# krlong014/PySolvers

Measured on AMD Instinct MI355X. Metric: CG iterations/sec + SpMV GB/s vs HBM roofline, 5-pt Laplacian N=10M, higher is better.
Workload: dtype f64

## Files before the change

include/psk_lab.h:

```cpp
#ifndef PSK_LAB_H
#define PSK_LAB_H

#include "psk.h"

#ifdef __cplusplus
extern "C" {
#endif

int psk_lab_occupy_begin(int32_t wgs, int32_t lds_bytes, double seconds);
int psk_lab_occupy_end(int32_t *timed_out);
int psk_lab_dispatch_probe(int32_t nwg, int32_t lds_bytes, double usec, int64_t *rec_out);
int psk_lab_occupy_xcc(int32_t *counts);
int psk_lab_trisolve_workers(const psk_prec *M, int32_t which, int32_t *enrolled, int32_t *grid);
int psk_lab_trisolve_plan(int64_t n, const int32_t *rowptr, const int32_t *colidx, const double *vals, int32_t upper,
                          int32_t unit, const int32_t *nat, int32_t num_cus, int64_t syncfree_waves, int32_t *schedule,
                          double *est, int64_t *info);
int psk_lab_amg_gs_pair(psk_prec *M, int32_t set, int32_t *levels_on, int32_t *levels_eligible);
int psk_lab_spmv_rotate(const psk_csr *A, const double *const *xs, double *const *ys, int32_t nbuf, int32_t reps,
                        int32_t dot, double *avg_ms);
int psk_lab_spmv_after_write(const psk_csr *A, double *x, double *y, const double *src, double *scratch,
                             int32_t target, int32_t reps, int32_t dot, double *avg_ms);
int psk_lab_cheby_ab(const psk_prec *M, const double *v, int32_t reps, double *fused_ms, double *pieces_ms);
#ifdef __cplusplus
}
#endif

#endif
```

pysolvers_amd/_native.py:

```python
import atexit
import ctypes
import os
import sys

import numpy as np

_HERE = os.path.dirname(os.path.abspath(__file__))
LIB_PATH = os.environ.get("PSK_LIBRARY", os.path.join(_HERE, "_lib", "libpsk.so"))

PSK_OK = 0
PSK_ERR_ARG, PSK_ERR_HIP, PSK_ERR_RCCL, PSK_ERR_ALLOC, PSK_ERR_UNSUPPORTED = -1, -2, -3, -4, -5
ABI_VERSION = 4
PSK_CONVERGED, PSK_MAXITER, PSK_BREAKDOWN, PSK_TRUE_RESID_FAIL = 0, 1, 2, 3
PSK_EXIT_NONE, PSK_EXIT_TOLERANCE, PSK_EXIT_ARNOLDI_BREAKDOWN, PSK_EXIT_MAXITER, PSK_EXIT_DOT_BREAKDOWN = 0, 1, 2, 3, 4
PSK_HOST, PSK_DEVICE = 0, 1
PSK_VCYCLE_X0_GIVEN = 1
PSK_PREC_IDENTITY, PSK_PREC_JACOBI, PSK_PREC_ILU, PSK_PREC_AMG, PSK_PREC_DENSE, PSK_PREC_CHEBYSHEV = 0, 1, 2, 3, 4, 5
PSK_LAYOUT_CSR, PSK_LAYOUT_SLICED, PSK_LAYOUT_SLICED_WIDE, PSK_LAYOUT_SLICED_DICT, PSK_LAYOUT_DIAG = 0, 1, 2, 3, 4
PSK_UNIQUE_ID_BYTES = 128

STATUS_NAMES = {PSK_CONVERGED: "converged", PSK_MAXITER: "maxiter", PSK_BREAKDOWN: "breakdown",
                PSK_TRUE_RESID_FAIL: "true residual above tolerance"}


class PskCtl(ctypes.Structure):
    _fields_ = [("maxiter", ctypes.c_int64), ("tau", ctypes.c_double),
                ("fail_on_maxiter", ctypes.c_int32), ("restart", ctypes.c_int32),
                ("check_every", ctypes.c_int32), ("time_kernels", ctypes.c_int32), ("norm_b", ctypes.c_double)]


class PskResult(ctypes.Structure):
    _fields_ = [("status", ctypes.c_int32), ("success", ctypes.c_int32), ("iters", ctypes.c_int64),
                ("resid", ctypes.c_double), ("resid_recursive", ctypes.c_double),
                ("norm_b", ctypes.c_double), ("loop_ms", ctypes.c_double), ("spmv_ms", ctypes.c_double),
                ("spmv_launches", ctypes.c_int64), ("hist_len", ctypes.c_int64), ("msg", ctypes.c_char * 256),
                ("exit", ctypes.c_int32), ("reserved", ctypes.c_int32),
                ("gather_ms", ctypes.c_double), ("halo_ms", ctypes.c_double), ("comm_samples", ctypes.c_int64)]


P = ctypes.c_void_p
I32, I64, F64 = ctypes.c_int32, ctypes.c_int64, ctypes.c_double
PP = ctypes.POINTER(ctypes.c_void_p)
SIGNATURES = {
    "psk_abi_version": (ctypes.c_int, []),
    "psk_last_error": (ctypes.c_char_p, []),
    "psk_device_count": (ctypes.c_int, [ctypes.POINTER(I32)]),
    "psk_set_device": (ctypes.c_int, [I32]),
    "psk_synchronize": (ctypes.c_int, []),
    "psk_shutdown": (ctypes.c_int, []),
    "psk_shutdown_ex": (ctypes.c_int, [ctypes.c_int32]),
    "psk_dmalloc": (ctypes.c_int, [I64, PP]),
    "psk_dfree": (ctypes.c_int, [P]),
    "psk_h2d": (ctypes.c_int, [P, P, I64]),
    "psk_d2h": (ctypes.c_int, [P, P, I64]),
    "psk_dmemset0": (ctypes.c_int, [P, I64]),
    "psk_csr_create": (ctypes.c_int, [I64, I64, P, P, P, I32, PP]),
    "psk_csr_create_fd2d": (ctypes.c_int, [F64, F64, I64, PP]),
    "psk_csr_create_rect": (ctypes.c_int, [I64, I64, I64, P, P, P, I32, PP]),
    "psk_csr_info": (ctypes.c_int, [P, ctypes.POINTER(I64), ctypes.POINTER(I64)]),
    "psk_csr_layout": (ctypes.c_int, [P, I32, ctypes.POINTER(I32)] + [ctypes.POINTER(I64)] * 3),
    "psk_csr_download": (ctypes.c_int, [P, P, P, P]),
    "psk_csr_destroy": (ctypes.c_int, [P]),
    "psk_spmv": (ctypes.c_int, [P, P, P, I32]),
    "psk_spmv_timed": (ctypes.c_int, [P, P, P, I32, ctypes.POINTER(F64)]),
    "psk_dot": (ctypes.c_int, [I64, P, P, I32, ctypes.POINTER(F64)]),
    "psk_nrm2": (ctypes.c_int, [I64, P, I32, ctypes.POINTER(F64)]),
    "psk_axpy": (ctypes.c_int, [I64, F64, P, P, I32]),
    "psk_prec_create": (ctypes.c_int, [P, I32, PP]),
    "psk_prec_apply": (ctypes.c_int, [P, I64, P, P, I32]),
    "psk_prec_jacobi_uniform": (ctypes.c_int, [P, ctypes.POINTER(I32), ctypes.POINTER(ctypes.c_double)]),
    "psk_prec_create_ilu": (ctypes.c_int, [I64, P, P, P, P, P, P, P, P, PP]),
    "psk_prec_destroy": (ctypes.c_int, [P]),
    "psk_prec_create_trisolve": (ctypes.c_int, [I64, P, P, P, I32, P, P, P, I32, P, P, PP]),
    "psk_prec_create_amg": (ctypes.c_int, [I32, PP, PP, PP, PP, P, I32, I32, I32, F64, PP]),
    "psk_prec_create_dense_inverse": (ctypes.c_int, [P, I32, PP]),
    "psk_prec_create_chebyshev": (ctypes.c_int, [P, I32, F64, F64, PP]),
    "psk_prec_chebyshev_info": (ctypes.c_int, [P, ctypes.POINTER(I32), ctypes.POINTER(F64), ctypes.POINTER(F64), P]),
    "psk_prec_trisolve_schedule": (ctypes.c_int, [P, I32, I32, ctypes.POINTER(I32), ctypes.POINTER(I64),
                                                   ctypes.POINTER(I32), ctypes.POINTER(F64), ctypes.POINTER(F64)]),
    "psk_prec_trisolve_grid_info": (ctypes.c_int, [P, I32, ctypes.POINTER(I64)]),
    "psk_trisolve_grid_plan": (ctypes.c_int, [I64, P, P, P, I32, ctypes.POINTER(I64)]),
    "psk_prec_info": (ctypes.c_int, [P, ctypes.POINTER(I32)] + [ctypes.POINTER(I64)] * 5),
    "psk_mm_info": (ctypes.c_int, [ctypes.c_char_p] + [ctypes.POINTER(I64)] * 3),
    "psk_mm_read": (ctypes.c_int, [ctypes.c_char_p, P, P, P, ctypes.POINTER(I64)]),
    "psk_csr_create_mm": (ctypes.c_int, [ctypes.c_char_p, PP]),
    "psk_sa_aggregate": (ctypes.c_int, [I64, P, P, P, F64, P, ctypes.POINTER(I64), P]),
    "psk_pcg": (ctypes.c_int, [P, P, P, P, ctypes.POINTER(PskCtl), ctypes.POINTER(PskResult), P, I32]),
    "psk_gmres": (ctypes.c_int, [P, P, P, P, ctypes.POINTER(PskCtl), ctypes.POINTER(PskResult), P, I32]),
    "psk_vcycle": (ctypes.c_int, [P, P, P, ctypes.POINTER(PskCtl), ctypes.POINTER(PskResult), P, I32, I32]),
    "psk_comm_unique_id": (ctypes.c_int, [P]),
    "psk_comm_init": (ctypes.c_int, [I32, I32, P, PP]),
    "psk_comm_destroy": (ctypes.c_int, [P]),
    "psk_comm_init_dry": (ctypes.c_int, [I32, I32, PP]),
    "psk_comm_init_host": (ctypes.c_int, [I32, I32, ctypes.c_char_p, PP]),
    "psk_comm_mailbox": (ctypes.c_int, [P, ctypes.c_char_p]),
    "psk_comm_mailbox_check": (ctypes.c_int, [P, I32]),
    "psk_csr_create_fd2d_dist": (ctypes.c_int, [F64, F64, I64, P, PP, ctypes.POINTER(I64),
                                                ctypes.POINTER(I64)]),
    "psk_csr_create_dist": (ctypes.c_int, [I64, P, P, P, P, P, PP]),
    "psk_csr_halo_cols": (ctypes.c_int, [P, P, ctypes.POINTER(I64)]),
    "psk_csr_halo_peers": (ctypes.c_int, [P, P, P, P, P, ctypes.POINTER(I32)]),
    "psk_csr_halo_pack": (ctypes.c_int, [P, P, P]),
    "psk_fd2d_dist_plan": (ctypes.c_int, [I64, I32, I32] + [ctypes.POINTER(I64)] * 5),
}


LAB_PATH = os.path.join(os.path.dirname(LIB_PATH), "libpsk_lab.so")
LAB_SIGNATURES = {
    "psk_lab_occupy_begin": (ctypes.c_int, [I32, I32, F64]),
    "psk_lab_occupy_end": (ctypes.c_int, [ctypes.POINTER(I32)]),
    "psk_lab_occupy_xcc": (ctypes.c_int, [ctypes.POINTER(I32)]),
    "psk_lab_dispatch_probe": (ctypes.c_int, [I32, I32, F64, P]),
    "psk_lab_trisolve_workers": (ctypes.c_int, [P, I32, ctypes.POINTER(I32), ctypes.POINTER(I32)]),
    "psk_lab_trisolve_plan": (ctypes.c_int, [I64, P, P, P, I32, I32, P, I32, I64, ctypes.POINTER(I32),
                                             ctypes.POINTER(F64), ctypes.POINTER(I64)]),
    "psk_lab_amg_gs_pair": (ctypes.c_int, [P, I32, ctypes.POINTER(I32), ctypes.POINTER(I32)]),
    "psk_lab_spmv_rotate": (ctypes.c_int, [P, ctypes.POINTER(P), ctypes.POINTER(P), I32, I32, I32, ctypes.POINTER(F64)]),
    "psk_lab_cheby_ab": (ctypes.c_int, [P, P, I32, ctypes.POINTER(F64), ctypes.POINTER(F64)]),
    "psk_lab_spmv_after_write": (ctypes.c_int, [P, P, P, P, P, I32, I32, I32, ctypes.POINTER(F64)]),
}
_lab = None


def load_lab():
    global _lab
    if _lab is None:
        if not os.path.exists(LAB_PATH):
            raise ImportError("libpsk_lab.so not found at %s (make -C pysolvers_amd/csrc)" % LAB_PATH)
        lab = ctypes.CDLL(LAB_PATH)
        for name, (res, args) in LAB_SIGNATURES.items():
            fn = getattr(lab, name)
            fn.restype = res
            fn.argtypes = args
        _lab = lab
    return _lab


def prec_info(h):
    k = I32()
    v = [I64() for _ in range(5)]
    check(lib.psk_prec_info(h, ctypes.byref(k), *[ctypes.byref(x) for x in v]), "psk_prec_info")
    return dict(kind=k.value, n=v[0].value, nnz_l=v[1].value, nnz_u=v[2].value, levels_l=v[3].value,
                levels_u=v[4].value)


def handle_array(hs):
    arr = (ctypes.c_void_p * max(len(hs), 1))()
    for i, h in enumerate(hs):
        arr[i] = h.value if isinstance(h, ctypes.c_void_p) else h
    return ctypes.cast(arr, PP), arr


def fd2d_dist_plan(m, nranks, rank):
    v = [I64() for _ in range(5)]
    check(lib.psk_fd2d_dist_plan(m, nranks, rank, *[ctypes.byref(x) for x in v]), "psk_fd2d_dist_plan")
    return tuple(x.value for x in v)


class PskError(RuntimeError):

    def __init__(self, code, where, text):
        super().__init__("%s failed (%d): %s" % (where, code, text))
        self.code = code


def _pin_runtime():
    import importlib.util
    if os.environ.get("PSK_NO_TORCH") == "1":
        return
    if importlib.util.find_spec("torch") is not None:
        import torch


def _load():
    if not os.path.exists(LIB_PATH):
        raise ImportError("libpsk.so not found at %s — build it with `python -c 'import __graft_entry__ as "
                          "g; g.build()'` (make -C pysolvers_amd/csrc)" % LIB_PATH)
    _pin_runtime()
    lib = ctypes.CDLL(LIB_PATH, mode=ctypes.RTLD_GLOBAL)
    for name, (res, args) in SIGNATURES.items():
        fn = getattr(lib, name)
        fn.restype = res
        fn.argtypes = args
    if lib.psk_abi_version() != ABI_VERSION:
        raise ImportError("libpsk ABI version mismatch (library %d, bindings %d)" % (lib.psk_abi_version(), ABI_VERSION))
    return lib


PSK_SHUTDOWN_RESET_DEVICE = 1
lib = _load()
shut_down = False


def _shutdown():
    global shut_down
    if not shut_down:
        shut_down = True
        reset = os.environ.get("PSK_SHUTDOWN_RESET") == "1"
        lib.psk_shutdown_ex(PSK_SHUTDOWN_RESET_DEVICE if reset else 0)


atexit.register(_shutdown)


def check(rc, where):
    if rc != PSK_OK:
        raise PskError(rc, where, lib.psk_last_error().decode(errors="replace"))


def ptr(a):
    if a is None:
        return None
    if isinstance(a, int):
        return ctypes.c_void_p(a)
    if isinstance(a, np.ndarray):
        return a.ctypes.data_as(ctypes.c_void_p)
    if hasattr(a, "data_ptr"):
        return ctypes.c_void_p(a.data_ptr())
    raise TypeError("cannot take the address of %r" % type(a))


def device_count():
    n = I32(0)
    check(lib.psk_device_count(ctypes.byref(n)), "psk_device_count")
    return n.value
```

pysolvers_amd/csrc/lab.hip:

```cpp
#include "trisolve.hpp"
#include "../../include/psk_lab.h"

#include <chrono>
#include <string>

namespace psk {

__global__ __launch_bounds__(1024) void occupy_kernel(uint32_t *flag, int64_t *started, uint64_t ticks,
                                                      int32_t *timed_out) {
    extern __shared__ unsigned char occ_lds[];
    if (threadIdx.x == 0) {
        occ_lds[0] = 1;
        __hip_atomic_fetch_add(started, (int64_t)1, __ATOMIC_RELAXED, __HIP_MEMORY_SCOPE_SYSTEM);
        const uint32_t xcc = __builtin_amdgcn_s_getreg((3 << 11) | 20) & 7u;
        __hip_atomic_fetch_add(reinterpret_cast<uint32_t *>(timed_out) + 32 + xcc, 1u, __ATOMIC_RELAXED,
                               __HIP_MEMORY_SCOPE_AGENT);
    }
    const uint64_t t0 = __builtin_amdgcn_s_memrealtime();
    while (__hip_atomic_load(flag, __ATOMIC_RELAXED, __HIP_MEMORY_SCOPE_AGENT) == 0) {
        if (__builtin_amdgcn_s_memrealtime() - t0 > ticks) {
            if (threadIdx.x == 0) atomicOr(timed_out, 1);
            break;
        }
        __builtin_amdgcn_s_sleep(8);
    }
}
__global__ void occupy_release_kernel(uint32_t *flag) {
    __hip_atomic_store(flag, 1u, __ATOMIC_RELAXED, __HIP_MEMORY_SCOPE_AGENT);
}

namespace {
struct Occupier {
    hipStream_t s = nullptr;
    uint32_t *dw = nullptr;
    int64_t *started = nullptr;
    bool active = false;
};
Occupier g_occ;
}

}

extern "C" int psk_lab_occupy_begin(int32_t wgs, int32_t lds_bytes, double seconds) {
    using namespace psk;
    Context *c;
    PSK_TRY(ctx(&c));
    if (g_occ.active) return fail(PSK_ERR_ARG, "psk_lab_occupy_begin: already active");
    if (wgs < 1 || lds_bytes < 16 || lds_bytes > 160 * 1024 || seconds <= 0)
        return fail(PSK_ERR_ARG, "psk_lab_occupy_begin: bad arguments");
    if (!g_occ.s) {
        PSK_HIP(hipStreamCreateWithFlags(&g_occ.s, hipStreamNonBlocking));
        PSK_HIP(hipMalloc(&g_occ.dw, 128 * sizeof(uint32_t)));
        PSK_HIP(hipHostMalloc(&g_occ.started, 64, hipHostMallocCoherent));
    }
    PSK_HIP(hipMemsetAsync(g_occ.dw, 0, 128 * sizeof(uint32_t), g_occ.s));
    PSK_HIP(hipStreamSynchronize(g_occ.s));
    *reinterpret_cast<volatile int64_t *>(g_occ.started) = 0;
    const uint64_t ticks = (uint64_t)(seconds * 1e8);
    hipLaunchKernelGGL(occupy_kernel, dim3((unsigned)wgs), dim3(1024), (size_t)lds_bytes, g_occ.s, g_occ.dw,
                       g_occ.started, ticks, reinterpret_cast<int32_t *>(g_occ.dw + 64));
    PSK_HIP(hipGetLastError());
    g_occ.active = true;
    const auto t0 = std::chrono::steady_clock::now();
    while (*reinterpret_cast<volatile int64_t *>(g_occ.started) < wgs &&
           std::chrono::steady_clock::now() - t0 < std::chrono::seconds(5)) {
    }
    const int64_t got = *reinterpret_cast<volatile int64_t *>(g_occ.started);
    return got >= wgs ? PSK_OK : fail(PSK_ERR_HIP, "psk_lab_occupy_begin: only " + std::to_string(got) + " of " +
                                                       std::to_string(wgs) + " occupiers started");
}

extern "C" int psk_lab_occupy_end(int32_t *timed_out) {
    using namespace psk;
    Context *c;
    PSK_TRY(ctx(&c));
    if (!g_occ.active) return fail(PSK_ERR_ARG, "psk_lab_occupy_end: not active");
    hipLaunchKernelGGL(occupy_release_kernel, dim3(1), dim3(1), 0, c->stream, g_occ.dw);
    PSK_HIP(hipGetLastError());
    PSK_HIP(hipStreamSynchronize(g_occ.s));
    int32_t h = 0;
    PSK_HIP(hipMemcpy(&h, g_occ.dw + 64, sizeof(int32_t), hipMemcpyDeviceToHost));
    g_occ.active = false;
    if (timed_out) *timed_out = h;
    return PSK_OK;
}

__global__ void dispatch_probe_kernel(uint64_t ticks, int64_t *rec) {
    extern __shared__ unsigned char dp_lds[];
    if (threadIdx.x == 0) {
        dp_lds[0] = 1;
        const uint64_t t0 = __builtin_amdgcn_s_memrealtime();
        uint64_t t = t0;
        while (t - t0 < ticks) {
            __builtin_amdgcn_s_sleep(4);
            t = __builtin_amdgcn_s_memrealtime();
        }
        rec[3 * blockIdx.x + 0] = (int64_t)t0;
        rec[3 * blockIdx.x + 1] = (int64_t)t;
        rec[3 * blockIdx.x + 2] = (int64_t)(__builtin_amdgcn_s_getreg((3 << 11) | 20) & 7u);
    }
}

extern "C" int psk_lab_dispatch_probe(int32_t nwg, int32_t lds_bytes, double usec, int64_t *rec_out) {
    using namespace psk;
    if (nwg < 1 || lds_bytes < 16 || lds_bytes > 160 * 1024 || usec < 0 || !rec_out)
        return fail(PSK_ERR_ARG, "psk_lab_dispatch_probe: bad arguments");
    Context *c;
    PSK_TRY(ctx(&c));
    int64_t *rec = nullptr;
    PSK_HIP(hipMalloc(&rec, (size_t)nwg * 3 * sizeof(int64_t)));
    hipLaunchKernelGGL(dispatch_probe_kernel, dim3((unsigned)nwg), dim3(128), (size_t)lds_bytes, c->stream,
                       (uint64_t)(usec * 100.0), rec);
    hipError_t e = hipGetLastError();
    if (e == hipSuccess) e = hipMemcpyAsync(rec_out, rec, (size_t)nwg * 3 * sizeof(int64_t), hipMemcpyDeviceToHost, c->stream);
    if (e == hipSuccess) e = hipStreamSynchronize(c->stream);
    (void)hipFree(rec);
    return e == hipSuccess ? PSK_OK : fail(PSK_ERR_HIP, hipGetErrorString(e));
}

extern "C" int psk_lab_occupy_xcc(int32_t *counts) {
    using namespace psk;
    if (!counts || !g_occ.dw) return fail(PSK_ERR_ARG, "psk_lab_occupy_xcc: no occupiers yet");
    PSK_HIP(hipMemcpy(counts, g_occ.dw + 96, 8 * sizeof(int32_t), hipMemcpyDeviceToHost));
    return PSK_OK;
}

extern "C" int psk_lab_trisolve_workers(const psk_prec *M, int32_t which, int32_t *enrolled, int32_t *grid) {
    using namespace psk;
    if (!M || M->kind != PSK_PREC_ILU) return fail(PSK_ERR_ARG, "psk_lab_trisolve_workers: not a triangular-solve chain");
    const TriFactor &T = which == 0 ? M->lo : M->up;
    if (!T.present || !T.sched) return fail(PSK_ERR_ARG, "psk_lab_trisolve_workers: factor absent");
    Context *c;
    PSK_TRY(ctx(&c));
    uint32_t v = 0;
    PSK_HIP(hipStreamSynchronize(c->stream));
    PSK_HIP(hipMemcpy(&v, T.sched + kSchedLast, sizeof(uint32_t), hipMemcpyDeviceToHost));
    if (enrolled) *enrolled = (int32_t)v;
    if (grid) *grid = syncfree_grid(c);
    return PSK_OK;
}

extern "C" int psk_lab_trisolve_plan(int64_t n, const int32_t *rowptr, const int32_t *colidx, const double *vals,
                                     int32_t upper, int32_t unit, const int32_t *nat, int32_t num_cus,
                                     int64_t syncfree_waves, int32_t *schedule, double *est, int64_t *info) {
    using namespace psk;
    if (n < 0 || !rowptr || (rowptr[n] > 0 && (!colidx || !vals)) || num_cus < 1 || syncfree_waves < 1 || !schedule || !est || !info)
        return fail(PSK_ERR_ARG, "psk_lab_trisolve_plan: bad arguments");
    FactorPlan P;
    PSK_TRY(plan_factor(n, rowptr, colidx, vals, upper != 0, unit != 0,
                        nat ? std::vector<int32_t>(nat, nat + n) : std::vector<int32_t>(), num_cus, syncfree_waves, P));
    const TriFactor &T = P.T;
    *schedule = T.schedule;
    for (int i = 0; i < 6; ++i) est[i] = T.est_us[i];
    const int64_t v[8] = {T.levels, T.band.K, T.band.nblocks, T.band.ring_words, T.band.narrow ? 1 : 0,
                          T.grid.K, T.grid.dict_n, T.lv.steps};
    for (int i = 0; i < 8; ++i) info[i] = v[i];
    return PSK_OK;
}

extern "C" int psk_lab_cheby_ab(const psk_prec *M, const double *v, int32_t reps, double *fused_ms, double *pieces_ms) {
    return psk::cheby_ab(M, v, reps, fused_ms, pieces_ms);
}

extern "C" int psk_lab_amg_gs_pair(psk_prec *M, int32_t set, int32_t *levels_on, int32_t *levels_eligible) {
    using namespace psk;
    if (set < -1 || set > 1) return fail(PSK_ERR_ARG, "psk_lab_amg_gs_pair: set must be -1, 0 or 1");
    Context *c;
    PSK_TRY(ctx(&c));
    PSK_HIP(hipStreamSynchronize(c->stream));
    int on = 0, el = 0;
    PSK_TRY(amg_gs_pair(M, set, &on, &el));
    if (levels_on) *levels_on = on;
    if (levels_eligible) *levels_eligible = el;
    return PSK_OK;
}

__global__ __launch_bounds__(256) void lab_copy_kernel(int64_t n, const double *__restrict__ src, double *__restrict__ dst) {
    const int64_t i = ((int64_t)blockIdx.x * 256 + threadIdx.x) * 2;
    if (i + 1 < n) {
        const double2 v = *reinterpret_cast<const double2 *>(src + i);
        *reinterpret_cast<double2 *>(dst + i) = v;
    } else if (i < n) {
        dst[i] = src[i];
    }
}

extern "C" int psk_lab_spmv_rotate(const psk_csr *A, const double *const *xs, double *const *ys, int32_t nbuf,
                                   int32_t reps, int32_t dot, double *avg_ms) {
    using namespace psk;
    if (!A || !xs || !ys || nbuf < 1 || reps < 1 || !avg_ms) return fail(PSK_ERR_ARG, "psk_lab_spmv_rotate: bad arguments");
    if (A->comm) return fail(PSK_ERR_UNSUPPORTED, "psk_lab_spmv_rotate: sharded matrix");
    for (int32_t i = 0; i < nbuf; ++i)
        if (!xs[i] || !ys[i]) return fail(PSK_ERR_ARG, "psk_lab_spmv_rotate: NULL buffer");
    Context *c;
    PSK_TRY(ctx(&c));
    hipEvent_t e0, e1;
    PSK_HIP(hipEventCreateWithFlags(&e0, hipEventDisableSystemFence));
    PSK_HIP(hipEventCreateWithFlags(&e1, hipEventDisableSystemFence));
    const int mode = dot ? kSpmvDot : kSpmvPlain;
    DevBuf part;
    int rc = part.ensure(64);
    double *pp = dot ? part.as<double>() : nullptr;
    for (int32_t i = 0; i < nbuf && rc == PSK_OK; ++i)
        rc = launch_spmv(A, mode, xs[i], ys[i], nullptr, nullptr, pp, nullptr, c->stream);
    if (rc == PSK_OK && hipEventRecord(e0, c->stream) != hipSuccess) rc = fail(PSK_ERR_HIP, "event record");
    for (int32_t r = 0; r < reps && rc == PSK_OK; ++r)
        rc = launch_spmv(A, mode, xs[r % nbuf], ys[r % nbuf], nullptr, nullptr, pp, nullptr, c->stream);
    if (rc == PSK_OK && hipEventRecord(e1, c->stream) != hipSuccess) rc = fail(PSK_ERR_HIP, "event record");
    float ms = 0.f;
    if (rc == PSK_OK && hipEventSynchronize(e1) != hipSuccess) rc = fail(PSK_ERR_HIP, "event sync");
    if (rc == PSK_OK && hipEventElapsedTime(&ms, e0, e1) != hipSuccess) rc = fail(PSK_ERR_HIP, "event time");
    (void)hipStreamSynchronize(c->stream);
    (void)hipEventDestroy(e0);
    (void)hipEventDestroy(e1);
    part.release();
    if (rc == PSK_OK) *avg_ms = (double)ms / reps;
    return rc;
}

extern "C" int psk_lab_spmv_after_write(const psk_csr *A, double *x, double *y, const double *src, double *scratch,
                                        int32_t target, int32_t reps, int32_t dot, double *avg_ms) {
    using namespace psk;
    if (!A || !x || !y || !src || !scratch || reps < 1 || reps > 256 || !avg_ms)
        return fail(PSK_ERR_ARG, "psk_lab_spmv_after_write: bad arguments");
    if (A->comm || A->ncols != A->n) return fail(PSK_ERR_UNSUPPORTED, "psk_lab_spmv_after_write: square unsharded only");
    Context *c;
    PSK_TRY(ctx(&c));
    std::vector<hipEvent_t> ea((size_t)reps), eb((size_t)reps);
    for (int32_t r = 0; r < reps; ++r) {
        PSK_HIP(hipEventCreateWithFlags(&ea[(size_t)r], hipEventDisableSystemFence));
        PSK_HIP(hipEventCreateWithFlags(&eb[(size_t)r], hipEventDisableSystemFence));
    }
    const int mode = dot ? kSpmvDot : kSpmvPlain;
    DevBuf part;
    int rc = part.ensure(64);
    double *pp = dot ? part.as<double>() : nullptr;
    const int64_t n = A->n;
    const unsigned g = (unsigned)((n + 511) / 512);
    double *dst = target == 1 ? x : scratch;
    rc = launch_spmv(A, mode, x, y, nullptr, nullptr, pp, nullptr, c->stream);
    for (int32_t r = 0; r < reps && rc == PSK_OK; ++r) {
        if (target > 0) {
            hipLaunchKernelGGL(lab_copy_kernel, dim3(g), dim3(256), 0, c->stream, n, src, dst);
            if (hipGetLastError() != hipSuccess) rc = fail(PSK_ERR_HIP, "lab copy");
        }
        if (rc == PSK_OK)
            rc = launch_spmv(A, mode, x, y, nullptr, nullptr, pp, nullptr, c->stream, ea[(size_t)r], eb[(size_t)r]);
    }
    double tot = 0.0;
    if (rc == PSK_OK && hipStreamSynchronize(c->stream) != hipSuccess) rc = fail(PSK_ERR_HIP, "sync");
    for (int32_t r = 0; r < reps && rc == PSK_OK; ++r) {
        float ms = 0.f;
        if (hipEventElapsedTime(&ms, ea[(size_t)r], eb[(size_t)r]) != hipSuccess) rc = fail(PSK_ERR_HIP, "event time");
        tot += ms;
    }
    (void)hipStreamSynchronize(c->stream);
    for (int32_t r = 0; r < reps; ++r) {
        (void)hipEventDestroy(ea[(size_t)r]);
        (void)hipEventDestroy(eb[(size_t)r]);
    }
    part.release();
    if (rc == PSK_OK) *avg_ms = tot / reps;
    return rc;
}
```

pysolvers_amd/csrc/pcg.hip:

```cpp
#include "psk_internal.hpp"
#include "pcg_state.hpp"

#include <cstdlib>

#include <climits>
#include <cmath>
#include <cstdio>


namespace psk {

template <int JAC, bool FUSED>
__global__ __launch_bounds__(kBlock) void pcg_init_kernel(int64_t n, const double *__restrict__ b,
                                                          const double *__restrict__ dinv, double ds,
                                                          double *__restrict__ p, GridSum gs, PcgInitFin fin,
                                                          int64_t ntiles) {
    constexpr int TPW = 2;
    const int tid = threadIdx.x;
    int64_t tl[TPW];
    bool tv[TPW];
    double acc[TPW][2];
    uint32_t ticket[TPW];
#pragma unroll
    for (int q = 0; q < TPW; ++q) {
        const int64_t t = (int64_t)blockIdx.x * TPW + q;
        tv[q] = t < ntiles;
        tl[q] = tv[q] ? t : ntiles - 1;
        const int64_t row = tl[q] * kBlock + tid;
        const bool has = tv[q] && row < n;
        const double bi = has ? __builtin_nontemporal_load(b + row) : 0.0;
        const double d = JAC == 1 ? (has ? dinv[row] : 0.0) : ds;
        const double u = JAC ? d * bi : bi;
        if (has) p[row] = u;
        acc[q][0] = has ? bi * bi : 0.0;
        acc[q][1] = has ? u * bi : 0.0;
    }
    __shared__ GridSumTile<2> gsl[TPW];
#pragma unroll
    for (int q = 0; q < TPW; ++q) {
        ticket[q] = 0;
        if (tv[q] && gs.grp_log2 >= 0 && tid == 0)
            ticket[q] = gridsum_draw(gridsum_counter(gs, gridsum_group_of(tl[q], gs.grp_log2)));
    }
    if (tid < TPW) gsl[tid].cnt = 0;
    if (tid == 0 && blockIdx.x == 0 && (gs.nt + TPW - 1) / TPW != gridDim.x) atomicOr(gs.err, 2);
    __syncthreads();
    if (FUSED)
        gridsum_tiles_publish<TPW, 2>(gs, gsl, acc, ticket, tl, tv, fin);
    else
        gridsum_tiles_publish<TPW, 2>(gs, gsl, acc, ticket, tl, tv);
}

__global__ void pcg_init_finish_kernel(const double *g, int P, double tau, PcgState *st, double *udr,
                                       int64_t *hdone, int64_t hgen) {
    if (threadIdx.x == 0) pcg_init_state(rank_sum(g, P, 2, 0), rank_sum(g, P, 2, 1), tau, st, udr, hdone, hgen, 0);
}

template <int JAC, bool FIRST>
__global__ __launch_bounds__(kBlock) void pcg_update_kernel(
    int64_t n, double *__restrict__ r, const double *__restrict__ b, const double *__restrict__ Ap,
    const double *__restrict__ dinv, double ds, const double *__restrict__ pap, int nparts, GridSum gs, PcgState *st,
    const double *__restrict__ udr, int64_t k, TileMap tm) {
    const double udk = udr[k];
    const int32_t dn = st->done;
    const double pap0 = pap[0];
    __asm__ volatile("" ::"s"(dn), "s"(pap0), "s"(udk));
    if (dn) return;
    double pTAp = pap0;
    for (int q = 1; q < nparts; ++q) pTAp += pap[q];
    __shared__ double sh[2 * kWaves];
    if (pTAp == 0.0) {
        if (blockIdx.x == 0 && threadIdx.x == 0) {
            st->brk_kind = 2;
            st->iters = k;
            set_done(st, 2, k + 2);
        }
        return;
    }
    const double alpha = udk / pTAp;
    if (blockIdx.x == 0 && threadIdx.x == 0) st->live = k;
    const int64_t tile = tile_of_block(tm);
    const int64_t i = tile * kVecTile + 2 * threadIdx.x;
    const bool pair = i + 1 < n;
    uint32_t ticket = 0;
    double rr = 0.0, ur = 0.0;
    if (pair) {
        const dv2 ro = FIRST ? ld2nt(b + i) : ld2(r + i), a = ld2nt(Ap + i);
        dv2 d{ds, ds};
        if (JAC == 1) d = ld2(dinv + i);
        ticket = gridsum_ticket(gs, tile);
        dv2 rn;
        rn.x = ro.x - alpha * a.x;
        rn.y = ro.y - alpha * a.y;
        double u0 = rn.x, u1 = rn.y;
        if (JAC) {
            u0 = d.x * rn.x;
            u1 = d.y * rn.y;
        }
        st2(r + i, rn);
        rr = fma(rn.x, rn.x, rr);
        rr = fma(rn.y, rn.y, rr);
        ur = fma(u0, rn.x, ur);
        ur = fma(u1, rn.y, ur);
    } else if (i < n) {
        ticket = gridsum_ticket(gs, tile);
        const double rn = (FIRST ? b[i] : r[i]) - alpha * Ap[i];
        const double u0 = JAC == 2 ? ds * rn : JAC ? dinv[i] * rn : rn;
        r[i] = rn;
        rr = rn * rn;
        ur = u0 * rn;
    }
    block_sum2(rr, ur, sh);
    const double v[2] = {rr, ur};
    if (threadIdx.x >= 64) return;
    const bool lane0 = threadIdx.x == 0;
    if (gs.grp_log2 < 0) {
        if (lane0) {
            gridsum_put(gs.gslots + tile * 2, v[0]);
            gridsum_put(gs.gslots + tile * 2 + 1, v[1]);
        }
        gridsum_final_wave<2>(gs);
        return;
    }
    if (lane0) {
        gridsum_put(gs.slots + gridsum_slot(gs, tile) * 2, v[0]);
        gridsum_put(gs.slots + gridsum_slot(gs, tile) * 2 + 1, v[1]);
    }
    const uint32_t tk = __builtin_amdgcn_readfirstlane(ticket);
    const int64_t g = gridsum_group_of(tile, gs.grp_log2);
    int64_t base;
    const int64_t cnt = gridsum_members(gs, g, base);
    if (tk != (uint32_t)(cnt - 1)) return;
    double gr[2];
    gridsum_take<2, 64>(gs.slots, g << gs.grp_log2, cnt, gs.err, nullptr, gr);
    if (lane0) {
        gridsum_reset(gridsum_counter(gs, g));
        gridsum_put(gs.gslots + g * 2, gr[0]);
        gridsum_put(gs.gslots + g * 2 + 1, gr[1]);
    }
    gridsum_final_wave<2>(gs);
}

template <int JAC>
__global__ __launch_bounds__(kBlock) void pcg_direction_kernel(
    int64_t n, double *__restrict__ x, const double *__restrict__ r, PRing pr, const double *__restrict__ dinv,
    double ds, const double *__restrict__ pap, const double *__restrict__ rrur, int nparts, PcgState *st,
    double *__restrict__ udr, double *__restrict__ hist, double *__restrict__ alphas, int64_t k, int64_t maxiter,
    int fail_on_maxiter, int64_t tile_base, TileMap tm) {
    const double udk = udr[k];
    const int64_t live = st->live;
    const double tauNB = st->tauNormB, pap0 = pap[0], rr0 = rrur[0], ur0 = rrur[1];
    __asm__ volatile("" ::"s"(live), "s"(pap0), "s"(rr0), "s"(ur0), "s"(udk), "s"(tauNB));
    if (live != k) return;
    double pTAp = pap0, rr = rr0, ur = ur0;
    for (int q = 1; q < nparts; ++q) {
        pTAp += pap[q];
        rr += rrur[2 * q];
        ur += rrur[2 * q + 1];
    }
    const int64_t tile = tile_base + tile_of_block(tm);
    const double *pcur = pr.b[k % kPcgDefer];
    double *pnext = pr.b[(k + 1) % kPcgDefer];
    const int q = pcg_pending(k);
    double alpha, beta;
    if (!pcg_direction_scalars(n, x, pcur, pTAp, rr, ur, udk, tauNB, st, udr, hist, k, maxiter, fail_on_maxiter,
                               alpha, beta, tile, &pr, alphas))
        return;
    const bool flush = q == kPcgDefer - 1 || k == maxiter - 1;
    const bool x0 = k < kPcgDefer;
    if (tile == 0 && threadIdx.x == 0) {
        alphas[k] = alpha;
        if (flush) st->x_written = 1;
    }
    const int64_t i = tile * kVecTile + 2 * threadIdx.x;
    if (i + 1 < n) {
        const dv2 ro = ld2nt(r + i), po = ld2(pcur + i);
        dv2 d{ds, ds};
        if (JAC == 1) d = ld2nt(dinv + i);
        double u0 = ro.x, u1 = ro.y;
        if (JAC) {
            u0 = d.x * ro.x;
            u1 = d.y * ro.y;
        }
        if (flush) {
            dv2 xo{0.0, 0.0};
            if (!x0) xo = ld2nt(x + i);
            dv2 pp[kPcgDefer > 1 ? kPcgDefer - 1 : 1];
#pragma unroll
            for (int t = 1; t < kPcgDefer; ++t)
                if (t <= q) pp[t - 1] = ld2nt(pr.b[(k - t) % kPcgDefer] + i);
#pragma unroll
            for (int t = kPcgDefer - 1; t >= 1; --t)
                if (t <= q) {
                    const double a = alphas[k - t];
                    xo.x = xo.x + a * pp[t - 1].x;
                    xo.y = xo.y + a * pp[t - 1].y;
                }
            dv2 xn;
            xn.x = xo.x + alpha * po.x;
            xn.y = xo.y + alpha * po.y;
            st2nt(x + i, xn);
        }
        dv2 pn;
        pn.x = u0 + beta * po.x;
        pn.y = u1 + beta * po.y;
        st2(pnext + i, pn);
    } else if (i < n) {
        const double u0 = JAC == 2 ? ds * r[i] : JAC ? dinv[i] * r[i] : r[i];
        const double pi = pcur[i];
        if (flush) x[i] = pcg_catch_up(x0 ? 0.0 : x[i], &pr, q, k, alphas, i) + alpha * pi;
        pnext[i] = u0 + beta * pi;
    }
}

__global__ void pcg_flush_kernel(int64_t n, double *__restrict__ x, PRing pr, const double *__restrict__ alphas,
                                 int64_t k) {
    const int64_t i = (int64_t)blockIdx.x * kBlock + threadIdx.x;
    if (i < n) x[i] = pcg_catch_up(k < kPcgDefer ? 0.0 : x[i], &pr, pcg_pending(k), k, alphas, i);
}

constexpr int kPcgStateWords = (int)(sizeof(PcgState) / 8);
constexpr int kPcgFinishWord = 8;
static_assert(sizeof(PcgState) % 8 == 0 && kPcgFinishWord + kPcgStateWords + 1 <= 64, "SolveKit::hmap words");
__global__ __launch_bounds__(kBlock) void pcg_finish_kernel(const PcgState *st, const uint32_t *cnt, const int32_t *err,
                                                            int64_t *hw) {
    constexpr int kPer = (kGridSumMaxGroups + kBlock) / kBlock;
    uint32_t v[kPer];
#pragma unroll
    for (int i = 0; i < kPer; ++i) {
        const int g = (int)threadIdx.x + i * kBlock;
        v[i] = cnt[(int64_t)(g < kGridSumMaxGroups ? g : kGridSumMaxGroups) * kGridSumCntStride];
    }
    uint32_t any = 0;
#pragma unroll
    for (int i = 0; i < kPer; ++i) any |= v[i];
    const bool bad = __syncthreads_or(any != 0);
    if (threadIdx.x < kPcgStateWords)
        __hip_atomic_store(hw + threadIdx.x, reinterpret_cast<const int64_t *>(st)[threadIdx.x], __ATOMIC_RELAXED,
                           __HIP_MEMORY_SCOPE_SYSTEM);
    if (threadIdx.x == 0)
        __hip_atomic_store(hw + kPcgStateWords, (int64_t)(*err | (bad ? 4 : 0)), __ATOMIC_RELAXED,
                           __HIP_MEMORY_SCOPE_SYSTEM);
}

__global__ __launch_bounds__(kBlock) void pcg_gen_init_kernel(int64_t n, const double *__restrict__ b,
                                                              double *__restrict__ x, double *__restrict__ r) {
    const int64_t i = (int64_t)blockIdx.x * kBlock + threadIdx.x;
    if (i < n) {
        r[i] = b[i];
        x[i] = 0.0;
    }
}

__global__ __launch_bounds__(kBlock) void pcg_gen_init2_kernel(int64_t n, const double *__restrict__ r,
                                                               const double *__restrict__ u, double *__restrict__ p,
                                                               GridSum gs, PcgInitFin fin) {
    __shared__ double sh[kWaves];
    const int64_t i = (int64_t)blockIdx.x * kVecTile + 2 * threadIdx.x;
    const uint32_t ticket = gridsum_ticket(gs);
    double bb = 0.0, ur = 0.0;
    for (int64_t j = i; j < i + 2 && j < n; ++j) {
        const double rj = r[j], uj = u[j];
        p[j] = uj;
        bb = fma(rj, rj, bb);
        ur = fma(uj, rj, ur);
    }
    const double v[2] = {block_sum(bb, sh), block_sum(ur, sh)};
    gridsum_publish<2>(gs, v, sh, ticket, fin);
}

__global__ __launch_bounds__(kBlock) void pcg_dot_kernel(int64_t n, const double *__restrict__ a,
                                                         const double *__restrict__ c, GridSum gs,
                                                         const PcgState *st) {
    if (st->done) return;
    __shared__ double sh[kWaves];
    const int64_t i = (int64_t)blockIdx.x * kVecTile + threadIdx.x;
    const uint32_t ticket = gridsum_ticket(gs);
    double acc = 0.0;
    if (i < n) acc = a[i] * c[i];
    if (i + kBlock < n) acc = fma(a[i + kBlock], c[i + kBlock], acc);
    const double v = block_sum(acc, sh);
    gridsum_publish<1>(gs, &v, sh, ticket);
}

__global__ __launch_bounds__(kBlock) void pcg_gen_direction_kernel(
    int64_t n, double *__restrict__ x, const double *__restrict__ u, double *__restrict__ p,
    const double *__restrict__ pap, const double *__restrict__ rrur, const double *__restrict__ ur_gen, PcgState *st,
    double *__restrict__ udr, double *__restrict__ hist, int64_t k, int64_t maxiter, int fail_on_maxiter) {
    if (st->live != k) return;
    double alpha, beta;
    if (!pcg_direction_scalars(n, x, p, *pap, rrur[0], *ur_gen, udr[k], st->tauNormB, st, udr, hist, k, maxiter,
                               fail_on_maxiter, alpha, beta, blockIdx.x))
        return;
    const int64_t i = (int64_t)blockIdx.x * kVecTile + 2 * threadIdx.x;
    for (int64_t j = i; j < i + 2 && j < n; ++j) {
        const double pj = p[j];
        x[j] = x[j] + alpha * pj;
        p[j] = u[j] + beta * pj;
    }
}


static inline size_t align_up(size_t v, size_t a) { return (v + a - 1) / a * a; }

struct PcgWork {
    double *x, *r, *p, *Ap, *u, *part1, *part2, *part3, *udr, *hist;
    PRing pr;
    double *alphas;
    double *pinit;
    double *part1g, *part2g, *initg;
    PcgState *st;
};

static int pcg_workspace(psk_csr *A, int64_t maxiter, bool gen, bool own_x, int P, PcgWork &w) {
    const size_t vec = align_up((size_t)A->n * 8, 256), vecc = align_up((size_t)A->ncols * 8, 256);
    const size_t nx = own_x ? 1 : 0;
    const size_t big = (2 + nx + (gen ? 1 : 0)) * vec + (gen ? 1 : kPcgDefer) * vecc;
    PSK_TRY(A->ws.ensure(big > 0 ? big : 256));
    char *b = A->ws.as<char>();
    w.r = reinterpret_cast<double *>(b);
    w.Ap = reinterpret_cast<double *>(b + vec);
    w.x = own_x ? reinterpret_cast<double *>(b + 2 * vec) : nullptr;
    char *pb = b + (2 + nx) * vec;
    w.p = reinterpret_cast<double *>(pb);
    w.u = gen ? reinterpret_cast<double *>(pb + vecc) : nullptr;
    for (int t = 0; t < kPcgDefer; ++t)
        w.pr.b[t] = gen ? (t == 0 ? w.p : nullptr) : reinterpret_cast<double *>(pb + t * vecc);
    const size_t small = align_up(sizeof(PcgState), 256) + 2 * align_up(kMaxGrid * 8, 256) +
                         align_up(2 * kMaxGrid * 8, 256) + align_up((size_t)(maxiter + 2) * 8, 256) +
                         align_up((size_t)(maxiter + 1) * 8, 256) + align_up((size_t)(maxiter + 1) * 8, 256) + 256;
    const size_t gath = P > 1 ? align_up((size_t)P * 8, 256) + 2 * align_up((size_t)P * 16, 256) : 0;
    PSK_TRY(A->ws_small.ensure(small + gath));
    char *s = A->ws_small.as<char>();
    w.st = reinterpret_cast<PcgState *>(s);
    s += align_up(sizeof(PcgState), 256);
    w.part1 = reinterpret_cast<double *>(s);
    s += align_up(kMaxGrid * 8, 256);
    w.part3 = reinterpret_cast<double *>(s);
    s += align_up(kMaxGrid * 8, 256);
    w.part2 = reinterpret_cast<double *>(s);
    s += align_up(2 * kMaxGrid * 8, 256);
    w.udr = reinterpret_cast<double *>(s);
    s += align_up((size_t)(maxiter + 2) * 8, 256);
    w.hist = reinterpret_cast<double *>(s);
    s += align_up((size_t)(maxiter + 1) * 8, 256);
    w.alphas = reinterpret_cast<double *>(s);
    s += align_up((size_t)(maxiter + 1) * 8, 256);
    w.pinit = reinterpret_cast<double *>(s);
    s += 256;
    if (P > 1) {
        w.part1g = reinterpret_cast<double *>(s);
        s += align_up((size_t)P * 8, 256);
        w.part2g = reinterpret_cast<double *>(s);
        s += align_up((size_t)P * 16, 256);
        w.initg = reinterpret_cast<double *>(s);
    } else {
        w.part1g = w.part1;
        w.part2g = w.part2;
        w.initg = w.pinit;
    }
    return PSK_OK;
}

static void set_msg(psk_result *res, const char *m) {
    std::snprintf(res->msg, sizeof(res->msg), "%s", m);
}

}

using namespace psk;

extern "C" int psk_pcg(const psk_csr *Ac, const psk_prec *M, const double *b, double *xout,
                       const psk_ctl *ctl, psk_result *res, double *hist, int32_t loc) {
    if (!Ac || !b || !xout || !ctl || !res) return fail(PSK_ERR_ARG, "psk_pcg: NULL argument");
    if (ctl->maxiter < 0) return fail(PSK_ERR_ARG, "psk_pcg: maxiter < 0");
    if (M && M->n != Ac->n) return fail(PSK_ERR_ARG, "psk_pcg: preconditioner size mismatch");
    if (!Ac->comm && Ac->ncols != Ac->n) return fail(PSK_ERR_ARG, "psk_pcg: matrix must be square");
    psk_csr *A = const_cast<psk_csr *>(Ac);
    Context *c;
    PSK_TRY(ctx(&c));
    std::lock_guard<std::mutex> solve_lock(c->solve_mu);
    hipStream_t s = c->stream;
    std::memset(res, 0, sizeof(*res));
    const int64_t n = A->n, maxiter = ctl->maxiter;
    const bool gen = prec_is_general(M);
    if (gen && A->comm) return fail(PSK_ERR_UNSUPPORTED, "psk_pcg: ILU preconditioning of a sharded matrix");
    const bool sharded = A->comm != nullptr;
    const int P = sharded ? A->comm->nranks : 1;
    const bool dev_io = loc == PSK_DEVICE;
    PcgWork w;
    PSK_TRY(pcg_workspace(A, maxiter, gen, !dev_io, P, w));
    if (dev_io) w.x = xout;
    SolveKit *kit;
    PSK_TRY(solve_kit(c, ctl->time_kernels > 0, &kit));
    const double *dinv = (M && M->kind == PSK_PREC_JACOBI) ? M->dinv : nullptr;
    const int jac = !dinv ? 0 : M->dinv_uniform ? 2 : 1;
    const double ds = jac == 2 ? M->dinv_value : 0.0;
    const int64_t nv = n > 0 ? (n + kVecTile - 1) / kVecTile : 1;
    if (nv > INT32_MAX) return fail(PSK_ERR_UNSUPPORTED, "psk_pcg: vector too long for a one-shot grid");
    const bool init_diag = !gen && !sharded && (jac == 0 || jac == 2) && pcg_init_diag_eligible(A);
    const int64_t nsl = n > 0 ? (n + kBlock - 1) / kBlock : 1;
    GridSum gs0, gs2, gs3;
    if (!init_diag) PSK_TRY(gridsum_prepare(c, gen ? nv : nsl, 2, w.pinit, &gs0));
    PSK_TRY(gridsum_prepare(c, nv, 2, w.part2, &gs2));
    PSK_TRY(gridsum_prepare(c, nv, 1, w.part3, &gs3));
    volatile int64_t *hdone = kit->hmap;
    const int64_t hgen = (int64_t)(++kit->solve_gen & 0x7FFFFF) << kStampGenShift;
    *hdone = 0;
    const PcgInitFin fin{ctl->tau, w.st, w.udr, const_cast<int64_t *>(hdone), hgen, gen ? 1 : 0, 0};
    const double *bd = b;
    if (!dev_io) {
        PSK_TRY(to_device_vec(b, loc, n, gen ? w.Ap : w.r, s));
        bd = gen ? w.Ap : w.r;
    }
    psk_comm *mbc = sharded && A->comm->mb ? A->comm : nullptr;
    uint64_t seq0 = 0;
    if (mbc) seq0 = mbox_next(mbc, &gs0);
    PSK_HIP(hipEventRecord(kit->ev0, s));
    const dim3 gk((unsigned)nv);
    if (gen) {
        const unsigned nb = (unsigned)((n + kBlock - 1) / kBlock);
        if (n > 0) hipLaunchKernelGGL(pcg_gen_init_kernel, dim3(nb), dim3(kBlock), 0, s, n, bd, w.x, w.r);
        PSK_TRY(prec_apply_dev(M, n, w.r, w.u, s));
        hipLaunchKernelGGL(pcg_gen_init2_kernel, gk, dim3(kBlock), 0, s, n, w.r, w.u, w.p, gs0, fin);
    } else if (init_diag) {
        PcgInitFin fin3 = fin;
        fin3.off = 1;
        PSK_TRY(launch_pcg_init_diag(A, bd, jac == 2 ? ds : 1.0, w.p, w.Ap, w.part1, fin3, s));
    } else {
        const dim3 gi((unsigned)((nsl + 1) / 2));
#define PSK_PCG_INIT(J, F) \
        hipLaunchKernelGGL((pcg_init_kernel<J, F>), gi, dim3(kBlock), 0, s, n, bd, dinv, ds, w.p, gs0, fin, nsl)
        if (jac == 2) { if (sharded) PSK_PCG_INIT(2, false); else PSK_PCG_INIT(2, true); }
        else if (jac == 1) { if (sharded) PSK_PCG_INIT(1, false); else PSK_PCG_INIT(1, true); }
        else { if (sharded) PSK_PCG_INIT(0, false); else PSK_PCG_INIT(0, true); }
#undef PSK_PCG_INIT
    }
    PSK_HIP(hipGetLastError());
    if (sharded) {
        if (mbc) PSK_TRY(mbox_gather(mbc, seq0, 2, w.initg, nullptr, s));
        else PSK_TRY(allgather(A, w.pinit, w.initg, 2, s));
        hipLaunchKernelGGL(pcg_init_finish_kernel, dim3(1), dim3(64), 0, s, w.initg, P, ctl->tau, w.st, w.udr,
                           const_cast<int64_t *>(hdone), hgen);
        PSK_HIP(hipGetLastError());
    }

    const int L = 2, NS = kPollSlots;
    static_assert(kPollSlots >= L + 2, "poll slots");
    int C = ctl->check_every > 0 ? ctl->check_every : (n >= (1 << 20) ? 2 : 16);
    hipEvent_t *fev = kit->fev;
    const int TP = kTimedSlots;
    hipEvent_t *ta = kit->ta, *tb = kit->tb;
    int64_t tk[kTimedSlots];
    bool tgat[kTimedSlots], thalo[kTimedSlots];
    for (int i = 0; i < TP; ++i) {
        tk[i] = -1;
        tgat[i] = thalo[i] = false;
    }
    std::vector<float> spmv_ms;
    if (ctl->time_kernels) spmv_ms.assign((size_t)maxiter, -1.0f);
    double gat_sum = 0.0, halo_sum = 0.0;
    int64_t gat_n = 0, halo_n = 0;
    auto harvest = [&](int slot) -> int {
        if (tk[slot] < 0) return PSK_OK;
        float ms = 0.f;
        PSK_HIP(hipEventSynchronize(tb[slot]));
        PSK_HIP(hipEventElapsedTime(&ms, ta[slot], tb[slot]));
        spmv_ms[(size_t)tk[slot]] = ms;
        tk[slot] = -1;
        if (tgat[slot]) {
            PSK_HIP(hipEventSynchronize(kit->gb[slot]));
            PSK_HIP(hipEventElapsedTime(&ms, kit->ga[slot], kit->gb[slot]));
            gat_sum += ms;
            ++gat_n;
            tgat[slot] = false;
        }
        if (thalo[slot]) {
            PSK_HIP(hipEventSynchronize(kit->hb[slot]));
            PSK_HIP(hipEventElapsedTime(&ms, kit->ha[slot], kit->hb[slot]));
            halo_sum += ms;
            ++halo_n;
            thalo[slot] = false;
        }
        return PSK_OK;
    };

    int64_t ov_lo = 0, ov_hi = nv;
    static const bool overlap_on = [] {
        const char *e = std::getenv("PSK_HALO_OVERLAP");
        return !(e && std::atoi(e) == 0);
    }();
    const bool overlap = overlap_on && sharded && !gen && halo_split(A, kVecTile, nv, ov_lo, ov_hi);
    hipStream_t cs = nullptr;
    hipEvent_t ev_k3a = kit->ev_a, ev_halo = kit->ev_b;
    bool halo_pending = false;
    if (overlap) PSK_TRY(comm_stream(c, &cs));

    int64_t launched = 0;
    int rc = PSK_OK;
    for (int64_t k = 0; k < maxiter && rc == PSK_OK; ++k) {
        if (k > 0 && k % C == 0) {
            const int64_t chunk = k / C;
            const int slot = (int)((chunk - 1) % NS);
            if (hipEventRecord(fev[slot], s) != hipSuccess) rc = fail(PSK_ERR_HIP, "event");
            if (rc == PSK_OK && chunk - 1 - L >= 0) {
                const int os = (int)((chunk - 1 - L) % NS);
                if (hipEventSynchronize(fev[os]) != hipSuccess) rc = fail(PSK_ERR_HIP, "event sync");
                else {
                    const int64_t hv = *hdone;
                    if ((hv & ~kStampMask) == hgen && (hv & kStampMask) != 0 &&
                        (hv & kStampMask) <= (chunk - L) * (int64_t)C + 1)
                        break;
                }
            }
            if (rc != PSK_OK) break;
        }
        double *pk = gen ? w.p : w.pr.b[k % kPcgDefer];
        double *pn = gen ? w.p : w.pr.b[(k + 1) % kPcgDefer];
        const bool timed = ctl->time_kernels > 0 && k % ctl->time_kernels == 0 && !(init_diag && k == 0);
        int slot = (int)((k / (ctl->time_kernels > 0 ? ctl->time_kernels : 1)) % TP);
        if (timed) {
            if ((rc = harvest(slot)) != PSK_OK) break;
            tk[slot] = k;
        }
        if (halo_pending) {
            if (hipStreamWaitEvent(s, ev_halo, 0) != hipSuccess) { rc = fail(PSK_ERR_HIP, "halo wait"); break; }
            halo_pending = false;
        } else if (A->comm) {
            const bool th = timed && !A->comm->dry && !A->peers.empty();
            if (th && hipEventRecord(kit->ha[slot], s) != hipSuccess) { rc = fail(PSK_ERR_HIP, "event"); break; }
            if ((rc = halo_exchange(A, pk, s)) != PSK_OK) break;
            if (th) {
                if (hipEventRecord(kit->hb[slot], s) != hipSuccess) { rc = fail(PSK_ERR_HIP, "event"); break; }
                thalo[slot] = true;
            }
        }
        uint64_t seq1 = 0;
        if (!(init_diag && k == 0) &&
            (rc = launch_spmv(A, kSpmvDot, pk, w.Ap, nullptr, nullptr, w.part1, &w.st->done, s, timed ? ta[slot] : nullptr,
                              timed ? tb[slot] : nullptr, 0, mbc ? &seq1 : nullptr)) != PSK_OK)
            break;
        const TileMap tm2 = tile_map_for(nv, false);
        if (sharded) {
            hipEvent_t g0 = timed ? kit->ga[slot] : nullptr, g1 = timed ? kit->gb[slot] : nullptr;
            if (mbc) {
                rc = mbox_gather(mbc, seq1, 1, w.part1g, &w.st->done, s, g0, g1);
            } else {
                if (g0 && hipEventRecord(g0, s) != hipSuccess) rc = fail(PSK_ERR_HIP, "event");
                if (rc == PSK_OK) rc = allgather(A, w.part1, w.part1g, 1, s);
                if (rc == PSK_OK && g1 && hipEventRecord(g1, s) != hipSuccess) rc = fail(PSK_ERR_HIP, "event");
            }
            if (rc != PSK_OK) break;
            if (timed) tgat[slot] = true;
        }
        GridSum gs2k = gs2;
        const uint64_t seq2 = mbc ? mbox_next(mbc, &gs2k) : 0;
        const bool first = k == 0 && !gen && dev_io;
        const double *pap_k = w.part1g;
#define PSK_PCG_K2(J, F)                                                                                       \
        hipLaunchKernelGGL((pcg_update_kernel<J, F>), gk, dim3(kBlock), 0, s, n, w.r, bd, w.Ap, dinv, ds, pap_k,     \
                           P, gs2k, w.st, w.udr, k, tm2)
        if (jac == 2) { if (first) PSK_PCG_K2(2, true); else PSK_PCG_K2(2, false); }
        else if (jac == 1) { if (first) PSK_PCG_K2(1, true); else PSK_PCG_K2(1, false); }
        else { if (first) PSK_PCG_K2(0, true); else PSK_PCG_K2(0, false); }
#undef PSK_PCG_K2
        if (sharded && (rc = mbc ? mbox_gather(mbc, seq2, 2, w.part2g, &w.st->done, s)
                                 : allgather(A, w.part2, w.part2g, 2, s)) != PSK_OK)
            break;
        if (gen) {
            if ((rc = prec_apply_dev(M, n, w.r, w.u, s)) != PSK_OK) break;
            hipLaunchKernelGGL(pcg_dot_kernel, gk, dim3(kBlock), 0, s, n, w.u, w.r, gs3, w.st);
            hipLaunchKernelGGL(pcg_gen_direction_kernel, gk, dim3(kBlock), 0, s, n, w.x, w.u, w.p, w.part1, w.part2,
                               w.part3, w.st, w.udr, w.hist, k, maxiter, ctl->fail_on_maxiter);
        } else {
            auto k3 = [&](int64_t t0, int64_t t1) {
                if (t1 <= t0) return;
                const dim3 g3((unsigned)(t1 - t0));
                const TileMap tm3 = tile_map_for(t1 - t0, false);
                if (jac == 2)
                    hipLaunchKernelGGL(pcg_direction_kernel<2>, g3, dim3(kBlock), 0, s, n, w.x, w.r, w.pr, dinv, ds,
                                       w.part1g, w.part2g, P, w.st, w.udr, w.hist, w.alphas, k, maxiter,
                                       ctl->fail_on_maxiter, t0, tm3);
                else if (jac == 1)
                    hipLaunchKernelGGL(pcg_direction_kernel<1>, g3, dim3(kBlock), 0, s, n, w.x, w.r, w.pr, dinv, ds,
                                       w.part1g, w.part2g, P, w.st, w.udr, w.hist, w.alphas, k, maxiter,
                                       ctl->fail_on_maxiter, t0, tm3);
                else
                    hipLaunchKernelGGL(pcg_direction_kernel<0>, g3, dim3(kBlock), 0, s, n, w.x, w.r, w.pr, dinv, ds,
                                       w.part1g, w.part2g, P, w.st, w.udr, w.hist, w.alphas, k, maxiter,
                                       ctl->fail_on_maxiter, t0, tm3);
            };
            if (overlap && k + 1 < maxiter) {
                k3(0, ov_lo);
                k3(ov_hi, nv);
                if ((rc = halo_exchange_async(A, pn, s, cs, ev_k3a, ev_halo, timed ? kit->ha[slot] : nullptr,
                                              timed ? kit->hb[slot] : nullptr)) != PSK_OK)
                    break;
                if (timed) thalo[slot] = true;
                k3(ov_lo, ov_hi);
                halo_pending = true;
            } else {
                k3(0, nv);
            }
        }
        if (hipGetLastError() != hipSuccess) { rc = fail(PSK_ERR_HIP, "pcg launch"); break; }
        launched = k + 1;
    }
    if (halo_pending && hipStreamWaitEvent(s, ev_halo, 0) != hipSuccess && rc == PSK_OK) rc = fail(PSK_ERR_HIP, "halo wait");
    if (rc == PSK_OK && hipEventRecord(kit->ev1, s) != hipSuccess) rc = fail(PSK_ERR_HIP, "event");
    int64_t *hw = kit->hmap + kPcgFinishWord;
    if (rc == PSK_OK) {
        hipLaunchKernelGGL(pcg_finish_kernel, dim3(1), dim3(kBlock), 0, s, w.st, c->gs_cnt, c->gs_err, hw);
        if (hipGetLastError() != hipSuccess) rc = fail(PSK_ERR_HIP, "pcg finish");
    }
    if (rc == PSK_OK && hipStreamSynchronize(s) != hipSuccess) rc = fail(PSK_ERR_HIP, "pcg sync");
    PcgState hs;
    std::memcpy(&hs, hw, sizeof(PcgState));
    if (rc == PSK_OK) rc = gridsum_check_result(c, (int32_t)hw[kPcgStateWords]);
    if (rc == PSK_OK && gen) rc = prec_check_error(M, s);
    if (rc == PSK_OK && ctl->time_kernels)
        for (int i = 0; i < TP && rc == PSK_OK; ++i) rc = harvest(i);
    if (rc == PSK_OK) {
        float ms = 0.f;
        (void)hipEventElapsedTime(&ms, kit->ev0, kit->ev1);
        res->loop_ms = ms;
        res->norm_b = hs.normB;
        int64_t nk = 0, nhist = 0;
        if (hs.done == 1) {
            res->status = PSK_CONVERGED;
            res->success = 1;
            res->iters = hs.iters;
            res->resid = hs.resid;
            res->exit = hs.normB == 0.0 ? PSK_EXIT_NONE
                        : hs.resid <= hs.tauNormB ? PSK_EXIT_TOLERANCE : PSK_EXIT_MAXITER;
            nk = nhist = hs.normB == 0.0 ? 0 : hs.iters;
        } else if (hs.done == 2) {
            res->status = PSK_BREAKDOWN;
            res->exit = PSK_EXIT_DOT_BREAKDOWN;
            res->success = 0;
            res->iters = hs.iters;
            res->resid = NAN;
            set_msg(res, hs.brk_kind == 1 ? "breakdown dot(u,r)==0" : "breakdown dot(p, Ap)==0");
            nk = hs.brk_kind == 1 ? 0 : hs.iters + 1;
            nhist = hs.brk_kind == 1 ? 0 : hs.iters;
        } else {
            res->status = PSK_MAXITER;
            res->exit = PSK_EXIT_MAXITER;
            res->success = 0;
            res->iters = maxiter > 0 ? maxiter - 1 : 0;
            set_msg(res, "failure to converge");
            nk = nhist = launched;
        }
        const int64_t nh = nhist < maxiter ? nhist : maxiter;
        if (hist && nh > 0 && hipMemcpy(hist, w.hist, (size_t)nh * 8, hipMemcpyDeviceToHost) != hipSuccess)
            rc = fail(PSK_ERR_HIP, "hist copy");
        if (rc == PSK_OK) {
            res->hist_len = nh;
            res->resid_recursive = nh > 0 ? hs.last_hist : hs.normB;
            if (res->status == PSK_MAXITER) res->resid = maxiter > 0 ? res->resid_recursive : hs.normB;
            bool x_written = hs.x_written != 0;
            bool more = !dev_io;
            if (!gen && hs.done == 2 && hs.brk_kind != 1 && pcg_pending(hs.iters) > 0 && n > 0) {
                hipLaunchKernelGGL(pcg_flush_kernel, dim3((unsigned)((n + kBlock - 1) / kBlock)), dim3(kBlock), 0, s, n,
                                   w.x, w.pr, w.alphas, (int64_t)hs.iters);
                if (hipGetLastError() != hipSuccess) rc = fail(PSK_ERR_HIP, "pcg flush");
                x_written = true;
                more = true;
            }
            if (rc == PSK_OK && !x_written && n > 0) {
                if (hipMemsetAsync(w.x, 0, (size_t)n * 8, s) != hipSuccess) rc = fail(PSK_ERR_HIP, "x zero");
                more = true;
            }
            if (rc == PSK_OK && !dev_io) rc = from_device_vec(w.x, loc, n, xout, s);
            if (rc == PSK_OK && more && hipStreamSynchronize(s) != hipSuccess) rc = fail(PSK_ERR_HIP, "x copy");
        }
        if (ctl->time_kernels) {
            double tot = 0.0;
            const int64_t cnt = nk < (int64_t)spmv_ms.size() ? nk : (int64_t)spmv_ms.size();
            int64_t nt = 0;
            for (int64_t i = 0; i < cnt; i += ctl->time_kernels)
                if (spmv_ms[(size_t)i] >= 0.0f) {
                    tot += spmv_ms[(size_t)i];
                    ++nt;
                }
            res->spmv_launches = nt;
            res->spmv_ms = nt > 0 ? tot / (double)nt : 0.0;
            res->gather_ms = gat_n > 0 ? gat_sum / (double)gat_n : 0.0;
            res->halo_ms = halo_n > 0 ? halo_sum / (double)halo_n : 0.0;
            res->comm_samples = gat_n;
        }
    }
    if (rc != PSK_OK) (void)hipStreamSynchronize(s);
    return rc;
}
```

pysolvers_amd/csrc/pcg_state.hpp:

```cpp
#pragma once
#include "psk_internal.hpp"

namespace psk {

struct PcgState {
    int32_t done;
    int32_t brk_kind;
    int64_t iters;
    double resid;
    double normB;
    double tauNormB;
    int64_t live;
    int64_t *hdone;
    int64_t hgen;
    double last_hist;
    int32_t x_written;
    int32_t pad;
};

constexpr int kStampGenShift = 40;
constexpr int64_t kStampMask = ((int64_t)1 << kStampGenShift) - 1;
__device__ __forceinline__ void set_done(PcgState *st, int32_t v, int64_t stamp) {
    st->done = v;
    if (st->hdone) {
        __hip_atomic_store(st->hdone, st->hgen | stamp, __ATOMIC_RELAXED, __HIP_MEMORY_SCOPE_SYSTEM);
        __threadfence_system();
    }
}

__device__ __forceinline__ void pcg_init_state(double bb, double ur, double tau, PcgState *st, double *udr,
                                               int64_t *hdone, int64_t hgen, int32_t x_written) {
    const double normB = sqrt(bb);
    st->normB = normB;
    st->tauNormB = tau * normB;
    st->iters = 0;
    st->resid = 0.0;
    st->brk_kind = 0;
    st->live = -1;
    st->hdone = hdone;
    st->hgen = hgen;
    st->last_hist = normB;
    st->x_written = x_written;
    udr[0] = ur;
    if (normB == 0.0) {
        st->iters = 1;
        set_done(st, 1, 1);
    } else if (ur == 0.0) {
        st->brk_kind = 1;
        st->iters = 0;
        set_done(st, 2, 1);
    } else {
        st->done = 0;
    }
}

struct PcgInitFin {
    double tau;
    PcgState *st;
    double *udr;
    int64_t *hdone;
    int64_t hgen;
    int32_t x_written;
    int32_t off;
    __device__ void operator()(const double *r) const {
        pcg_init_state(r[off], r[off + 1], tau, st, udr, hdone, hgen, x_written);
    }
};

#ifndef PSK_PCG_DEFER
#define PSK_PCG_DEFER 8
#endif
constexpr int kPcgDefer = PSK_PCG_DEFER;
static_assert(kPcgDefer >= 1 && kPcgDefer <= 8, "kPcgDefer");
struct PRing {
    double *b[kPcgDefer];
};
__host__ __device__ inline int pcg_pending(int64_t k) { return (int)(k % kPcgDefer); }

__device__ __forceinline__ double pcg_catch_up(double xj, const PRing *pr, int q, int64_t k,
                                               const double *__restrict__ alphas, int64_t j) {
    for (int t = q; t >= 1; --t) xj = xj + alphas[k - t] * pr->b[(k - t) % kPcgDefer][j];
    return xj;
}

__device__ inline bool pcg_direction_scalars(int64_t n, double *__restrict__ x, const double *__restrict__ p,
                                             double pTAp, double rr, double ur, double udk, double tauNB,
                                             PcgState *st, double *__restrict__ udr, double *__restrict__ hist, int64_t k,
                                             int64_t maxiter, int fail_on_maxiter, double &alpha, double &beta,
                                             int64_t tile, const PRing *pr = nullptr,
                                             const double *__restrict__ alphas = nullptr) {
    alpha = udk / pTAp;
    const double normR = sqrt(rr);
    if (tile == 0 && threadIdx.x == 0) {
        hist[k] = normR;
        st->last_hist = normR;
    }
    if (normR <= tauNB || (!fail_on_maxiter && k == maxiter - 1)) {
        const int64_t i = tile * kVecTile + 2 * threadIdx.x;
        const bool x0 = pr && k < kPcgDefer;
        for (int64_t j = i; j < i + 2 && j < n; ++j) {
            double xj = x0 ? 0.0 : x[j];
            if (pr) xj = pcg_catch_up(xj, pr, pcg_pending(k), k, alphas, j);
            x[j] = xj + alpha * p[j];
        }
        if (tile == 0 && threadIdx.x == 0) {
            st->iters = k + 1;
            st->resid = normR;
            st->x_written = 1;
            set_done(st, 1, k + 2);
        }
        return false;
    }
    beta = ur / udk;
    if (tile == 0 && threadIdx.x == 0) udr[k + 1] = ur;
    return true;
}

bool pcg_init_diag_eligible(const psk_csr *A);
int launch_pcg_init_diag(const psk_csr *A, const double *b, double xs, double *p, double *Ap, double *out3,
                         const PcgInitFin &fin, hipStream_t s);

}
```

pysolvers_amd/csrc/psk_internal.hpp:

```cpp
#pragma once

#include <hip/hip_runtime.h>
#include <rccl/rccl.h>

#include <cstdint>
#include <cstring>
#include <mutex>
#include <string>
#include <vector>

#include "../../include/psk.h"

namespace psk {

constexpr int kBlock = 256;
constexpr int kWaves = kBlock / 64;
constexpr int kChunk = 1280;
constexpr int kMaxGrid = 2048;
constexpr int kVecTile = 2 * kBlock;
constexpr int64_t kMaxNnz = (int64_t)INT32_MAX - kChunk - kBlock;

void set_error(int code, const std::string &msg);
int fail(int code, const std::string &msg);
const char *hip_err_str(hipError_t e);
// ... 356 lines not shown
    const int64_t t = gs.nt - sb * S;
    return t >= S ? ((int64_t)1 << gl) : (t - l + kGridSumL - 1) >> kGridSumLLog;
}

__device__ __forceinline__ void gridsum_put(uint64_t *sl, double v) {
    __hip_atomic_store(sl, (uint64_t)__double_as_longlong(v), __ATOMIC_RELAXED, __HIP_MEMORY_SCOPE_AGENT);
}
__device__ __forceinline__ uint32_t gridsum_draw(uint32_t *c) {
    return __hip_atomic_fetch_add(c, 1u, __ATOMIC_RELAXED, __HIP_MEMORY_SCOPE_AGENT);
}
__device__ __forceinline__ void gridsum_reset(uint32_t *c) {
    __hip_atomic_store(c, 0u, __ATOMIC_RELAXED, __HIP_MEMORY_SCOPE_AGENT);
}
__device__ __forceinline__ uint32_t *gridsum_counter(const GridSum &gs, int64_t g) {
    return gs.cnt + g * kGridSumCntStride;
}
__device__ __forceinline__ uint64_t gridsum_wait(const uint64_t *sl, int32_t *err) {
    uint64_t bits = __hip_atomic_load(sl, __ATOMIC_RELAXED, __HIP_MEMORY_SCOPE_AGENT);
    if (bits != kGridSumSentinel) return bits;
    const uint64_t t0 = __builtin_amdgcn_s_memrealtime();
    while ((bits = __hip_atomic_load(sl, __ATOMIC_RELAXED, __HIP_MEMORY_SCOPE_AGENT)) == kGridSumSentinel) {
        if (__builtin_amdgcn_s_memrealtime() - t0 > kGridSumWaitTicks) {
            atomicOr(err, 1);
            return 0x7FF8000000000000ull;
        }
        __builtin_amdgcn_s_sleep(1);
    }
    return bits;
}

template <int W, int NT>
__device__ __forceinline__ void gridsum_take(uint64_t *src, int64_t start, int64_t cnt, int32_t *err, double *sh,
                                             double *res) {
    constexpr int B = NT == 64 ? 8 : 4;
    const uint32_t lane = NT == 64 ? (threadIdx.x & 63) : threadIdx.x;
    const uint32_t n = (uint32_t)cnt;
    uint64_t *p = src + start * W;
#pragma unroll
    for (int c = 0; c < W; ++c) {
        double a = 0.0;
        bool ok = true;
        for (uint32_t m0 = lane; m0 < n; m0 += NT * B) {
            uint64_t v[B];
#pragma unroll
            for (int i = 0; i < B; ++i) {
                const uint32_t m = __builtin_elementwise_min(m0 + (uint32_t)(i * NT), n - 1);
                v[i] = __hip_atomic_load(p + (m * W + c), __ATOMIC_RELAXED, __HIP_MEMORY_SCOPE_AGENT);
            }
#pragma unroll
            for (int i = 0; i < B; ++i) {
                const uint64_t x = m0 + (uint32_t)(i * NT) < n ? v[i] : 0x8000000000000000ull;
                ok = ok && x != kGridSumSentinel;
                a += __longlong_as_double((long long)x);
            }
        }
        if (!ok) {
            a = 0.0;
            for (uint32_t m = lane; m < n; m += NT)
                a += __longlong_as_double((long long)gridsum_wait(p + (m * W + c), err));
        }
        for (uint32_t m = lane; m < n; m += NT)
            p[m * W + c] = kGridSumSentinel;
        res[c] = NT == 64 ? wave_total(a) : block_sum(a, sh);
    }
}

__device__ __forceinline__ int64_t gridsum_slot(const GridSum &gs, int64_t t) {
    const int32_t gl = gs.grp_log2;
    const int64_t g = gridsum_group_of(t, gl), j = (t & ((kGridSumL << gl) - 1)) >> kGridSumLLog;
    return (g << gl) + j;
}

__device__ __forceinline__ uint32_t gridsum_ticket(const GridSum &gs, int64_t tile) {
    uint32_t t = 0;
    if (threadIdx.x == 0 && gridDim.x != gs.nt) atomicOr(gs.err, 2);
    if (gs.grp_log2 >= 0 && threadIdx.x == 0) t = gridsum_draw(gridsum_counter(gs, gridsum_group_of(tile, gs.grp_log2)));
    return t;
}
__device__ __forceinline__ uint32_t gridsum_ticket(const GridSum &gs) { return gridsum_ticket(gs, blockIdx.x); }

struct GridSumNoFin {
    __device__ void operator()(const double *) const {}
};

template <int W, class F = GridSumNoFin>
__device__ __forceinline__ void gridsum_final(const GridSum &gs, double *sh, const F &fin = F()) {
    __shared__ uint32_t tk;
    if (threadIdx.x == 0) tk = gridsum_draw(gridsum_counter(gs, kGridSumMaxGroups));
    __syncthreads();
    const bool last = tk == (uint32_t)(gs.ngroups - 1);
    __syncthreads();
    if (!last) return;
    double r[W];
    gridsum_take<W, kBlock>(gs.gslots, 0, gs.ngroups, gs.err, sh, r);
    if (threadIdx.x == 0) {
        gridsum_reset(gridsum_counter(gs, kGridSumMaxGroups));
#pragma unroll
        for (int c = 0; c < W; ++c) gs.out[c] = r[c];
        gridsum_mail<W>(gs, r);
        fin(r);
    }
}

template <int W, class F = GridSumNoFin>
__device__ __forceinline__ void gridsum_publish_tile(const GridSum &gs, const double *v, double *sh, uint32_t ticket,
                                                     int64_t b, const F &fin = F()) {
    if (gs.grp_log2 < 0) {
        if (threadIdx.x == 0)
#pragma unroll
            for (int c = 0; c < W; ++c) gridsum_put(gs.gslots + b * W + c, v[c]);
        gridsum_final<W>(gs, sh, fin);
        return;
    }
    __shared__ uint32_t tk;
    if (threadIdx.x == 0) {
#pragma unroll
        for (int c = 0; c < W; ++c) gridsum_put(gs.slots + gridsum_slot(gs, b) * W + c, v[c]);
        tk = ticket;
    }
    __syncthreads();
    const int64_t g = gridsum_group_of(b, gs.grp_log2);
    int64_t base;
    const int64_t cnt = gridsum_members(gs, g, base);
    const bool last = tk == (uint32_t)(cnt - 1);
    __syncthreads();
    if (!last) return;
    double r[W];
    gridsum_take<W, kBlock>(gs.slots, g << gs.grp_log2, cnt, gs.err, sh, r);
    if (threadIdx.x == 0) {
        gridsum_reset(gridsum_counter(gs, g));
#pragma unroll
        for (int c = 0; c < W; ++c) gridsum_put(gs.gslots + g * W + c, r[c]);
    }
    gridsum_final<W>(gs, sh, fin);
}
template <int W, class F = GridSumNoFin>
__device__ __forceinline__ void gridsum_publish(const GridSum &gs, const double *v, double *sh, uint32_t ticket,
                                                const F &fin = F()) {
    gridsum_publish_tile<W>(gs, v, sh, ticket, blockIdx.x, fin);
}

template <int W>
struct GridSumTile {
    uint32_t cnt;
    uint32_t ticket;
    double part[kWaves * W];
};
template <int W>
__device__ __forceinline__ uint32_t gridsum_tile_begin(const GridSum &gs, GridSumTile<W> &L, int64_t tile) {
    if (threadIdx.x == 0) {
        L.cnt = 0;
        if (gridDim.x != gs.nt) atomicOr(gs.err, 2);
    }
    __syncthreads();
    uint32_t t = 0;
    if (gs.grp_log2 >= 0 && threadIdx.x == 0) t = gridsum_draw(gridsum_counter(gs, gridsum_group_of(tile, gs.grp_log2)));
    return t;
}

template <int W, class F = GridSumNoFin>
__device__ __forceinline__ void gridsum_final_wave(const GridSum &gs, const F &fin = F()) {
    const bool lane0 = (threadIdx.x & 63) == 0;
    uint32_t f = 0;
    if (lane0) f = gridsum_draw(gridsum_counter(gs, kGridSumMaxGroups));
    f = __builtin_amdgcn_readfirstlane(f);
    if (f != (uint32_t)(gs.ngroups - 1)) return;
    double r[W];
    gridsum_take<W, 64>(gs.gslots, 0, gs.ngroups, gs.err, nullptr, r);
    if (lane0) {
        gridsum_reset(gridsum_counter(gs, kGridSumMaxGroups));
#pragma unroll
        for (int c = 0; c < W; ++c) gs.out[c] = r[c];
        gridsum_mail<W>(gs, r);
        fin(r);
    }
}

template <int W>
__device__ __forceinline__ void gridsum_tile_publish(const GridSum &gs, GridSumTile<W> &L, const double *v,
                                                     uint32_t ticket, int64_t tile) {
    const bool lane0 = (threadIdx.x & 63) == 0;
    const int wave = __builtin_amdgcn_readfirstlane(threadIdx.x >> 6);
    uint32_t old = 0;
    if (lane0) {
#pragma unroll
        for (int c = 0; c < W; ++c) L.part[wave * W + c] = v[c];
        if (threadIdx.x == 0) L.ticket = ticket;
        __builtin_amdgcn_fence(__ATOMIC_RELEASE, "workgroup", "local");
        old = atomicAdd(&L.cnt, 1u);
    }
    if (__builtin_amdgcn_readfirstlane(old) != kWaves - 1) return;
    __builtin_amdgcn_fence(__ATOMIC_ACQUIRE, "workgroup", "local");
    double s[W];
#pragma unroll
    for (int c = 0; c < W; ++c) {
        s[c] = L.part[c];
#pragma unroll
        for (int w = 1; w < kWaves; ++w) s[c] += L.part[w * W + c];
    }
    const uint32_t tk = L.ticket;
    if (gs.grp_log2 < 0) {
        if (lane0)
#pragma unroll
            for (int c = 0; c < W; ++c) gridsum_put(gs.gslots + tile * W + c, s[c]);
        gridsum_final_wave<W>(gs);
        return;
    }
    if (lane0)
#pragma unroll
        for (int c = 0; c < W; ++c) gridsum_put(gs.slots + gridsum_slot(gs, tile) * W + c, s[c]);
    const int64_t g = gridsum_group_of(tile, gs.grp_log2);
    int64_t base;
    const int64_t cnt = gridsum_members(gs, g, base);
    if (tk != (uint32_t)(cnt - 1)) return;
    double r[W];
    gridsum_take<W, 64>(gs.slots, g << gs.grp_log2, cnt, gs.err, nullptr, r);
    if (lane0) {
        gridsum_reset(gridsum_counter(gs, g));
#pragma unroll
        for (int c = 0; c < W; ++c) gridsum_put(gs.gslots + g * W + c, r[c]);
    }
    gridsum_final_wave<W>(gs);
}

template <int TPW, int W, class F = GridSumNoFin>
__device__ __forceinline__ void gridsum_tiles_publish(const GridSum &gs, GridSumTile<W> *L, const double (*acc)[W],
                                                      const uint32_t *ticket, const int64_t *tl, const bool *tv,
                                                      const F &fin = F()) {
    const bool lane0 = (threadIdx.x & 63) == 0;
    const int wave = __builtin_amdgcn_readfirstlane(threadIdx.x >> 6);
    bool mine[TPW];
    uint32_t tk[TPW];
#pragma unroll
    for (int q = 0; q < TPW; ++q) {
        mine[q] = false;
        tk[q] = 0;
        if (!tv[q]) continue;
        double ws[W];
#pragma unroll
        for (int c = 0; c < W; ++c) ws[c] = wave_total(acc[q][c]);
        uint32_t old = 0;
        if (lane0) {
#pragma unroll
            for (int c = 0; c < W; ++c) L[q].part[wave * W + c] = ws[c];
            if (threadIdx.x == 0) L[q].ticket = ticket[q];
            __builtin_amdgcn_fence(__ATOMIC_RELEASE, "workgroup", "local");
            old = atomicAdd(&L[q].cnt, 1u);
        }
        if (__builtin_amdgcn_readfirstlane(old) != kWaves - 1) continue;
        __builtin_amdgcn_fence(__ATOMIC_ACQUIRE, "workgroup", "local");
        double sum[W];
#pragma unroll
        for (int c = 0; c < W; ++c) {
            sum[c] = L[q].part[c];
#pragma unroll
            for (int w = 1; w < kWaves; ++w) sum[c] += L[q].part[w * W + c];
        }
        tk[q] = L[q].ticket;
        if (lane0)
#pragma unroll
            for (int c = 0; c < W; ++c)
                gridsum_put(gs.grp_log2 < 0 ? gs.gslots + tl[q] * W + c : gs.slots + gridsum_slot(gs, tl[q]) * W + c, sum[c]);
        mine[q] = true;
    }
#pragma unroll
    for (int q = 0; q < TPW; ++q) {
        if (!mine[q]) continue;
        if (gs.grp_log2 < 0) {
            gridsum_final_wave<W>(gs, fin);
            continue;
        }
        const int64_t g = gridsum_group_of(tl[q], gs.grp_log2);
        int64_t base;
        const int64_t cnt = gridsum_members(gs, g, base);
        if (tk[q] != (uint32_t)(cnt - 1)) continue;
        double r[W];
        gridsum_take<W, 64>(gs.slots, g << gs.grp_log2, cnt, gs.err, nullptr, r);
        if (lane0) {
            gridsum_reset(gridsum_counter(gs, g));
#pragma unroll
            for (int c = 0; c < W; ++c) gridsum_put(gs.gslots + g * W + c, r[c]);
        }
        gridsum_final_wave<W>(gs, fin);
    }
}

int gridsum_prepare(Context *c, int64_t nt, int W, double *out, GridSum *gs);
int gridsum_check(Context *c);
int gridsum_check_enqueue(Context *c, int32_t *host_word);
int gridsum_check_result(Context *c, int32_t host_word);

struct TileMap {
    int64_t a;
    int32_t r;
    int32_t rev;
    int64_t c;
};
inline TileMap tile_map_for(int64_t ntiles, bool banded, bool rev = false) {
    return banded && ntiles >= 64 ? TileMap{ntiles >> 3, (int32_t)(ntiles & 7), rev ? 1 : 0, 0} : TileMap{0, 0, 0, 0};
}
inline TileMap tile_map_chunked(int64_t ntiles, int64_t c) {
    return c > 0 && ntiles >= 8 * c ? TileMap{0, 0, 0, c} : TileMap{0, 0, 0, 0};
}
__device__ __forceinline__ int64_t tile_of_block(TileMap tm) {
    const int64_t b = blockIdx.x;
    if (tm.c > 0) {
        const int64_t k = b & 7, j = b >> 3;
        const int64_t t = ((j / tm.c) * 8 + k) * tm.c + j % tm.c;
        const int64_t full = (int64_t)(gridDim.x / (8 * tm.c)) * 8 * tm.c;
        return b < full ? t : b;
    }
    if (tm.a == 0) return b;
    const int64_t k = b & 7, j = b >> 3;
    const int64_t start = k * tm.a + (k < tm.r ? k : tm.r);
    return tm.rev ? start + (tm.a + (k < tm.r ? 1 : 0)) - 1 - j : start + j;
}

typedef double dv2 __attribute__((ext_vector_type(2)));
__device__ __forceinline__ dv2 ld2(const double *p) { return *reinterpret_cast<const dv2 *>(p); }
__device__ __forceinline__ dv2 ld2nt(const double *p) {
    return __builtin_nontemporal_load(reinterpret_cast<const dv2 *>(p));
}
__device__ __forceinline__ void st2(double *p, dv2 v) { *reinterpret_cast<dv2 *>(p) = v; }
__device__ __forceinline__ void st2nt(double *p, dv2 v) { __builtin_nontemporal_store(v, reinterpret_cast<dv2 *>(p)); }

__device__ __forceinline__ void block_range(int64_t ntiles, int64_t &t0, int64_t &t1) {
    const int64_t g = gridDim.x, b = blockIdx.x;
    t0 = ntiles * b / g;
    t1 = ntiles * (b + 1) / g;
}

inline int grid_for_rows(const Context *c, int64_t rows, int per_tile) {
    int64_t tiles = (rows + per_tile - 1) / per_tile;
    if (tiles < 1) tiles = 1;
    return (int)(tiles < c->grid_cap ? tiles : c->grid_cap);
}

int to_device_vec(const double *src, int32_t loc, int64_t n, double *dst, hipStream_t s);
int from_device_vec(const double *src, int32_t loc, int64_t n, double *dst, hipStream_t s);
int halo_exchange(psk_csr *A, double *x_local, hipStream_t s);
int halo_exchange_async(psk_csr *A, double *x, hipStream_t s, hipStream_t cs, hipEvent_t ev_a, hipEvent_t ev_b,
                        hipEvent_t t0 = nullptr, hipEvent_t t1 = nullptr);
bool halo_split(const psk_csr *A, int64_t tile, int64_t nv, int64_t &lo, int64_t &hi);
int allgather(psk_csr *A, const double *send, double *recv, int64_t count, hipStream_t s);
uint64_t mbox_next(psk_comm *c, GridSum *gs);
int mbox_gather(psk_comm *c, uint64_t seq, int W, double *recv, const int32_t *done, hipStream_t s,
                hipEvent_t ev0 = nullptr, hipEvent_t ev1 = nullptr);

enum SpmvMode : int {
    kSpmvPlain = 0,
    kSpmvDot = 1,
    kSpmvJacobiDot = 2,
    kSpmvPlainDot = 3,
    kSpmvResid = 4,
    kSpmvAdd = 5,
};
int fd2d_fill(psk_csr *A, int64_t m, double a, double b, int64_t row_begin, int64_t row_end,
              int64_t halo_lo_start, hipStream_t s);
int prec_apply_dev(const psk_prec *M, int64_t n, const double *v, double *out, hipStream_t s);
int ilu_apply(const psk_prec *M, const double *v, double *out, hipStream_t s);
int ilu_apply_add(const psk_prec *M, const double *v, double *x, hipStream_t s);
int amg_gs_pair(psk_prec *M, int set, int *on, int *eligible);
int ilu_check_error(const psk_prec *M, hipStream_t s);
int amg_apply(const psk_prec *M, const double *v, double *out, hipStream_t s);
void amg_free(AmgHierarchy *h);
struct AmgLoop {
    psk_csr *A;
    double *x, *r, *normb2, *sum;
    DevBuf *work;
};
int amg_loop_view(const psk_prec *M, AmgLoop *out);
int amg_loop_start(const psk_prec *M, const Context *c, const double *v, hipStream_t s);
int amg_cycle(const psk_prec *M, const Context *c, const double *v, hipStream_t s);
int amg_residual(const psk_prec *M, const double *v, hipStream_t s);
int dense_apply(const psk_prec *M, const double *v, double *out, hipStream_t s);
int dense_check_error(const psk_prec *M, hipStream_t s);
void dense_free(DenseInverse *d);
int cheby_apply(const psk_prec *M, const double *v, double *out, hipStream_t s);
void cheby_free(Chebyshev *ch);
int cheby_ab(const psk_prec *M, const double *v, int reps, double *fused_ms, double *pieces_ms);
inline bool prec_is_general(const psk_prec *M) {
    return M && (M->kind == PSK_PREC_ILU || M->kind == PSK_PREC_AMG || M->kind == PSK_PREC_DENSE ||
                 M->kind == PSK_PREC_CHEBYSHEV);
}
int prec_check_error(const psk_prec *M, hipStream_t s);
int tile_rows_for(int64_t n, int64_t nnz);
int csr_choose_layout(psk_csr *A, hipStream_t s);
void sliced_free(psk_csr *A);
int launch_spmv(const psk_csr *A, int mode, const double *x, double *y, const double *aux_d,
                const double *aux_q, double *partial, const int32_t *done_flag, hipStream_t s,
                hipEvent_t ev0 = nullptr, hipEvent_t ev1 = nullptr, int rev = 0, uint64_t *mail_seq = nullptr);

}
```

pysolvers_amd/csrc/spmv.hip:

```cpp
#include "psk_internal.hpp"
#include "pcg_state.hpp"

#include <hip/hip_ext.h>

#include <algorithm>
#include <atomic>
#include <climits>
#include <cstdlib>
#include <cmath>

namespace psk {

__device__ __forceinline__ int32_t ld_stream(const int32_t *p) { return __builtin_nontemporal_load(p); }
__device__ __forceinline__ double ld_stream(const double *p) { return __builtin_nontemporal_load(p); }

template <int MODE>
__device__ __forceinline__ bool spmv_publishes(const GridSum &gs) {
    return MODE != kSpmvPlain && MODE != kSpmvAdd && (MODE != kSpmvResid || gs.out != nullptr);
}
template <int MODE>
__device__ __forceinline__ uint32_t spmv_begin(const GridSum &gs, GridSumTile<1> &L, int64_t t) {
    return spmv_publishes<MODE>(gs) ? gridsum_tile_begin<1>(gs, L, t) : 0u;
}
__device__ __forceinline__ void spmv_publish(const GridSum &gs, GridSumTile<1> &L, double acc, uint32_t ticket,
// ... 355 lines not shown
        const int32_t *pword = spcol + tl[q] * (int64_t)((NP + NI) * kSlice) + tid;
#pragma unroll
        for (int p = 0; p < NP; ++p) cw[q][p] = (uint32_t)ld_stream(pword + p * kSlice);
        if (DK > 0) {
#pragma unroll
            for (int i = 0; i < NI; ++i) iw[q][i] = (uint32_t)ld_stream(pword + (NP + i) * kSlice);
            if (CMP) iw[q][0] = 0;
        } else {
            const double *v0 = sval + tl[q] * (int64_t)(UW * kSlice);
#pragma unroll
            for (int p = 0; p < UW / 2; ++p) {
                const dv2 v2 = __builtin_nontemporal_load(reinterpret_cast<const dv2 *>(v0 + 2 * p * kSlice) + tid);
                vv[q][2 * p] = v2.x;
                vv[q][2 * p + 1] = v2.y;
            }
            if (UW & 1) vv[q][UW - 1] = ld_stream(v0 + (UW - 1) * kSlice + tid);
        }
    }
    double eq[TPW];
#pragma unroll
    for (int q = 0; q < TPW; ++q) {
        const int64_t row = tl[q] * kSlice + tid;
        eq[q] = 0.0;
        if (MODE == kSpmvResid || MODE == kSpmvAdd || MODE == kSpmvJacobiDot || MODE == kSpmvPlainDot)
            eq[q] = aux_q[row < n ? row : 0];
    }
    const DictRegs dv = load_dict<DK>(sdict);
    if (dn != 0) {
#pragma unroll
        for (int q = 0; q < TPW; ++q) {
#pragma unroll
            for (int p = 0; p < NP; ++p) __asm__ volatile("" ::"v"(cw[q][p]));
            if (DK > 0) {
#pragma unroll
                for (int i = 0; i < NI; ++i) __asm__ volatile("" ::"v"(iw[q][i]));
            } else {
#pragma unroll
                for (int j = 0; j < UW; ++j) __asm__ volatile("" ::"v"(vv[q][j]));
            }
        }
        return;
    }
    constexpr bool PUB = MODE != kSpmvPlain && MODE != kSpmvAdd;
    __shared__ GridSumTile<1> gsl[TPW];
    uint32_t ticket[TPW];
    const bool pub = PUB && spmv_publishes<MODE>(gs);
    if (pub) {
        if (tid < TPW) gsl[tid].cnt = 0;
        if (tid == 0 && blockIdx.x == 0 && (gs.nt + TPW - 1) / TPW != gridDim.x) atomicOr(gs.err, 2);
        __syncthreads();
#pragma unroll
        for (int q = 0; q < TPW; ++q) {
            ticket[q] = 0;
            if (tv[q] && gs.grp_log2 >= 0 && tid == 0)
                ticket[q] = gridsum_draw(gridsum_counter(gs, gridsum_group_of(tl[q], gs.grp_log2)));
        }
    }
    int32_t cc[TPW][UW];
    double xv[TPW][UW], acc[TPW], yv[TPW];
#pragma unroll
    for (int q = 0; q < TPW; ++q) {
        const int32_t row32 = (int32_t)(tl[q] * kSlice + tid);
#pragma unroll
        for (int j = 0; j < UW; ++j) {
            cc[q][j] = unpack_delta(row32, (int16_t)((j & 1) ? (cw[q][j >> 1] >> 16) : (cw[q][j >> 1] & 0xffff)));
            const int32_t cl = cc[q][j] >= 0 ? cc[q][j] : 0;
            xv[q][j] = x[cl];
            if (MODE == kSpmvJacobiDot) xv[q][j] = aux_d[cl] * xv[q][j];
        }
    }
#pragma unroll
    for (int q = 0; q < TPW; ++q) {
        const int64_t row = tl[q] * kSlice + tid;
        const bool has = tv[q] && row < n;
        if (DK > 0) {
#pragma unroll
            for (int j = 0; j < UW; ++j)
                vv[q][j] = dict_pick<DK>(dv, CMP ? (cw[q][NP - 1] >> (16 + j)) & 1u : (iw[q][j >> 2] >> (8 * (j & 3))) & 0xff);
        }
        double sum = 0.0;
#pragma unroll
        for (int j = 0; j < UW; ++j)
            if (cc[q][j] >= 0) sum = sum + vv[q][j] * xv[q][j];
        if (MODE == kSpmvDot) eq[q] = diag_x<UW>(cc[q], xv[q], (int32_t)row, x, has);
        yv[q] = spmv_row_value<MODE>(has, sum, eq[q], acc[q]);
    }
    if (pub) spmv_publish_multi<TPW>(gs, gsl, acc, ticket, tl, tv);
#pragma unroll
    for (int q = 0; q < TPW; ++q) {
        const int64_t row = tl[q] * kSlice + tid;
        spmv_store_row<MODE>(tv[q] && row < n, row, yv[q], y);
    }
}

constexpr int kDiagMax = 8;
#ifndef PSK_DIAG_TPW
#define PSK_DIAG_TPW 2
#endif
constexpr int kDiagTpw = PSK_DIAG_TPW;
#ifndef PSK_DIAG_DPP
#define PSK_DIAG_DPP 1
#endif
constexpr bool kDiagDpp = PSK_DIAG_DPP != 0;
struct DiagDesc {
    int32_t d[kDiagMax];
    double v[kDiagMax];
    int64_t lo, hi;
    int64_t ncols;
    int32_t K, jd;
};

__device__ __forceinline__ int64_t diag_col(const DiagDesc &dd, int64_t n, int64_t row, int j) {
    int64_t c = row + dd.d[j];
    c += c < 0 ? dd.lo : (c >= n ? dd.hi : 0);
    return c < 0 ? 0 : (c >= dd.ncols ? dd.ncols - 1 : c);
}

__device__ __forceinline__ int32_t spmv_vzero() {
    int32_t z;
    __asm__ volatile("v_mov_b32 %0, 0" : "=v"(z));
    return z;
}

template <bool SHR>
__device__ __forceinline__ double wave_shift1(double v, double edge) {
    constexpr int ctrl = SHR ? 0x138 : 0x130;
    const int lo = __builtin_amdgcn_update_dpp(__double2loint(edge), __double2loint(v), ctrl, 0xF, 0xF, false);
    const int hi = __builtin_amdgcn_update_dpp(__double2hiint(edge), __double2hiint(v), ctrl, 0xF, 0xF, false);
    return __hiloint2double(hi, lo);
}

__device__ __forceinline__ int64_t diag_col_off(const DiagDesc &dd, int64_t n, int64_t row, int64_t off) {
    int64_t c = row + off;
    c += c < 0 ? dd.lo : (c >= n ? dd.hi : 0);
    return c < 0 ? 0 : (c >= dd.ncols ? dd.ncols - 1 : c);
}

template <int MODE, int KM, int TPW, int NB = 0>
__global__ __launch_bounds__(kBlock) void spmv_diag_kernel(
    int64_t n, const uint8_t *__restrict__ mask, DiagDesc dd, const double *__restrict__ x, double *__restrict__ y,
    const double *__restrict__ aux_d, const double *__restrict__ aux_q, GridSum gs, const int32_t *__restrict__ done,
    TileMap tm, int64_t ntiles) {
    constexpr int JD = NB == 1 ? 0 : NB == 2 ? 2 : -1, JM1 = NB == 1 ? 3 : NB == 2 ? 1 : -1,
                  JP1 = NB == 1 ? 4 : NB == 2 ? 3 : -1;
    static_assert(NB == 0 || KM == 5, "NB: the 5-diagonal patterns only");
    PSK_SPMV_PROF_AT(0);
    const int32_t dnv = (done ? done : &g_spmv_never_done)[spmv_vzero()];
    const int tid = threadIdx.x;
    const int64_t grp = tile_of_block(tm);
    int64_t tl[TPW];
    bool tv[TPW];
    uint32_t mk[TPW];
    double xv[TPW][KM], eq[TPW], xe[TPW];
#pragma unroll
    for (int q = 0; q < TPW; ++q) {
        const int64_t t = grp * TPW + q;
        tv[q] = t < ntiles;
        tl[q] = tv[q] ? t : ntiles - 1;
        mk[q] = __builtin_nontemporal_load(mask + tl[q] * kSlice + tid);
    }
#pragma unroll
    for (int q = 0; q < TPW; ++q) {
        const int64_t row = tl[q] * kSlice + tid;
#pragma unroll
        for (int j = 0; j < KM; ++j) {
            if (NB && (j == JM1 || j == JP1)) continue;
            const int64_t c = diag_col(dd, n, row, j);
            xv[q][j] = x[c];
            if (MODE == kSpmvJacobiDot) xv[q][j] = aux_d[c] * xv[q][j];
        }
        if (NB) {
            const int lane = tid & 63;
            const int64_t c = diag_col_off(dd, n, row, lane == 0 ? -1 : (lane == 63 ? 1 : 0));
            xe[q] = x[c];
            if (MODE == kSpmvJacobiDot) xe[q] = aux_d[c] * xe[q];
        }
        eq[q] = 0.0;
        if (MODE == kSpmvResid || MODE == kSpmvAdd || MODE == kSpmvJacobiDot || MODE == kSpmvPlainDot)
            eq[q] = aux_q[row < n ? row : 0];
    }
    constexpr bool PUB = MODE != kSpmvPlain && MODE != kSpmvAdd;
    const bool pub = PUB && spmv_publishes<MODE>(gs);
    uint32_t ticket[TPW];
#pragma unroll
    for (int q = 0; q < TPW; ++q) {
        ticket[q] = 0;
        if (pub && tv[q] && gs.grp_log2 >= 0 && tid == 0)
            ticket[q] = gridsum_draw(gridsum_counter(gs, gridsum_group_of(tl[q], gs.grp_log2)));
    }
    if (__builtin_amdgcn_readfirstlane(dnv) != 0) {
#pragma unroll
        for (int q = 0; q < TPW; ++q) {
            __asm__ volatile("" ::"v"(mk[q]));
            if (NB) __asm__ volatile("" ::"v"(xe[q]));
#pragma unroll
            for (int j = 0; j < KM; ++j)
                if (!(NB && (j == JM1 || j == JP1))) __asm__ volatile("" ::"v"(xv[q][j]));
            if (pub && tv[q] && gs.grp_log2 >= 0 && tid == 0)
                __hip_atomic_fetch_sub(gridsum_counter(gs, gridsum_group_of(tl[q], gs.grp_log2)), 1u, __ATOMIC_RELAXED,
                                       __HIP_MEMORY_SCOPE_AGENT);
        }
        return;
    }
    __shared__ GridSumTile<1> gsl[TPW];
    if (pub) {
        if (tid < TPW) gsl[tid].cnt = 0;
        if (tid == 0 && blockIdx.x == 0 && (gs.nt + TPW - 1) / TPW != gridDim.x) atomicOr(gs.err, 2);
        __syncthreads();
    }
    double acc[TPW], yv[TPW];
    if (NB) {
#pragma unroll
        for (int q = 0; q < TPW; ++q) {
            xv[q][JM1] = wave_shift1<true>(xv[q][JD], xe[q]);
            xv[q][JP1] = wave_shift1<false>(xv[q][JD], xe[q]);
        }
    }
#pragma unroll
    for (int q = 0; q < TPW; ++q) {
        const int64_t row = tl[q] * kSlice + tid;
        const bool has = tv[q] && row < n;
        double sum = 0.0;
#pragma unroll
        for (int j = 0; j < KM; ++j) {
            const double t = sum + dd.v[j] * xv[q][j];
            sum = ((mk[q] >> j) & 1u) ? t : sum;
        }
        if (MODE == kSpmvDot) {
            double d = 0.0;
            bool found = false;
#pragma unroll
            for (int j = 0; j < KM; ++j) {
                const bool here = j == dd.jd && ((mk[q] >> j) & 1u);
                d = here ? xv[q][j] : d;
                found = found || here;
            }
            if (!found && has) d = x[row];
            eq[q] = d;
        }
        yv[q] = spmv_row_value<MODE>(has, sum, eq[q], acc[q]);
    }
#ifdef PSK_SPMV_PROF
    if (threadIdx.x == 0) __asm__ volatile("" ::"v"(acc[0]));
#endif
    PSK_SPMV_PROF_AT(1);
    if (pub) spmv_publish_multi<TPW>(gs, gsl, acc, ticket, tl, tv);
#pragma unroll
    for (int q = 0; q < TPW; ++q) {
        const int64_t row = tl[q] * kSlice + tid;
        spmv_store_row<MODE>(tv[q] && row < n, row, yv[q], y);
    }
    PSK_SPMV_PROF_AT(2);
}


typedef double dv2u __attribute__((ext_vector_type(2), aligned(8)));
__device__ __forceinline__ dv2 ldu2(const double *p) {
    const dv2u v = *reinterpret_cast<const dv2u *>(p);
    return dv2{v.x, v.y};
}
__device__ __forceinline__ dv2 ldu2nt(const double *p) {
    const dv2u v = __builtin_nontemporal_load(reinterpret_cast<const dv2u *>(p));
    return dv2{v.x, v.y};
}
__device__ __forceinline__ void stu2(double *p, dv2 v) { *reinterpret_cast<dv2u *>(p) = dv2u{v.x, v.y}; }
__device__ __forceinline__ void stu2nt(double *p, dv2 v) {
    __builtin_nontemporal_store(dv2u{v.x, v.y}, reinterpret_cast<dv2u *>(p));
}

__device__ __forceinline__ double lane_f64(double x, int l) {
    return __hiloint2double(__builtin_amdgcn_readlane(__double2hiint(x), l),
                            __builtin_amdgcn_readlane(__double2loint(x), l));
}
__device__ __forceinline__ void diag_pair_totals(double v, double &t0, double &t1) {
    v += dpp_f64<0xB1>(v);
    v += dpp_f64<0x141>(v);
    v += dpp_f64<0x104>(v);
    t0 = ((lane_f64(v, 0) + lane_f64(v, 8)) + lane_f64(v, 16)) + lane_f64(v, 24);
    t1 = ((lane_f64(v, 32) + lane_f64(v, 40)) + lane_f64(v, 48)) + lane_f64(v, 56);
}

struct PairFix {
    int64_t c0, c1;
    bool bad;
};
__device__ __forceinline__ dv2 diag_pair_x(const DiagDesc &dd, int64_t n, int64_t r, int64_t d,
                                           const double *__restrict__ x, PairFix &f) {
    int64_t c0 = r + d, c1 = c0 + 1;
    c0 += c0 < 0 ? dd.lo : (c0 >= n ? dd.hi : 0);
    c1 += c1 < 0 ? dd.lo : (c1 >= n ? dd.hi : 0);
    f.bad = !(c1 == c0 + 1 && c0 >= 0 && c1 < dd.ncols);
    f.c0 = c0 < 0 ? 0 : (c0 >= dd.ncols ? dd.ncols - 1 : c0);
    f.c1 = c1 < 0 ? 0 : (c1 >= dd.ncols ? dd.ncols - 1 : c1);
    const int64_t a = c0 < 0 ? 0 : (c0 > dd.ncols - 2 ? dd.ncols - 2 : c0);
    return ldu2(x + a);
}
__device__ __forceinline__ void diag_pair_fix(dv2 &v, const PairFix &f, const double *__restrict__ x) {
    if (f.bad) {
        v.x = x[f.c0];
        v.y = x[f.c1];
    }
}

template <int MODE, int NB, int H>
__global__ __launch_bounds__(kBlock, (H == 2 && MODE != kSpmvPlain && MODE != kSpmvDot) ? 4 : 8) void spmv_diagp_kernel(
    int64_t n, const uint8_t *__restrict__ mask, DiagDesc dd, const double *__restrict__ x, double *__restrict__ y,
    const double *__restrict__ aux_d, const double *__restrict__ aux_q, GridSum gs, const int32_t *__restrict__ done,
    TileMap tm, int64_t ntiles) {
    constexpr int KM = 5;
    static_assert(NB == 1 || NB == 2, "the 5-diagonal DPP orders");
    static_assert(H == 1 || H == 2, "half-slices per wave");
    constexpr int JD = NB == 1 ? 0 : 2, JM1 = NB == 1 ? 3 : 1, JP1 = NB == 1 ? 4 : 3;
    constexpr int GD = NB == 1 ? 0 : 1;
    constexpr int TPB = H == 2 ? kWaves : kWaves / 2;
    constexpr bool JX = MODE == kSpmvJacobiDot;
    constexpr bool EQ = MODE == kSpmvResid || MODE == kSpmvAdd || MODE == kSpmvJacobiDot || MODE == kSpmvPlainDot;
    const int32_t dnv = (done ? done : &g_spmv_never_done)[spmv_vzero()];
    const int lane = threadIdx.x & 63;
    const int wave = __builtin_amdgcn_readfirstlane(threadIdx.x >> 6);
    const int64_t grp = tile_of_block(tm);
    const int64_t t = grp * TPB + (H == 2 ? wave : wave >> 1);
    const bool tv = t < ntiles;
    const int64_t tl = tv ? t : ntiles - 1;
    const int64_t r0 = tl * kSlice + (H == 2 ? 0 : 128 * (wave & 1));
    uint32_t mk[H];
    dv2 xv[H][3], dg[H][3], eq[H];
    PairFix fx[H][3];
    double xe, de = 1.0;
#pragma unroll
    for (int h = 0; h < H; ++h) {
        const int64_t row = r0 + 128 * h + 2 * lane;
        mk[h] = __builtin_nontemporal_load(reinterpret_cast<const uint16_t *>(mask + row));
    }
#pragma unroll
    for (int h = 0; h < H; ++h) {
        const int64_t row = r0 + 128 * h + 2 * lane;
        int g = 0;
#pragma unroll
        for (int j = 0; j < KM; ++j) {
            if (j == JM1 || j == JP1) continue;
            xv[h][g] = diag_pair_x(dd, n, row, dd.d[j], x, fx[h][g]);
            if (JX) dg[h][g] = diag_pair_x(dd, n, row, dd.d[j], aux_d, fx[h][g]);
            ++g;
        }
        eq[h] = dv2{0.0, 0.0};
        if (EQ) eq[h] = ldu2(aux_q + (row + 1 < n ? row : (n >= 2 ? n - 2 : 0)));
    }
    {
        const int64_t er = lane == 0 ? r0 - 1 : (lane == 63 ? r0 + 128 * H : r0 + 2 * lane);
        const int64_t c = diag_col_off(dd, n, er, 0);
        xe = x[c];
        if (JX) de = aux_d[c];
    }
    constexpr bool PUB = MODE != kSpmvPlain && MODE != kSpmvAdd;
    const bool pub = PUB && spmv_publishes<MODE>(gs);
    const bool drawer = H == 2 || (wave & 1) == 0;
    uint32_t ticket = 0;
    if (pub && tv && drawer && gs.grp_log2 >= 0 && lane == 0)
        ticket = gridsum_draw(gridsum_counter(gs, gridsum_group_of(tl, gs.grp_log2)));
    if (__builtin_amdgcn_readfirstlane(dnv) != 0) {
#pragma unroll
        for (int h = 0; h < H; ++h) {
            __asm__ volatile("" ::"v"(mk[h]));
#pragma unroll
            for (int g = 0; g < 3; ++g) {
                __asm__ volatile("" ::"v"(xv[h][g].x), "v"(xv[h][g].y));
                if (JX) __asm__ volatile("" ::"v"(dg[h][g].x), "v"(dg[h][g].y));
            }
            if (EQ) __asm__ volatile("" ::"v"(eq[h].x), "v"(eq[h].y));
        }
        __asm__ volatile("" ::"v"(xe), "v"(de));
        if (pub && tv && drawer && gs.grp_log2 >= 0 && lane == 0)
            __hip_atomic_fetch_sub(gridsum_counter(gs, gridsum_group_of(tl, gs.grp_log2)), 1u, __ATOMIC_RELAXED,
                                   __HIP_MEMORY_SCOPE_AGENT);
        return;
    }
    __shared__ GridSumTile<1> gsl[H == 1 ? TPB : 1];
    if (H == 1 && pub) {
        if (threadIdx.x < TPB) gsl[threadIdx.x].cnt = 0;
        __syncthreads();
    }
    if (pub && threadIdx.x == 0 && blockIdx.x == 0 && (gs.nt + TPB - 1) / TPB != gridDim.x) atomicOr(gs.err, 2);
#pragma unroll
    for (int h = 0; h < H; ++h)
#pragma unroll
        for (int g = 0; g < 3; ++g) {
            diag_pair_fix(xv[h][g], fx[h][g], x);
            if (JX) {
                diag_pair_fix(dg[h][g], fx[h][g], aux_d);
                xv[h][g].x = dg[h][g].x * xv[h][g].x;
                xv[h][g].y = dg[h][g].y * xv[h][g].y;
            }
        }
    if (JX) xe = de * xe;
    double xl[H], xr[H];
    if constexpr (H == 2) {
        const double a63 = lane_f64(xv[0][GD].y, 63), b0 = lane_f64(xv[1][GD].x, 0);
        xl[0] = wave_shift1<true>(xv[0][GD].y, xe);
        xr[0] = wave_shift1<false>(xv[0][GD].x, b0);
        xl[1] = wave_shift1<true>(xv[1][GD].y, a63);
        xr[1] = wave_shift1<false>(xv[1][GD].x, xe);
    } else {
        xl[0] = wave_shift1<true>(xv[0][GD].y, xe);
        xr[0] = wave_shift1<false>(xv[0][GD].x, xe);
    }
    double acc[H];
    dv2 yv[H];
#pragma unroll
    for (int h = 0; h < H; ++h) {
        const int64_t row = r0 + 128 * h + 2 * lane;
        double c0[KM], c1[KM];
        int g = 0;
#pragma unroll
        for (int j = 0; j < KM; ++j) {
            if (j == JM1) {
                c0[j] = xl[h];
                c1[j] = xv[h][GD].x;
            } else if (j == JP1) {
                c0[j] = xv[h][GD].y;
                c1[j] = xr[h];
            } else {
                c0[j] = xv[h][g].x;
                c1[j] = xv[h][g].y;
                ++g;
            }
        }
        const uint32_t m0 = mk[h] & 0xffu, m1 = mk[h] >> 8;
        double s0 = 0.0, s1 = 0.0;
#pragma unroll
        for (int j = 0; j < KM; ++j) {
            const double u0 = s0 + dd.v[j] * c0[j], u1 = s1 + dd.v[j] * c1[j];
            s0 = ((m0 >> j) & 1u) ? u0 : s0;
            s1 = ((m1 >> j) & 1u) ? u1 : s1;
        }
        const bool has0 = tv && row < n, has1 = tv && row + 1 < n;
        double e0 = eq[h].x, e1 = eq[h].y;
        if (EQ && row + 1 >= n) {
            e0 = eq[h].y;
            e1 = 0.0;
        }
        if (MODE == kSpmvDot) {
            const bool f0 = (m0 >> JD) & 1u, f1 = (m1 >> JD) & 1u;
            e0 = f0 ? c0[JD] : 0.0;
            e1 = f1 ? c1[JD] : 0.0;
            if (!f0 && has0) e0 = x[row];
            if (!f1 && has1) e1 = x[row + 1];
        }
        double a0, a1;
        yv[h].x = spmv_row_value<MODE>(has0, s0, e0, a0);
        yv[h].y = spmv_row_value<MODE>(has1, s1, e1, a1);
        acc[h] = a0 + a1;
    }
    if (pub && tv) {
        double w[2 * H];
#pragma unroll
        for (int h = 0; h < H; ++h) diag_pair_totals(acc[h], w[2 * h], w[2 * h + 1]);
        bool reduce = false;
        uint32_t tk = 0;
        double s = 0.0;
        if (H == 2) {
            s = ((w[0] + w[1]) + w[2]) + w[3];
            tk = __builtin_amdgcn_readfirstlane(ticket);
            reduce = true;
        } else {
            GridSumTile<1> &L = gsl[wave >> 1];
            const int hb = wave & 1;
            uint32_t old = 0;
            if (lane == 0) {
                L.part[2 * hb] = w[0];
                L.part[2 * hb + 1] = w[1];
                if (hb == 0) L.ticket = ticket;
                __builtin_amdgcn_fence(__ATOMIC_RELEASE, "workgroup", "local");
                old = atomicAdd(&L.cnt, 1u);
            }
            if (__builtin_amdgcn_readfirstlane(old) == 1) {
                __builtin_amdgcn_fence(__ATOMIC_ACQUIRE, "workgroup", "local");
                s = ((L.part[0] + L.part[1]) + L.part[2]) + L.part[3];
                tk = L.ticket;
                reduce = true;
            }
        }
        if (reduce) {
            if (gs.grp_log2 < 0) {
                if (lane == 0) gridsum_put(gs.gslots + tl, s);
                gridsum_final_wave<1>(gs);
            } else {
                if (lane == 0) gridsum_put(gs.slots + gridsum_slot(gs, tl), s);
                const int64_t g = gridsum_group_of(tl, gs.grp_log2);
                int64_t base;
                const int64_t cnt = gridsum_members(gs, g, base);
                if (tk == (uint32_t)(cnt - 1)) {
                    double r[1];
                    gridsum_take<1, 64>(gs.slots, g << gs.grp_log2, cnt, gs.err, nullptr, r);
                    if (lane == 0) {
                        gridsum_reset(gridsum_counter(gs, g));
                        gridsum_put(gs.gslots + g, r[0]);
                    }
                    gridsum_final_wave<1>(gs);
                }
            }
        }
    }
#pragma unroll
    for (int h = 0; h < H; ++h) {
        const int64_t row = r0 + 128 * h + 2 * lane;
        if (!tv || row >= n) continue;
        if (row + 1 < n) {
            if (MODE == kSpmvResid || MODE == kSpmvAdd) stu2(y + row, yv[h]);
            else stu2nt(y + row, yv[h]);
        } else {
            spmv_store_row<MODE>(true, row, yv[h].x, y);
        }
    }
}

template <int NB>
__global__ __launch_bounds__(kBlock) void pcg_init_diag_kernel(int64_t n, const uint8_t *__restrict__ mask, DiagDesc dd,
                                                               const double *__restrict__ b, double xs,
                                                               double *__restrict__ p, double *__restrict__ y,
                                                               GridSum gs, PcgInitFin fin, TileMap tm, int64_t ntiles) {
    constexpr int TPW = kDiagTpw, KM = 5;
    static_assert(NB == 1 || NB == 2, "the DPP orders of spmv_diag_kernel");
    constexpr int JD = NB == 1 ? 0 : 2, JM1 = NB == 1 ? 3 : 1, JP1 = NB == 1 ? 4 : 3;
    const int tid = threadIdx.x, lane = tid & 63;
    const int64_t grp = tile_of_block(tm);
    int64_t tl[TPW];
    bool tv[TPW];
    uint32_t mk[TPW];
    double xv[TPW][KM], xe[TPW];
#pragma unroll
    for (int q = 0; q < TPW; ++q) {
        const int64_t t = grp * TPW + q;
        tv[q] = t < ntiles;
        tl[q] = tv[q] ? t : ntiles - 1;
        mk[q] = __builtin_nontemporal_load(mask + tl[q] * kSlice + tid);
    }
#pragma unroll
    for (int q = 0; q < TPW; ++q) {
        const int64_t row = tl[q] * kSlice + tid;
#pragma unroll
        for (int j = 0; j < KM; ++j) {
            if (j == JM1 || j == JP1) continue;
            xv[q][j] = b[diag_col(dd, n, row, j)];
        }
        xe[q] = b[diag_col_off(dd, n, row, lane == 0 ? -1 : (lane == 63 ? 1 : 0))];
    }
    uint32_t ticket[TPW];
#pragma unroll
    for (int q = 0; q < TPW; ++q) {
        ticket[q] = 0;
        if (tv[q] && gs.grp_log2 >= 0 && tid == 0)
            ticket[q] = gridsum_draw(gridsum_counter(gs, gridsum_group_of(tl[q], gs.grp_log2)));
    }
    __shared__ GridSumTile<3> gsl[TPW];
    if (tid < TPW) gsl[tid].cnt = 0;
    if (tid == 0 && blockIdx.x == 0 && (gs.nt + TPW - 1) / TPW != gridDim.x) atomicOr(gs.err, 2);
    __syncthreads();
    double acc[TPW][3], yv[TPW], pv[TPW];
#pragma unroll
    for (int q = 0; q < TPW; ++q) {
        const int64_t row = tl[q] * kSlice + tid;
        const bool has = tv[q] && row < n;
        const double braw = xv[q][JD];
#pragma unroll
        for (int j = 0; j < KM; ++j)
            if (j != JM1 && j != JP1) xv[q][j] = xs * xv[q][j];
        xe[q] = xs * xe[q];
        xv[q][JM1] = wave_shift1<true>(xv[q][JD], xe[q]);
        xv[q][JP1] = wave_shift1<false>(xv[q][JD], xe[q]);
        double sum = 0.0;
#pragma unroll
        for (int j = 0; j < KM; ++j) {
            const double t = sum + dd.v[j] * xv[q][j];
            sum = ((mk[q] >> j) & 1u) ? t : sum;
        }
        pv[q] = xv[q][JD];
        yv[q] = sum;
        acc[q][0] = has ? pv[q] * sum : 0.0;
        acc[q][1] = has ? braw * braw : 0.0;
        acc[q][2] = has ? pv[q] * braw : 0.0;
    }
    gridsum_tiles_publish<TPW, 3>(gs, gsl, acc, ticket, tl, tv, fin);
#pragma unroll
    for (int q = 0; q < TPW; ++q) {
        const int64_t row = tl[q] * kSlice + tid;
        if (tv[q] && row < n) {
            __builtin_nontemporal_store(yv[q], y + row);
            p[row] = pv[q];
        }
    }
}



__global__ __launch_bounds__(kBlock) void diag_detect_kernel(int64_t n, const int32_t *__restrict__ rowptr,
                                                             const int32_t *__restrict__ colidx,
                                                             const double *__restrict__ vals, DiagDesc dd,
                                                             uint8_t *__restrict__ mask, int64_t npad,
                                                             int32_t *__restrict__ bad) {
    const int64_t row = (int64_t)blockIdx.x * kBlock + threadIdx.x;
    if (row >= npad) return;
    uint32_t mk = 0;
    if (row < n) {
        int j = 0;
        bool ok = true;
        for (int32_t e = rowptr[row]; e < rowptr[row + 1] && ok; ++e) {
            const int64_t c = colidx[e];
            const double v = vals[e];
            while (j < dd.K) {
                int64_t cj = row + dd.d[j];
                cj += cj < 0 ? dd.lo : (cj >= n ? dd.hi : 0);
                if (cj == c && same_bits(v, dd.v[j])) break;
                ++j;
            }
            if (j == dd.K) ok = false;
            else mk |= 1u << j++;
        }
        if (!ok) atomicOr(bad, 1);
    }
    mask[row] = (uint8_t)mk;
}

template <int MODE, int DK>
__global__ __launch_bounds__(kBlock) void spmv_sliced_kernel(
    int64_t n, const int64_t *__restrict__ soff, const int64_t *__restrict__ swoff, const int8_t *__restrict__ sfmt,
    const int32_t *__restrict__ scol, const int32_t *__restrict__ spcol, const double *__restrict__ sval,
    const double *__restrict__ sdict,
    const double *__restrict__ x, double *__restrict__ y, const double *__restrict__ aux_d,
    const double *__restrict__ aux_q, GridSum gs, const int32_t *__restrict__ done, TileMap tm) {
    if (done != nullptr && *done != 0) return;
    const int tid = threadIdx.x;
    const int64_t t = tile_of_block(tm), row = t * kSlice + tid;
    const bool has = row < n;
    const int64_t o = soff[t];
    const int w = (int)((soff[t + 1] - o) / kSlice);
    const bool packed = sfmt[t] != 0;
    const int64_t wo = swoff[t];
    const int32_t *pword = spcol + wo;
    const int32_t *vword = pword + (packed ? (int64_t)((w + 1) / 2) * kSlice : 0);
    const DictRegs dv = load_dict<DK>(sdict);
    __shared__ GridSumTile<1> gsl;
    const uint32_t ticket = spmv_begin<MODE>(gs, gsl, t);
    const int32_t row32 = (int32_t)row;
    double eq = 0.0;
    if (has) {
        if (MODE == kSpmvDot && w > kSliceRegs) eq = x[row];
        if (MODE == kSpmvResid || MODE == kSpmvAdd || MODE == kSpmvJacobiDot || MODE == kSpmvPlainDot)
            eq = aux_q[row];
    }
    double sum = 0.0;
    if (w <= kSliceRegs) {
        int32_t cc[kSliceRegs];
        double vv[kSliceRegs], xv[kSliceRegs];
#pragma unroll
        for (int j = 0; j < kSliceRegs; ++j) {
            cc[j] = -1;
            vv[j] = 0.0;
        }
        int32_t vw[kSliceRegs / 4];
        if (DK > 0) {
#pragma unroll
            for (int q = 0; q < kSliceRegs / 4; ++q) vw[q] = 4 * q < w ? ld_stream(vword + q * kSlice + tid) : 0;
        } else {
#pragma unroll
            for (int p = 0; p < kSliceRegs / 2; ++p) {
                if (2 * p + 1 < w) {
                    const dv2 v2 =
                        __builtin_nontemporal_load(reinterpret_cast<const dv2 *>(sval + o + 2 * p * kSlice) + tid);
                    vv[2 * p] = v2.x;
                    vv[2 * p + 1] = v2.y;
                } else if (2 * p < w) {
                    vv[2 * p] = ld_stream(sval + o + 2 * p * kSlice + tid);
                }
            }
        }
        if (packed) {
#pragma unroll
            for (int p = 0; p < kSliceRegs / 2; ++p)
                if (2 * p < w) {
                    const int32_t word = ld_stream(pword + p * kSlice + tid);
                    cc[2 * p] = unpack_delta(row32, (int16_t)(word & 0xffff));
                    cc[2 * p + 1] = unpack_delta(row32, (int16_t)(word >> 16));
                }
        } else {
#pragma unroll
// ... 157 lines not shown
void sliced_free(psk_csr *A) {
    void *ptrs[] = {A->sl_off, A->sl_woff, A->sl_fmt, A->sl_col, A->sl_pcol, A->sl_val, A->sl_dict};
    for (void *p : ptrs)
        if (p) (void)hipFree(p);
    A->sl_off = nullptr;
    A->sl_woff = nullptr;
    A->sl_fmt = nullptr;
    A->sl_col = nullptr;
    A->sl_pcol = nullptr;
    A->sl_val = nullptr;
    A->sl_dict = nullptr;
    A->sl_dict_n = 0;
    A->sl_uniform_w = 0;
    A->sl_compact = 0;
    A->sl_slots = 0;
    A->sl_packed_slots = 0;
    A->sl_stream_bytes = 0;
}

void diag_free(psk_csr *A) {
    if (A->dg_mask) (void)hipFree(A->dg_mask);
    A->dg_mask = nullptr;
    A->dg_K = 0;
    A->dg_jd = -1;
}

static DiagDesc diag_desc(const psk_csr *A) {
    DiagDesc dd{};
    for (int j = 0; j < kDiagMax; ++j) {
        dd.d[j] = A->dg_d[j];
        dd.v[j] = A->dg_v[j];
    }
    dd.lo = A->dg_lo;
    dd.hi = A->dg_hi;
    dd.ncols = A->ncols;
    dd.K = A->dg_K;
    dd.jd = A->dg_jd;
    return dd;
}

static int diag_build(psk_csr *A, hipStream_t s, bool force) {
    auto no = [&](const char *why) { return force ? fail(PSK_ERR_UNSUPPORTED, std::string("diagonal layout: ") + why) : PSK_OK; };
    const int64_t n = A->n, nt = (n + kSlice - 1) / kSlice;
    if (n == 0 || A->nnz == 0) return no("empty matrix");
    if (nt > INT32_MAX) return no("too many slices");
    DevBuf tmp;
    struct Release {
        DevBuf &b;
        ~Release() { b.release(); }
    } rel{tmp};
    PSK_TRY(tmp.ensure((size_t)nt * 2 * sizeof(int32_t) + 64));
    int32_t *dw = tmp.as<int32_t>(), *dspan = dw + nt;
    int32_t *dbad = dw + 2 * nt;
    hipLaunchKernelGGL(sliced_shape_kernel, dim3((unsigned)nt), dim3(kBlock), 0, s, n, A->rowptr, A->colidx, dw, dspan);
    PSK_HIP(hipGetLastError());
    std::vector<int32_t> wd((size_t)nt);
    PSK_HIP(hipMemcpyAsync(wd.data(), dw, (size_t)nt * sizeof(int32_t), hipMemcpyDeviceToHost, s));
    PSK_HIP(hipStreamSynchronize(s));
    const int32_t K = *std::max_element(wd.begin(), wd.end());
    if (K < 1 || K > kDiagMax) return no("rows wider than 8 entries");
    std::vector<int32_t> rp(kSlice + 1), cols(K);
    std::vector<double> vals(K);
    int64_t trow = -1;
    for (int64_t tries = 0, i = 0; i < nt && tries < 64 && trow < 0; ++i) {
        const int64_t t = (nt / 2 + i) % nt;
        if (wd[(size_t)t] != K) continue;
        ++tries;
        const int64_t r0 = t * kSlice, nr = std::min<int64_t>(kSlice, n - r0);
        PSK_HIP(hipMemcpy(rp.data(), A->rowptr + r0, (size_t)(nr + 1) * sizeof(int32_t), hipMemcpyDeviceToHost));
        for (int64_t r = 0; r < nr && trow < 0; ++r) {
            if (rp[(size_t)r + 1] - rp[(size_t)r] != K) continue;
            PSK_HIP(hipMemcpy(cols.data(), A->colidx + rp[(size_t)r], (size_t)K * 4, hipMemcpyDeviceToHost));
            bool owned = true;
            for (int j = 0; j < K; ++j) owned = owned && cols[(size_t)j] >= 0 && cols[(size_t)j] < n;
            if (!owned) continue;
            PSK_HIP(hipMemcpy(vals.data(), A->vals + rp[(size_t)r], (size_t)K * 8, hipMemcpyDeviceToHost));
            trow = r0 + r;
        }
    }
    if (trow < 0) return no("no full-width row of owned columns");
    DiagDesc dd{};
    dd.K = K;
    dd.jd = -1;
    int64_t dmin = 0;
    for (int j = 0; j < K; ++j) {
        const int64_t d = (int64_t)cols[(size_t)j] - trow;
        for (int i = 0; i < j; ++i)
            if (dd.d[i] == d) return no("repeated column in a row");
        dd.d[j] = (int32_t)d;
        dd.v[j] = vals[(size_t)j];
        if (d == 0) dd.jd = j;
        dmin = std::min(dmin, d);
    }
    const int64_t halo = A->ncols - n;
    dd.lo = halo > 0 ? n - dmin : 0;
    dd.hi = halo > 0 && halo == -2 * dmin ? -dmin : 0;
    dd.ncols = A->ncols;
    uint8_t *mask = nullptr;
    if (hipMalloc(&mask, (size_t)nt * kSlice) != hipSuccess) {
        (void)hipGetLastError();
        return force ? fail(PSK_ERR_ALLOC, "diagonal layout: hipMalloc") : PSK_OK;
    }
    PSK_HIP(hipMemsetAsync(dbad, 0, sizeof(int32_t), s));
    hipLaunchKernelGGL(diag_detect_kernel, dim3((unsigned)nt), dim3(kBlock), 0, s, n, A->rowptr, A->colidx, A->vals, dd,
                       mask, nt * kSlice, dbad);
    int32_t bad = 0;
    hipError_t e = hipGetLastError();
    if (e == hipSuccess) e = hipMemcpyAsync(&bad, dbad, sizeof(int32_t), hipMemcpyDeviceToHost, s);
    if (e == hipSuccess) e = hipStreamSynchronize(s);
    if (e != hipSuccess || bad) {
        (void)hipFree(mask);
        if (e != hipSuccess) return fail(PSK_ERR_HIP, std::string("diagonal layout: ") + hipGetErrorString(e));
        return no("an entry off the diagonals or with another value");
    }
    sliced_free(A);
    diag_free(A);
    A->dg_mask = mask;
    A->dg_K = K;
    A->dg_jd = dd.jd;
    for (int j = 0; j < kDiagMax; ++j) {
        A->dg_d[j] = j < K ? dd.d[j] : 0;
        A->dg_v[j] = j < K ? dd.v[j] : 0.0;
    }
    A->dg_lo = dd.lo;
    A->dg_hi = dd.hi;
    return PSK_OK;
}

static int find_value_dict(const psk_csr *A, hipStream_t s, std::vector<double> &dict) {
    dict.clear();
    if (A->nnz == 0) return PSK_OK;
    DevBuf tmp;
    struct Release {
        DevBuf &b;
        ~Release() { b.release(); }
    } rel{tmp};
    PSK_TRY(tmp.ensure((size_t)(kDictMax + kDictCand + 1) * sizeof(double)));
    double *ddict = tmp.as<double>(), *dcand = ddict + kDictMax;
    int32_t *dn = reinterpret_cast<int32_t *>(dcand + kDictCand);
    const int64_t blocks = std::min<int64_t>((A->nnz + kBlock - 1) / kBlock, 2048);
    std::vector<double> cand(kDictCand);
    for (int pass = 0; pass <= kDictMax; ++pass) {
        if (!dict.empty())
            PSK_HIP(hipMemcpyAsync(ddict, dict.data(), dict.size() * sizeof(double), hipMemcpyHostToDevice, s));
        PSK_HIP(hipMemsetAsync(dn, 0, sizeof(int32_t), s));
        hipLaunchKernelGGL(dict_scan_kernel, dim3((unsigned)blocks), dim3(kBlock), 0, s, A->nnz, A->vals, ddict,
                           (int)dict.size(), dn, dcand);
        PSK_HIP(hipGetLastError());
        int32_t nc = 0;
        PSK_HIP(hipMemcpyAsync(&nc, dn, sizeof(int32_t), hipMemcpyDeviceToHost, s));
        PSK_HIP(hipMemcpyAsync(cand.data(), dcand, kDictCand * sizeof(double), hipMemcpyDeviceToHost, s));
        PSK_HIP(hipStreamSynchronize(s));
        if (nc == 0) return PSK_OK;
        for (int i = 0; i < std::min(nc, kDictCand); ++i) {
            bool seen = false;
            for (double d : dict) seen = seen || std::memcmp(&d, &cand[(size_t)i], sizeof(double)) == 0;
            if (!seen) dict.push_back(cand[(size_t)i]);
            if ((int)dict.size() > kDictMax) {
                dict.clear();
                return PSK_OK;
            }
        }
    }
    dict.clear();
    return PSK_OK;
}

static int sliced_build(psk_csr *A, hipStream_t s, bool force, bool pack, bool use_dict, bool force_dict) {
    sliced_free(A);
    diag_free(A);
    std::vector<double> dict;
    if (use_dict) PSK_TRY(find_value_dict(A, s, dict));
    if (force_dict && dict.empty())
        return fail(PSK_ERR_UNSUPPORTED, "sliced layout: more than 8 distinct values, no value dictionary");
    const int64_t nt = (A->n + kSlice - 1) / kSlice;
    if (nt == 0) return PSK_OK;
    if (nt > INT32_MAX) return force ? fail(PSK_ERR_UNSUPPORTED, "sliced layout: too many slices") : PSK_OK;
    DevBuf tmp;
    struct Release {
        DevBuf &b;
        ~Release() { b.release(); }
    } rel{tmp};
    PSK_TRY(tmp.ensure((size_t)nt * 2 * sizeof(int32_t)));
    int32_t *dw = tmp.as<int32_t>(), *dspan = dw + nt;
    hipLaunchKernelGGL(sliced_shape_kernel, dim3((unsigned)nt), dim3(kBlock), 0, s, A->n, A->rowptr, A->colidx, dw,
                       dspan);
    PSK_HIP(hipGetLastError());
    std::vector<int32_t> wd((size_t)nt * 2);
    PSK_HIP(hipMemcpyAsync(wd.data(), tmp.p, (size_t)nt * 2 * sizeof(int32_t), hipMemcpyDeviceToHost, s));
    PSK_HIP(hipStreamSynchronize(s));
    int64_t wmax = 0, wsum = 0;
    bool all_pack = pack;
    for (int64_t t = 0; t < nt; ++t) {
        wmax = std::max<int64_t>(wmax, wd[(size_t)t]);
        wsum += wd[(size_t)t];
        all_pack = all_pack && wd[(size_t)(nt + t)] <= kMaxDelta16;
    }
    const bool uniform = all_pack && wmax > 0 && wmax <= kSliceRegs && wmax * nt * 100 <= wsum * 101;
    if (uniform)
        for (int64_t t = 0; t < nt; ++t) wd[(size_t)t] = (int32_t)wmax;
    const bool compact = uniform && !dict.empty() && dict.size() <= 2 && (wmax & 1) && wmax <= 15;
    std::vector<int64_t> off((size_t)nt + 1), woff((size_t)nt + 1);
    std::vector<int8_t> fmt((size_t)nt);
    off[0] = 0;
    woff[0] = 0;
    int64_t packed_slots = 0, col_bytes = 0, val_bytes = 0;
    for (int64_t t = 0; t < nt; ++t) {
        const int64_t w = wd[(size_t)t];
        off[(size_t)t + 1] = off[(size_t)t] + w * kSlice;
        fmt[(size_t)t] = (pack && wd[(size_t)(nt + t)] <= kMaxDelta16) ? 1 : 0;
        if (fmt[(size_t)t]) packed_slots += w * kSlice;
        col_bytes += (fmt[(size_t)t] ? 4 * ((w + 1) / 2) : 4 * w) * kSlice;
        val_bytes += (dict.empty() ? 8 * w : compact ? 0 : 4 * ((w + 3) / 4)) * kSlice;
        const int64_t words = (fmt[(size_t)t] ? (w + 1) / 2 : 0) + (dict.empty() || compact ? 0 : (w + 3) / 4);
        woff[(size_t)t + 1] = woff[(size_t)t] + words * kSlice;
    }
    const int64_t slots = off[(size_t)nt], nwords = woff[(size_t)nt];
    const int64_t wide_slots = slots - packed_slots;
    const int64_t stream = val_bytes + 8 * (int64_t)dict.size() + col_bytes + (uniform ? 0 : 17 * nt + 16);
    if (!force && stream > 12 * A->nnz + 4 * (A->n + 1)) return PSK_OK;
    const size_t ms = slots > 0 ? (size_t)slots : 1;
    bool ok = hipMalloc(&A->sl_off, (size_t)(nt + 1) * 8) == hipSuccess &&
              hipMalloc(&A->sl_woff, (size_t)(nt + 1) * 8) == hipSuccess &&
              hipMalloc(&A->sl_fmt, (size_t)nt) == hipSuccess;
    if (ok && dict.empty()) ok = hipMalloc(&A->sl_val, ms * 8) == hipSuccess;
    if (ok && wide_slots > 0) ok = hipMalloc(&A->sl_col, ms * 4) == hipSuccess;
    if (ok && nwords > 0) ok = hipMalloc(&A->sl_pcol, (size_t)nwords * 4) == hipSuccess;
    if (ok && !dict.empty()) ok = hipMalloc(&A->sl_dict, kDictMax * 8) == hipSuccess;
    if (!ok) {
        (void)hipGetLastError();
        sliced_free(A);
        return force ? fail(PSK_ERR_ALLOC, "sliced layout: hipMalloc") : PSK_OK;
    }
    PSK_HIP(hipMemcpyAsync(A->sl_off, off.data(), (size_t)(nt + 1) * 8, hipMemcpyHostToDevice, s));
    PSK_HIP(hipMemcpyAsync(A->sl_woff, woff.data(), (size_t)(nt + 1) * 8, hipMemcpyHostToDevice, s));
    PSK_HIP(hipMemcpyAsync(A->sl_fmt, fmt.data(), (size_t)nt, hipMemcpyHostToDevice, s));
    if (!dict.empty()) {
        std::vector<double> padded(dict);
        padded.resize(kDictMax, 0.0);
        PSK_HIP(hipMemcpyAsync(A->sl_dict, padded.data(), kDictMax * 8, hipMemcpyHostToDevice, s));
    }
    A->sl_dict_n = (int32_t)dict.size();
    A->sl_uniform_w = uniform ? (int32_t)wmax : 0;
    A->sl_compact = compact ? 1 : 0;
    hipLaunchKernelGGL(sliced_fill_kernel, dim3((unsigned)nt), dim3(kBlock), 0, s, A->n, A->rowptr, A->colidx, A->vals,
                       A->sl_off, A->sl_woff, A->sl_fmt, A->sl_col, A->sl_pcol, A->sl_val, A->sl_dict,
                       A->sl_dict_n, compact ? 1 : 0);
    PSK_HIP(hipGetLastError());
    PSK_HIP(hipStreamSynchronize(s));
    A->sl_slots = slots;
    A->sl_packed_slots = packed_slots;
    A->sl_stream_bytes = stream;
    (void)wide_slots;
    return PSK_OK;
}

int csr_choose_layout(psk_csr *A, hipStream_t s) {
    const char *e = std::getenv("PSK_SPMV_LAYOUT");
    if (e && std::strcmp(e, "csr") == 0) return PSK_OK;
    const char *de = std::getenv("PSK_SPMV_DIAG");
    const bool diag_env = e && std::strcmp(e, "diag") == 0;
    if ((!e || diag_env) && !(de && std::atoi(de) == 0)) {
        PSK_TRY(diag_build(A, s, false));
        if (A->dg_mask) return PSK_OK;
    }
    if (diag_env) e = nullptr;
    const bool wide = e && std::strcmp(e, "sliced_wide") == 0;
    const bool plain = e && std::strcmp(e, "sliced") == 0;
    const bool force = e && (plain || wide || std::strcmp(e, "sliced_dict") == 0);
    int rc = sliced_build(A, s, force, !wide, !wide && !plain, false);
    if (rc != PSK_OK) sliced_free(A);
    return rc;
}

int tile_rows_for(int64_t n, int64_t nnz) {
    const double avg = n > 0 ? (double)nnz / (double)n : 1.0;
    int r = kBlock;
    while (r > 32 && avg * r > kChunk) r >>= 1;
    return r;
}

__global__ void spmv_empty_dot_kernel(GridSum gs, const int32_t *done) {
    if (threadIdx.x != 0 || (done && *done)) return;
    const double z[1] = {0.0};
    gs.out[0] = 0.0;
    gridsum_mail<1>(gs, z);
}

static bool spmv_xcd_bands() { return true; }

#ifndef PSK_CSR_CHUNK
#define PSK_CSR_CHUNK 128
#endif
static int64_t spmv_csr_chunk() { return PSK_CSR_CHUNK; }

#ifndef PSK_DIAG_PAIR
#define PSK_DIAG_PAIR 2
#endif
static int diag_pair_h() { return PSK_DIAG_PAIR; }
static int spmv_tpw() { return 2; }

static int64_t spmv_tiles(const psk_csr *A) { return (A->n + A->tile_rows - 1) / A->tile_rows; }

int launch_spmv(const psk_csr *A, int mode, const double *x, double *y, const double *aux_d,
                const double *aux_q, double *partial, const int32_t *done_flag, hipStream_t s, hipEvent_t ev0,
                hipEvent_t ev1, int rev, uint64_t *mail_seq) {
    Context *c;
    PSK_TRY(ctx(&c));
    const bool sliced = A->sl_off != nullptr || A->dg_mask != nullptr;
    const int64_t nwg = sliced ? (A->n + kSlice - 1) / kSlice : spmv_tiles(A);
    GridSum gs{nullptr, nullptr, nullptr, nullptr, 0, 0, -1, nullptr, nullptr, 0, 0};
    if (partial && nwg > 0) PSK_TRY(gridsum_prepare(c, nwg, 1, partial, &gs));
    if (partial && nwg == 0) gs.out = partial;
    if (mail_seq) {
        if (!partial || !A->comm || !A->comm->mb) return fail(PSK_ERR_ARG, "launch_spmv: mailbox without a dot");
        *mail_seq = mbox_next(A->comm, &gs);
    }
    if (A->n == 0) {
        if (partial) {
            hipLaunchKernelGGL(spmv_empty_dot_kernel, dim3(1), dim3(64), 0, s, gs, done_flag);
            PSK_HIP(hipGetLastError());
        }
        return PSK_OK;
    }
    dim3 gd((unsigned)nwg), bd(kBlock);
    TileMap tm = tile_map_for(nwg, sliced && spmv_xcd_bands(), rev != 0);
    if (!sliced && spmv_csr_chunk() > 0) tm = tile_map_chunked(nwg, spmv_csr_chunk());
    const int tpw = spmv_tpw();
    const int64_t nwg2 = (nwg + tpw - 1) / tpw;
    const dim3 gd2((unsigned)(nwg2 > 0 ? nwg2 : 1));
    const TileMap tm2 = tile_map_for(nwg2, sliced && spmv_xcd_bands(), rev != 0);
    if (A->dg_mask) {
        const DiagDesc dd = diag_desc(A);
        const int km = A->dg_K <= 3 ? 3 : A->dg_K <= 5 ? 5 : 8;
        const int64_t nwgd = (nwg + kDiagTpw - 1) / kDiagTpw;
        const dim3 gdd((unsigned)(nwgd > 0 ? nwgd : 1));
        const TileMap tmd = tile_map_for(nwgd, spmv_xcd_bands(), rev != 0);
        const int nbk = !kDiagDpp || A->dg_K != 5 ? 0
                        : (A->dg_d[0] == 0 && A->dg_d[3] == -1 && A->dg_d[4] == 1) ? 1
                        : (A->dg_d[2] == 0 && A->dg_d[1] == -1 && A->dg_d[3] == 1) ? 2 : 0;
        const int pairh = (nbk != 0 && A->n >= 2 && dd.ncols >= 2) ? diag_pair_h() : 0;
        const int64_t nwgp = pairh ? (nwg + (pairh == 2 ? 4 : 2) - 1) / (pairh == 2 ? 4 : 2) : 1;
        const dim3 gdp((unsigned)nwgp);
        const TileMap tmp = tile_map_for(nwgp, spmv_xcd_bands(), rev != 0);
#define PSK_DIAGP(M, NB, H)                                                                                        \
    hipExtLaunchKernelGGL((spmv_diagp_kernel<M, NB, H>), gdp, bd, 0, s, ev0, ev1, 0, A->n, A->dg_mask, dd, x, y, aux_d, \
                          aux_q, gs, done_flag, tmp, nwg)
#define PSK_DIAG_LAUNCH(M, KM)                                                                                     \
    do {                                                                                                           \
        if (KM == 5 && pairh == 2 && nbk == 1) PSK_DIAGP(M, 1, 2);                                                 \
        else if (KM == 5 && pairh == 2 && nbk == 2) PSK_DIAGP(M, 2, 2);                                            \
        else if (KM == 5 && pairh == 1 && nbk == 1) PSK_DIAGP(M, 1, 1);                                            \
        else if (KM == 5 && pairh == 1 && nbk == 2) PSK_DIAGP(M, 2, 1);                                            \
        else if (KM == 5 && nbk == 1)                                                                              \
            hipExtLaunchKernelGGL((spmv_diag_kernel<M, 5, kDiagTpw, 1>), gdd, bd, 0, s, ev0, ev1, 0, A->n, A->dg_mask, \
                                  dd, x, y, aux_d, aux_q, gs, done_flag, tmd, nwg);                                 \
        else if (KM == 5 && nbk == 2)                                                                              \
            hipExtLaunchKernelGGL((spmv_diag_kernel<M, 5, kDiagTpw, 2>), gdd, bd, 0, s, ev0, ev1, 0, A->n, A->dg_mask, \
                                  dd, x, y, aux_d, aux_q, gs, done_flag, tmd, nwg);                                 \
        else                                                                                                       \
            hipExtLaunchKernelGGL((spmv_diag_kernel<M, KM, kDiagTpw>), gdd, bd, 0, s, ev0, ev1, 0, A->n, A->dg_mask, dd, \
                                  x, y, aux_d, aux_q, gs, done_flag, tmd, nwg);                                     \
    } while (0)
#define PSK_DIAG_MODE(M)                                                                                           \
    do {                                                                                                           \
        if (km == 3) PSK_DIAG_LAUNCH(M, 3);                                                                        \
        else if (km == 5) PSK_DIAG_LAUNCH(M, 5);                                                                   \
        else PSK_DIAG_LAUNCH(M, 8);                                                                                \
    } while (0)
        switch (mode) {
        case kSpmvPlain: PSK_DIAG_MODE(kSpmvPlain); break;
        case kSpmvDot: PSK_DIAG_MODE(kSpmvDot); break;
        case kSpmvJacobiDot: PSK_DIAG_MODE(kSpmvJacobiDot); break;
        case kSpmvPlainDot: PSK_DIAG_MODE(kSpmvPlainDot); break;
        case kSpmvResid: PSK_DIAG_MODE(kSpmvResid); break;
        case kSpmvAdd: PSK_DIAG_MODE(kSpmvAdd); break;
        default:
            return fail(PSK_ERR_ARG, "unknown spmv mode");
        }
#undef PSK_DIAG_MODE
#undef PSK_DIAG_LAUNCH
#undef PSK_DIAGP
        PSK_HIP(hipGetLastError());
        return PSK_OK;
    }
    if (sliced) {
        const int dk = !A->sl_dict ? 0 : A->sl_dict_n <= 2 ? 2 : A->sl_dict_n <= 4 ? 4 : 8;
        const int uw = A->sl_uniform_w;
#define PSK_UNI_LAUNCH(M, DK, UW)                                                                              \
    hipExtLaunchKernelGGL((spmv_uniform_kernel<M, DK, UW>), gd, bd, 0, s, ev0, ev1, 0, A->n, A->sl_pcol, A->sl_val, A->sl_dict, \
                       x, y, aux_d, aux_q, gs, done_flag, tm)
#define PSK_SLICED_LAUNCH_DK(M, DK)                                                                            \
    do {                                                                                                       \
        switch (uw) {                                                                                          \
        case 0:                                                                                                \
            hipExtLaunchKernelGGL((spmv_sliced_kernel<M, DK>), gd, bd, 0, s, ev0, ev1, 0, A->n, A->sl_off, A->sl_woff,         \
                               A->sl_fmt, A->sl_col, A->sl_pcol, A->sl_val, A->sl_dict, x, y, aux_d, aux_q, gs, \
                               done_flag, tm);                                                                     \
            break;                                                                                             \
        case 1: PSK_UNI_LAUNCH(M, DK, 1); break;                                                               \
        case 2: PSK_UNI_LAUNCH(M, DK, 2); break;                                                               \
        case 3: PSK_UNI_LAUNCH(M, DK, 3); break;                                                               \
        case 4: PSK_UNI_LAUNCH(M, DK, 4); break;                                                               \
        case 5: PSK_UNI_LAUNCH(M, DK, 5); break;                                                               \
        case 6: PSK_UNI_LAUNCH(M, DK, 6); break;                                                               \
        case 7: PSK_UNI_LAUNCH(M, DK, 7); break;                                                               \
        default: PSK_UNI_LAUNCH(M, DK, 8); break;                                                              \
        }                                                                                                      \
    } while (0)
#define PSK_UNI_LAUNCH_C(M, UW)                                                                                \
    do {                                                                                                       \
        if (tpw == 2)                                                                                          \
            hipExtLaunchKernelGGL((spmv_uniform_multi_kernel<M, 2, UW, true, 2>), gd2, bd, 0, s, ev0, ev1, 0, A->n,   \
                                  A->sl_pcol, A->sl_val, A->sl_dict, x, y, aux_d, aux_q, gs, done_flag, tm2, nwg);  \
        else if (tpw == 3)                                                                                     \
            hipExtLaunchKernelGGL((spmv_uniform_multi_kernel<M, 2, UW, true, 3>), gd2, bd, 0, s, ev0, ev1, 0, A->n,   \
                                  A->sl_pcol, A->sl_val, A->sl_dict, x, y, aux_d, aux_q, gs, done_flag, tm2, nwg);  \
        else if (tpw == 4)                                                                                     \
            hipExtLaunchKernelGGL((spmv_uniform_multi_kernel<M, 2, UW, true, 4>), gd2, bd, 0, s, ev0, ev1, 0, A->n,   \
                                  A->sl_pcol, A->sl_val, A->sl_dict, x, y, aux_d, aux_q, gs, done_flag, tm2, nwg);  \
        else                                                                                                   \
            hipExtLaunchKernelGGL((spmv_uniform_kernel<M, 2, UW, true>), gd, bd, 0, s, ev0, ev1, 0, A->n, A->sl_pcol,  \
                                  A->sl_val, A->sl_dict, x, y, aux_d, aux_q, gs, done_flag, tm);                 \
    } while (0)
#define PSK_SLICED_LAUNCH(M)                                                                                   \
    do {                                                                                                       \
        if (A->sl_compact) {                                       \
            if (uw == 1) PSK_UNI_LAUNCH_C(M, 1);                                                               \
            else if (uw == 3) PSK_UNI_LAUNCH_C(M, 3);                                                          \
            else if (uw == 5) PSK_UNI_LAUNCH_C(M, 5);                                                          \
            else PSK_UNI_LAUNCH_C(M, 7);                                                                       \
        } else if (dk == 0) PSK_SLICED_LAUNCH_DK(M, 0);                                                        \
        else if (dk == 2) PSK_SLICED_LAUNCH_DK(M, 2);                                                          \
        else if (dk == 4) PSK_SLICED_LAUNCH_DK(M, 4);                                                          \
        else PSK_SLICED_LAUNCH_DK(M, 8);                                                                       \
    } while (0)
        switch (mode) {
        case kSpmvPlain: PSK_SLICED_LAUNCH(kSpmvPlain); break;
        case kSpmvDot: PSK_SLICED_LAUNCH(kSpmvDot); break;
        case kSpmvJacobiDot: PSK_SLICED_LAUNCH(kSpmvJacobiDot); break;
        case kSpmvPlainDot: PSK_SLICED_LAUNCH(kSpmvPlainDot); break;
        case kSpmvResid: PSK_SLICED_LAUNCH(kSpmvResid); break;
        case kSpmvAdd: PSK_SLICED_LAUNCH(kSpmvAdd); break;
        default:
            return fail(PSK_ERR_ARG, "unknown spmv mode");
        }
#undef PSK_SLICED_LAUNCH
#undef PSK_SLICED_LAUNCH_DK
#undef PSK_UNI_LAUNCH
#undef PSK_UNI_LAUNCH_C
        PSK_HIP(hipGetLastError());
        return PSK_OK;
    }
    const int tr = A->tile_rows;
    const int32_t nz = (int32_t)A->nnz;
#define PSK_SPMV_LAUNCH(M)                                                                                  \
    hipExtLaunchKernelGGL(spmv_kernel<M>, gd, bd, 0, s, ev0, ev1, 0, A->n, tr, A->rowptr, A->colidx, A->vals, x, y, aux_d, \
                       aux_q, gs, done_flag, nz, tm)
    switch (mode) {
    case kSpmvPlain: PSK_SPMV_LAUNCH(kSpmvPlain); break;
    case kSpmvDot: PSK_SPMV_LAUNCH(kSpmvDot); break;
    case kSpmvJacobiDot: PSK_SPMV_LAUNCH(kSpmvJacobiDot); break;
    case kSpmvPlainDot: PSK_SPMV_LAUNCH(kSpmvPlainDot); break;
    case kSpmvResid: PSK_SPMV_LAUNCH(kSpmvResid); break;
    case kSpmvAdd: PSK_SPMV_LAUNCH(kSpmvAdd); break;
    default:
        return fail(PSK_ERR_ARG, "unknown spmv mode");
    }
#undef PSK_SPMV_LAUNCH
    PSK_HIP(hipGetLastError());
    return PSK_OK;
}

static int diag_nb(const psk_csr *A) {
    if (!kDiagDpp || !A->dg_mask || A->dg_K != 5) return 0;
    if (A->dg_d[0] == 0 && A->dg_d[3] == -1 && A->dg_d[4] == 1) return 1;
    if (A->dg_d[2] == 0 && A->dg_d[1] == -1 && A->dg_d[3] == 1) return 2;
    return 0;
}

bool pcg_init_diag_eligible(const psk_csr *A) { return !A->comm && A->n > 0 && diag_nb(A) != 0; }

int launch_pcg_init_diag(const psk_csr *A, const double *b, double xs, double *p, double *Ap, double *out3,
                         const PcgInitFin &fin, hipStream_t s) {
    if (!pcg_init_diag_eligible(A)) return fail(PSK_ERR_ARG, "launch_pcg_init_diag: not eligible");
    Context *c;
    PSK_TRY(ctx(&c));
    const int64_t nwg = (A->n + kSlice - 1) / kSlice, nwgd = (nwg + kDiagTpw - 1) / kDiagTpw;
    GridSum gs;
    PSK_TRY(gridsum_prepare(c, nwg, 3, out3, &gs));
    const DiagDesc dd = diag_desc(A);
    const TileMap tmd = tile_map_for(nwgd, spmv_xcd_bands());
    if (diag_nb(A) == 1)
        hipLaunchKernelGGL(pcg_init_diag_kernel<1>, dim3((unsigned)nwgd), dim3(kBlock), 0, s, A->n, A->dg_mask, dd, b, xs,
                           p, Ap, gs, fin, tmd, nwg);
    else
        hipLaunchKernelGGL(pcg_init_diag_kernel<2>, dim3((unsigned)nwgd), dim3(kBlock), 0, s, A->n, A->dg_mask, dd, b, xs,
                           p, Ap, gs, fin, tmd, nwg);
    PSK_HIP(hipGetLastError());
    return PSK_OK;
}

__device__ __forceinline__ int64_t fd_rowptr(int64_t m, int64_t k) {
    int64_t mk = k < m ? k : m;
    int64_t top = k - m * (m - 1);
    if (top < 0) top = 0;
    return 5 * k - mk - top - (k + m - 1) / m - k / m;
}

__global__ void fd2d_kernel(int64_t m, int64_t row_begin, int64_t row_end, double dval, double oval,
                            int32_t *rowptr, int32_t *colidx, double *vals, int64_t halo_lo_start,
                            int64_t n_own) {
    const int64_t i = (int64_t)blockIdx.x * blockDim.x + threadIdx.x;
    const int64_t nloc = row_end - row_begin;
    if (i > nloc) return;
    const int64_t k = row_begin + i;
    const int64_t base = fd_rowptr(m, row_begin);
    const int64_t off = fd_rowptr(m, k) - base;
    rowptr[i] = (int32_t)off;
    if (i == nloc) return;
    const int64_t ix = k % m, iy = k / m;
    auto lc = [&](int64_t c) -> int32_t {
        if (c >= row_begin && c < row_end) return (int32_t)(c - row_begin);
        if (c < row_begin) return (int32_t)(n_own + (c - halo_lo_start));
        return (int32_t)(n_own + (row_begin - halo_lo_start) + (c - row_end));
    };
    int64_t p = off;
    colidx[p] = lc(k);
    vals[p++] = dval;
    if (iy > 0) { colidx[p] = lc(k - m); vals[p++] = oval; }
    if (iy < m - 1) { colidx[p] = lc(k + m); vals[p++] = oval; }
    if (ix > 0) { colidx[p] = lc(k - 1); vals[p++] = oval; }
    if (ix < m - 1) { colidx[p] = lc(k + 1); vals[p++] = oval; }
}

int fd2d_fill(psk_csr *A, int64_t m, double a, double b, int64_t row_begin, int64_t row_end,
              int64_t halo_lo_start, hipStream_t s) {
    const double h = std::fabs(b - a) / (double)(m + 1);
    const double dval = -4.0 / h / h;
    const double oval = 1.0 / h / h;
    const int64_t nloc = row_end - row_begin;
    const int64_t threads = nloc + 1;
    const int64_t blocks = (threads + kBlock - 1) / kBlock;
    hipLaunchKernelGGL(fd2d_kernel, dim3((unsigned)blocks), dim3(kBlock), 0, s, m, row_begin, row_end,
                       dval, oval, A->rowptr, A->colidx, A->vals, halo_lo_start, nloc);
    PSK_HIP(hipGetLastError());
    return PSK_OK;
}

__global__ void jacobi_dinv_kernel(int64_t n, const int32_t *rowptr, const int32_t *colidx,
                                   const double *vals, double *dinv) {
    const int64_t i = (int64_t)blockIdx.x * blockDim.x + threadIdx.x;
    if (i >= n) return;
    double d = 0.0;
    for (int32_t jj = rowptr[i]; jj < rowptr[i + 1]; ++jj)
        if (colidx[jj] == (int32_t)i) d = d + vals[jj];
    dinv[i] = 1.0 / d;
}

__global__ __launch_bounds__(kBlock) void dot_partial_kernel(int64_t n, const double *__restrict__ x,
                                                             const double *__restrict__ y,
                                                             double *__restrict__ part) {
    __shared__ double sh[kWaves];
    int64_t t0, t1;
    const int64_t ntiles = (n + kVecTile - 1) / kVecTile;
    block_range(ntiles, t0, t1);
    const int64_t i0 = t0 * kVecTile, i1 = (t1 * kVecTile < n) ? t1 * kVecTile : n;
    double acc = 0.0;
    for (int64_t i = i0 + threadIdx.x; i < i1; i += kBlock) acc = fma(x[i], y[i], acc);
    const double s = block_sum(acc, sh);
    if (threadIdx.x == 0) part[blockIdx.x] = s;
}

__global__ __launch_bounds__(kBlock) void reduce_final_kernel(const double *part, int np, double *out,
                                                              int do_sqrt) {
    __shared__ double sh[kWaves];
    const double s = reduce_partials(part, np, 1, sh);
    if (threadIdx.x == 0) out[0] = do_sqrt ? sqrt(s) : s;
}

__global__ void axpy_kernel(int64_t n, double alpha, const double *__restrict__ x, double *__restrict__ y) {
    const int64_t i = (int64_t)blockIdx.x * blockDim.x + threadIdx.x;
    if (i < n) y[i] = y[i] + alpha * x[i];
}

__global__ void scale_kernel(int64_t n, const double *__restrict__ d, const double *__restrict__ v,
                             double *__restrict__ out) {
    const int64_t i = (int64_t)blockIdx.x * blockDim.x + threadIdx.x;
    if (i < n) out[i] = d[i] * v[i];
}

int prec_apply_dev(const psk_prec *M, int64_t n, const double *v, double *out, hipStream_t s) {
    if (n == 0) return PSK_OK;
    if (!M || M->kind == PSK_PREC_IDENTITY) {
        PSK_HIP(hipMemcpyAsync(out, v, (size_t)n * 8, hipMemcpyDeviceToDevice, s));
        return PSK_OK;
    }
    if (M->kind == PSK_PREC_JACOBI) {
        hipLaunchKernelGGL(scale_kernel, dim3((unsigned)((n + kBlock - 1) / kBlock)), dim3(kBlock), 0, s, n,
                           M->dinv, v, out);
        PSK_HIP(hipGetLastError());
        return PSK_OK;
    }
    if (M->kind == PSK_PREC_ILU) return ilu_apply(M, v, out, s);
    if (M->kind == PSK_PREC_AMG) return amg_apply(M, v, out, s);
    if (M->kind == PSK_PREC_DENSE) return dense_apply(M, v, out, s);
    if (M->kind == PSK_PREC_CHEBYSHEV) return cheby_apply(M, v, out, s);
    return fail(PSK_ERR_UNSUPPORTED, "unknown preconditioner kind");
}

}

using namespace psk;

static int csr_alloc(psk_csr *A, int64_t n, int64_t nnz) {
    hipError_t e;
    e = hipMalloc(&A->rowptr, (size_t)(n + 1) * sizeof(int32_t));
    if (e != hipSuccess) return fail(PSK_ERR_ALLOC, "hipMalloc rowptr");
    {
        const size_t m = nnz > 0 ? (size_t)nnz : 1;
        e = hipMalloc(&A->colidx, m * sizeof(int32_t));
        if (e != hipSuccess) return fail(PSK_ERR_ALLOC, "hipMalloc colidx");
        e = hipMalloc(&A->vals, m * sizeof(double));
        if (e != hipSuccess) return fail(PSK_ERR_ALLOC, "hipMalloc vals");
        if (nnz == 0) {
            e = hipMemset(A->colidx, 0, sizeof(int32_t));
            if (e == hipSuccess) e = hipMemset(A->vals, 0, sizeof(double));
            if (e != hipSuccess) return fail(PSK_ERR_HIP, "hipMemset dummy entry");
        }
    }
    return PSK_OK;
}

static void csr_free(psk_csr *A) {
    if (A->rowptr) (void)hipFree(A->rowptr);
    if (A->colidx) (void)hipFree(A->colidx);
    if (A->vals) (void)hipFree(A->vals);
    A->rowptr = nullptr;
    A->colidx = nullptr;
    A->vals = nullptr;
    sliced_free(A);
    diag_free(A);
    A->ws.release();
    A->ws_small.release();
    A->sendbuf.release();
    if (A->pack_idx) (void)hipFree(A->pack_idx);
    A->pack_idx = nullptr;
    A->pack_count = 0;
    A->peers.clear();
}

extern "C" {

int psk_csr_create(int64_t n, int64_t nnz, const int32_t *rowptr, const int32_t *colidx,
                   const double *vals, int32_t loc, psk_csr **out) {
    return psk_csr_create_rect(n, n, nnz, rowptr, colidx, vals, loc, out);
}

int psk_csr_create_rect(int64_t n, int64_t ncols, int64_t nnz, const int32_t *rowptr, const int32_t *colidx,
                        const double *vals, int32_t loc, psk_csr **out) {
    if (!out || n < 0 || ncols < 0 || nnz < 0 || !rowptr || (nnz > 0 && (!colidx || !vals)))
        return fail(PSK_ERR_ARG, "psk_csr_create: bad arguments");
    if (nnz > kMaxNnz || n >= INT32_MAX || ncols >= INT32_MAX)
        return fail(PSK_ERR_UNSUPPORTED, "psk_csr_create: int32 CSR indices required (nnz < 2^31 - 1536)");
    if (loc == PSK_HOST) {
        if (rowptr[0] != 0 || rowptr[n] != nnz)
            return fail(PSK_ERR_ARG, "psk_csr_create: rowptr[0] must be 0 and rowptr[n] == nnz");
        for (int64_t i = 0; i < n; ++i)
            if (rowptr[i + 1] < rowptr[i]) return fail(PSK_ERR_ARG, "psk_csr_create: rowptr not monotone");
        for (int64_t j = 0; j < nnz; ++j)
            if (colidx[j] < 0 || colidx[j] >= ncols) return fail(PSK_ERR_ARG, "psk_csr_create: column index out of range");
    }
    Context *c;
    PSK_TRY(ctx(&c));
    psk_csr *A = new psk_csr();
    A->n = n;
    A->ncols = ncols;
    A->nnz = nnz;
    A->tile_rows = tile_rows_for(n, nnz);
    A->n_global = n;
    A->row_begin = 0;
    A->row_end = n;
    A->device = c->device;
    int rc = csr_alloc(A, n, nnz);
    if (rc != PSK_OK) {
        csr_free(A);
        delete A;
        return rc;
    }
    const hipMemcpyKind k = loc == PSK_HOST ? hipMemcpyHostToDevice : hipMemcpyDeviceToDevice;
    hipError_t e = hipMemcpyAsync(A->rowptr, rowptr, (size_t)(n + 1) * sizeof(int32_t), k, c->stream);
    if (e == hipSuccess && nnz > 0)
        e = hipMemcpyAsync(A->colidx, colidx, (size_t)nnz * sizeof(int32_t), k, c->stream);
    if (e == hipSuccess && nnz > 0)
        e = hipMemcpyAsync(A->vals, vals, (size_t)nnz * sizeof(double), k, c->stream);
    if (e == hipSuccess) e = hipStreamSynchronize(c->stream);
    if (e != hipSuccess) {
        csr_free(A);
        delete A;
        return fail(PSK_ERR_HIP, std::string("psk_csr_create copy: ") + hipGetErrorString(e));
    }
    rc = csr_choose_layout(A, c->stream);
    if (rc != PSK_OK) {
        csr_free(A);
        delete A;
        return rc;
    }
    *out = A;
    return PSK_OK;
}

int psk_csr_create_fd2d(double a, double b, int64_t m, psk_csr **out) {
    if (!out || m < 1) return fail(PSK_ERR_ARG, "psk_csr_create_fd2d: m must be >= 1");
    const int64_t n = m * m;
    const int64_t nnz = (m == 1) ? 1 : 5 * n - 4 * m;
    if (nnz > kMaxNnz) return fail(PSK_ERR_UNSUPPORTED, "FD2D: nnz exceeds int32 CSR");
    Context *c;
    PSK_TRY(ctx(&c));
    psk_csr *A = new psk_csr();
    A->n = n;
    A->ncols = n;
    A->nnz = nnz;
    A->tile_rows = tile_rows_for(n, nnz);
    A->n_global = n;
    A->row_end = n;
    A->device = c->device;
    int rc = csr_alloc(A, n, nnz);
    if (rc == PSK_OK) rc = fd2d_fill(A, m, a, b, 0, n, 0, c->stream);
    if (rc == PSK_OK) {
        hipError_t e = hipStreamSynchronize(c->stream);
        if (e != hipSuccess) rc = fail(PSK_ERR_HIP, std::string("fd2d: ") + hipGetErrorString(e));
    }
    if (rc == PSK_OK) rc = csr_choose_layout(A, c->stream);
    if (rc != PSK_OK) {
        csr_free(A);
        delete A;
        return rc;
    }
    *out = A;
    return PSK_OK;
}

int psk_csr_info(const psk_csr *A, int64_t *n, int64_t *nnz) {
    if (!A) return fail(PSK_ERR_ARG, "NULL matrix");
    if (n) *n = A->n;
    if (nnz) *nnz = A->nnz;
    return PSK_OK;
}

int psk_csr_layout(psk_csr *A, int32_t set, int32_t *layout, int64_t *slots, int64_t *packed_slots,
                   int64_t *stream_bytes) {
    if (!A) return fail(PSK_ERR_ARG, "psk_csr_layout: NULL matrix");
    if (set != -1 && set != PSK_LAYOUT_CSR && set != PSK_LAYOUT_SLICED && set != PSK_LAYOUT_SLICED_WIDE &&
        set != PSK_LAYOUT_SLICED_DICT && set != PSK_LAYOUT_DIAG)
        return fail(PSK_ERR_ARG, "psk_csr_layout: set must be -1 or a PSK_LAYOUT_* value");
    if (set != -1) {
        Context *c;
        PSK_TRY(ctx(&c));
        PSK_HIP(hipStreamSynchronize(c->stream));
        if (set == PSK_LAYOUT_CSR) {
            sliced_free(A);
            diag_free(A);
        } else if (set == PSK_LAYOUT_DIAG) {
            PSK_TRY(diag_build(A, c->stream, true));
        } else {
            PSK_TRY(sliced_build(A, c->stream, true, set != PSK_LAYOUT_SLICED_WIDE, set == PSK_LAYOUT_SLICED_DICT,
                                 set == PSK_LAYOUT_SLICED_DICT));
        }
    }
    if (layout)
        *layout = A->dg_mask                  ? PSK_LAYOUT_DIAG
                  : !A->sl_off                ? PSK_LAYOUT_CSR
                  : A->sl_dict                ? PSK_LAYOUT_SLICED_DICT
                  : A->sl_packed_slots == 0   ? PSK_LAYOUT_SLICED_WIDE
                                              : PSK_LAYOUT_SLICED;
    if (slots) *slots = A->dg_mask ? A->n * A->dg_K : A->sl_slots;
    if (packed_slots) *packed_slots = A->dg_mask ? 0 : A->sl_packed_slots;
    if (stream_bytes)
        *stream_bytes = A->dg_mask ? A->n : A->sl_off ? A->sl_stream_bytes : 12 * A->nnz + 4 * (A->n + 1);
    return PSK_OK;
}

int psk_csr_download(const psk_csr *A, int32_t *rowptr, int32_t *colidx, double *vals) {
    if (!A) return fail(PSK_ERR_ARG, "NULL matrix");
// ... 251 lines not shown
```

Measured before the change: 7098.

## Stagger deferred x-update flush across vector blocks, fused into SpMV launch

Replaces the periodic whole-vector x catch-up (every kPcgDefer iterations in the direction kernel) with a staggered scheme. The vector is split into S blocks, and each PCG iteration flushes one block's pending x updates. The flush runs as extra workgroups interleaved inside the diagonal-pair SpMV dot launch, so the catch-up traffic is spread evenly and overlaps the SpMV rather than causing a periodic bandwidth spike in the direction kernel. It adds grid-interleaving arithmetic, an extra template instantiation and more complex end-of-solve flush logic, plus lab hooks for testing.

```diff
diff --git a/include/psk_lab.h b/include/psk_lab.h
--- a/include/psk_lab.h
+++ b/include/psk_lab.h
@@ -21,6 +21,11 @@
 int psk_lab_spmv_after_write(const psk_csr *A, double *x, double *y, const double *src, double *scratch,
                              int32_t target, int32_t reps, int32_t dot, double *avg_ms);
 int psk_lab_cheby_ab(const psk_prec *M, const double *v, int32_t reps, double *fused_ms, double *pieces_ms);
+int psk_lab_pcg_stagger(int32_t *blocks, int32_t *ring);
+int psk_lab_pcg_staggers(const psk_csr *A, const psk_prec *M, int32_t *on);
+int psk_lab_pcg_flush_schedule(int32_t S, int64_t nv, int64_t tile, int64_t k, int32_t in_spmv, int32_t *blk,
+                               int64_t *first_last);
+int psk_lab_pcg_flush(int64_t n, int64_t k, int32_t stag, double *x, const double *ring, const double *alphas);
 #ifdef __cplusplus
 }
 #endif
diff --git a/pysolvers_amd/_native.py b/pysolvers_amd/_native.py
--- a/pysolvers_amd/_native.py
+++ b/pysolvers_amd/_native.py
@@ -118,6 +118,10 @@
     "psk_lab_spmv_rotate": (ctypes.c_int, [P, ctypes.POINTER(P), ctypes.POINTER(P), I32, I32, I32, ctypes.POINTER(F64)]),
     "psk_lab_cheby_ab": (ctypes.c_int, [P, P, I32, ctypes.POINTER(F64), ctypes.POINTER(F64)]),
     "psk_lab_spmv_after_write": (ctypes.c_int, [P, P, P, P, P, I32, I32, I32, ctypes.POINTER(F64)]),
+    "psk_lab_pcg_stagger": (ctypes.c_int, [ctypes.POINTER(I32), ctypes.POINTER(I32)]),
+    "psk_lab_pcg_staggers": (ctypes.c_int, [P, P, ctypes.POINTER(I32)]),
+    "psk_lab_pcg_flush_schedule": (ctypes.c_int, [I32, I64, I64, I64, I32, ctypes.POINTER(I32), ctypes.POINTER(I64)]),
+    "psk_lab_pcg_flush": (ctypes.c_int, [I64, I64, I32, P, P, P]),
 }
 _lab = None
 
diff --git a/pysolvers_amd/csrc/lab.hip b/pysolvers_amd/csrc/lab.hip
--- a/pysolvers_amd/csrc/lab.hip
+++ b/pysolvers_amd/csrc/lab.hip
@@ -1,4 +1,5 @@
 #include "trisolve.hpp"
+#include "pcg_state.hpp"
 #include "../../include/psk_lab.h"
 
 #include <chrono>
@@ -263,3 +264,56 @@
     if (rc == PSK_OK) *avg_ms = tot / reps;
     return rc;
 }
+
+extern "C" int psk_lab_pcg_stagger(int32_t *blocks, int32_t *ring) {
+    if (blocks) *blocks = psk::kPcgStagger;
+    if (ring) *ring = psk::kPcgDefer;
+    return PSK_OK;
+}
+
+extern "C" int psk_lab_pcg_staggers(const psk_csr *A, const psk_prec *M, int32_t *on) {
+    if (!A || !on) return psk::fail(PSK_ERR_ARG, "psk_lab_pcg_staggers: NULL argument");
+    *on = psk::pcg_staggers(A, M) ? 1 : 0;
+    return PSK_OK;
+}
+
+extern "C" int psk_lab_pcg_flush_schedule(int32_t S, int64_t nv, int64_t tile, int64_t k, int32_t in_spmv,
+                                          int32_t *blk, int64_t *first_last) {
+    using namespace psk;
+    if (S < 1 || nv < 1 || tile < 0 || tile >= nv || k < 0 || !blk || !first_last)
+        return fail(PSK_ERR_ARG, "psk_lab_pcg_flush_schedule: bad arguments");
+    *blk = pcg_block_of_tile(tile, nv, S);
+    const PcgPend pd = pcg_flush_pending(S, *blk, k, in_spmv != 0);
+    first_last[0] = pd.first;
+    first_last[1] = pd.last;
+    return PSK_OK;
+}
+
+extern "C" int psk_lab_pcg_flush(int64_t n, int64_t k, int32_t stag, double *x, const double *ring,
+                                 const double *alphas) {
+    using namespace psk;
+    if (n < 1 || k < 1 || !x || !ring || !alphas) return fail(PSK_ERR_ARG, "psk_lab_pcg_flush: bad arguments");
+    if (stag && kPcgStagger == 0) return fail(PSK_ERR_UNSUPPORTED, "psk_lab_pcg_flush: built without the staggered flush");
+    Context *c;
+    PSK_TRY(ctx(&c));
+    const size_t vec = ((size_t)n * 8 + 255) / 256 * 256, al = ((size_t)k * 8 + 255) / 256 * 256;
+    DevBuf buf;
+    PSK_TRY(buf.ensure((kPcgDefer + 1) * vec + al));
+    char *d = buf.as<char>();
+    double *dx = reinterpret_cast<double *>(d), *da = reinterpret_cast<double *>(d + (kPcgDefer + 1) * vec);
+    PRing pr;
+    for (int t = 0; t < kPcgDefer; ++t) pr.b[t] = reinterpret_cast<double *>(d + (size_t)(t + 1) * vec);
+    int rc = PSK_OK;
+    if (hipMemcpyAsync(dx, x, (size_t)n * 8, hipMemcpyHostToDevice, c->stream) != hipSuccess ||
+        hipMemcpyAsync(da, alphas, (size_t)k * 8, hipMemcpyHostToDevice, c->stream) != hipSuccess)
+        rc = fail(PSK_ERR_HIP, "psk_lab_pcg_flush: copy");
+    for (int t = 0; t < kPcgDefer && rc == PSK_OK; ++t)
+        if (hipMemcpyAsync(pr.b[t], ring + (size_t)t * (size_t)n, (size_t)n * 8, hipMemcpyHostToDevice, c->stream) != hipSuccess)
+            rc = fail(PSK_ERR_HIP, "psk_lab_pcg_flush: copy");
+    if (rc == PSK_OK) rc = launch_pcg_flush(n, dx, pr, da, k, stag != 0, c->stream);
+    if (rc == PSK_OK && hipMemcpyAsync(x, dx, (size_t)n * 8, hipMemcpyDeviceToHost, c->stream) != hipSuccess)
+        rc = fail(PSK_ERR_HIP, "psk_lab_pcg_flush: copy back");
+    if (hipStreamSynchronize(c->stream) != hipSuccess && rc == PSK_OK) rc = fail(PSK_ERR_HIP, "psk_lab_pcg_flush: sync");
+    buf.release();
+    return rc;
+}
diff --git a/pysolvers_amd/csrc/pcg.hip b/pysolvers_amd/csrc/pcg.hip
--- a/pysolvers_amd/csrc/pcg.hip
+++ b/pysolvers_amd/csrc/pcg.hip
@@ -141,7 +141,7 @@
     gridsum_final_wave<2>(gs);
 }
 
-template <int JAC>
+template <int JAC, bool STAG>
 __global__ __launch_bounds__(kBlock) void pcg_direction_kernel(
     int64_t n, double *__restrict__ x, const double *__restrict__ r, PRing pr, const double *__restrict__ dinv,
     double ds, const double *__restrict__ pap, const double *__restrict__ rrur, int nparts, PcgState *st,
@@ -161,13 +161,16 @@
     const int64_t tile = tile_base + tile_of_block(tm);
     const double *pcur = pr.b[k % kPcgDefer];
     double *pnext = pr.b[(k + 1) % kPcgDefer];
-    const int q = pcg_pending(k);
+    constexpr int S = kPcgStagger > 0 ? kPcgStagger : 1;
+    const PcgPend pd = STAG ? pcg_flush_pending(S, pcg_block_of_tile(tile, (n + kVecTile - 1) / kVecTile, S), k, false)
+                            : pcg_uniform_pending(k);
+    const int q = (int)(k - pd.first);
     double alpha, beta;
     if (!pcg_direction_scalars(n, x, pcur, pTAp, rr, ur, udk, tauNB, st, udr, hist, k, maxiter, fail_on_maxiter,
-                               alpha, beta, tile, &pr, alphas))
+                               alpha, beta, tile, &pr, alphas, pd))
         return;
-    const bool flush = q == kPcgDefer - 1 || k == maxiter - 1;
-    const bool x0 = k < kPcgDefer;
+    const bool flush = (!STAG && q == kPcgDefer - 1) || k == maxiter - 1;
+    const bool x0 = pd.first == 0;
     if (tile == 0 && threadIdx.x == 0) {
         alphas[k] = alpha;
         if (flush) st->x_written = 1;
@@ -208,15 +211,29 @@
     } else if (i < n) {
         const double u0 = JAC == 2 ? ds * r[i] : JAC ? dinv[i] * r[i] : r[i];
         const double pi = pcur[i];
-        if (flush) x[i] = pcg_catch_up(x0 ? 0.0 : x[i], &pr, q, k, alphas, i) + alpha * pi;
+        if (flush) x[i] = pcg_catch_up(x0 ? 0.0 : x[i], &pr, pd.first, k, alphas, i) + alpha * pi;
         pnext[i] = u0 + beta * pi;
     }
 }
 
+template <bool STAG>
 __global__ void pcg_flush_kernel(int64_t n, double *__restrict__ x, PRing pr, const double *__restrict__ alphas,
                                  int64_t k) {
     const int64_t i = (int64_t)blockIdx.x * kBlock + threadIdx.x;
-    if (i < n) x[i] = pcg_catch_up(k < kPcgDefer ? 0.0 : x[i], &pr, pcg_pending(k), k, alphas, i);
+    constexpr int S = kPcgStagger > 0 ? kPcgStagger : 1;
+    const PcgPend pd = STAG ? pcg_flush_pending(S, pcg_block_of_tile(i / kVecTile, (n + kVecTile - 1) / kVecTile, S), k,
+                                                false)
+                            : pcg_uniform_pending(k);
+    if (i < n && pd.first <= pd.last) x[i] = pcg_catch_up(pd.first == 0 ? 0.0 : x[i], &pr, pd.first, k, alphas, i);
+}
+
+int launch_pcg_flush(int64_t n, double *x, const PRing &pr, const double *alphas, int64_t k, bool stag, hipStream_t s) {
+    if (n <= 0) return PSK_OK;
+    const dim3 g((unsigned)((n + kBlock - 1) / kBlock));
+    if (stag && kPcgStagger > 0) hipLaunchKernelGGL(pcg_flush_kernel<true>, g, dim3(kBlock), 0, s, n, x, pr, alphas, k);
+    else hipLaunchKernelGGL(pcg_flush_kernel<false>, g, dim3(kBlock), 0, s, n, x, pr, alphas, k);
+    PSK_HIP(hipGetLastError());
+    return PSK_OK;
 }
 
 constexpr int kPcgStateWords = (int)(sizeof(PcgState) / 8);
@@ -362,6 +379,10 @@
     return PSK_OK;
 }
 
+bool pcg_staggers(const psk_csr *A, const psk_prec *M) {
+    return kPcgStagger > 0 && !prec_is_general(M) && !A->comm && A->n > 0 && spmv_flush_eligible(A);
+}
+
 static void set_msg(psk_result *res, const char *m) {
     std::snprintf(res->msg, sizeof(res->msg), "%s", m);
 }
@@ -399,6 +420,7 @@
     const int64_t nv = n > 0 ? (n + kVecTile - 1) / kVecTile : 1;
     if (nv > INT32_MAX) return fail(PSK_ERR_UNSUPPORTED, "psk_pcg: vector too long for a one-shot grid");
     const bool init_diag = !gen && !sharded && (jac == 0 || jac == 2) && pcg_init_diag_eligible(A);
+    const bool stag = pcg_staggers(A, M);
     const int64_t nsl = n > 0 ? (n + kBlock - 1) / kBlock : 1;
     GridSum gs0, gs2, gs3;
     if (!init_diag) PSK_TRY(gridsum_prepare(c, gen ? nv : nsl, 2, w.pinit, &gs0));
@@ -536,9 +558,11 @@
             }
         }
         uint64_t seq1 = 0;
+        SpmvFlush fl{w.x, w.alphas, w.pr, k, nv, 0, 0, 0, 0};
         if (!(init_diag && k == 0) &&
             (rc = launch_spmv(A, kSpmvDot, pk, w.Ap, nullptr, nullptr, w.part1, &w.st->done, s, timed ? ta[slot] : nullptr,
-                              timed ? tb[slot] : nullptr, 0, mbc ? &seq1 : nullptr)) != PSK_OK)
+                              timed ? tb[slot] : nullptr, 0, mbc ? &seq1 : nullptr, stag && k >= 1 ? &fl : nullptr)) !=
+                PSK_OK)
             break;
         const TileMap tm2 = tile_map_for(nv, false);
         if (sharded) {
@@ -577,18 +601,14 @@
                 if (t1 <= t0) return;
                 const dim3 g3((unsigned)(t1 - t0));
                 const TileMap tm3 = tile_map_for(t1 - t0, false);
-                if (jac == 2)
-                    hipLaunchKernelGGL(pcg_direction_kernel<2>, g3, dim3(kBlock), 0, s, n, w.x, w.r, w.pr, dinv, ds,
-                                       w.part1g, w.part2g, P, w.st, w.udr, w.hist, w.alphas, k, maxiter,
-                                       ctl->fail_on_maxiter, t0, tm3);
-                else if (jac == 1)
-                    hipLaunchKernelGGL(pcg_direction_kernel<1>, g3, dim3(kBlock), 0, s, n, w.x, w.r, w.pr, dinv, ds,
-                                       w.part1g, w.part2g, P, w.st, w.udr, w.hist, w.alphas, k, maxiter,
-                                       ctl->fail_on_maxiter, t0, tm3);
-                else
-                    hipLaunchKernelGGL(pcg_direction_kernel<0>, g3, dim3(kBlock), 0, s, n, w.x, w.r, w.pr, dinv, ds,
-                                       w.part1g, w.part2g, P, w.st, w.udr, w.hist, w.alphas, k, maxiter,
-                                       ctl->fail_on_maxiter, t0, tm3);
+#define PSK_PCG_K3(J, SG)                                                                                      \
+                hipLaunchKernelGGL((pcg_direction_kernel<J, SG>), g3, dim3(kBlock), 0, s, n, w.x, w.r, w.pr, dinv, ds, \
+                                   w.part1g, w.part2g, P, w.st, w.udr, w.hist, w.alphas, k, maxiter,               \
+                                   ctl->fail_on_maxiter, t0, tm3)
+                if (jac == 2) { if (stag) PSK_PCG_K3(2, (kPcgStagger > 0)); else PSK_PCG_K3(2, false); }
+                else if (jac == 1) { if (stag) PSK_PCG_K3(1, (kPcgStagger > 0)); else PSK_PCG_K3(1, false); }
+                else { if (stag) PSK_PCG_K3(0, (kPcgStagger > 0)); else PSK_PCG_K3(0, false); }
+#undef PSK_PCG_K3
             };
             if (overlap && k + 1 < maxiter) {
                 k3(0, ov_lo);
@@ -660,12 +680,20 @@
             if (res->status == PSK_MAXITER) res->resid = maxiter > 0 ? res->resid_recursive : hs.normB;
             bool x_written = hs.x_written != 0;
             bool more = !dev_io;
-            if (!gen && hs.done == 2 && hs.brk_kind != 1 && pcg_pending(hs.iters) > 0 && n > 0) {
-                hipLaunchKernelGGL(pcg_flush_kernel, dim3((unsigned)((n + kBlock - 1) / kBlock)), dim3(kBlock), 0, s, n,
-                                   w.x, w.pr, w.alphas, (int64_t)hs.iters);
-                if (hipGetLastError() != hipSuccess) rc = fail(PSK_ERR_HIP, "pcg flush");
-                x_written = true;
-                more = true;
+            if (!gen && hs.done == 2 && hs.brk_kind != 1 && n > 0) {
+                bool pending = false;
+                const int nblk = stag ? kPcgStagger : 1;
+                for (int b = 0; b < nblk; ++b) {
+                    if (stag && (int64_t)b * pcg_block_tiles(nv, kPcgStagger) >= nv) continue;
+                    const PcgPend pd = stag ? pcg_flush_pending(kPcgStagger, b, hs.iters, false) : pcg_uniform_pending(hs.iters);
+                    pending = pending || pd.first <= pd.last;
+                    x_written = x_written || pd.first > 0;
+                }
+                if (pending) {
+                    rc = launch_pcg_flush(n, w.x, w.pr, w.alphas, (int64_t)hs.iters, stag, s);
+                    x_written = true;
+                    more = true;
+                }
             }
             if (rc == PSK_OK && !x_written && n > 0) {
                 if (hipMemsetAsync(w.x, 0, (size_t)n * 8, s) != hipSuccess) rc = fail(PSK_ERR_HIP, "x zero");
diff --git a/pysolvers_amd/csrc/pcg_state.hpp b/pysolvers_amd/csrc/pcg_state.hpp
--- a/pysolvers_amd/csrc/pcg_state.hpp
+++ b/pysolvers_amd/csrc/pcg_state.hpp
@@ -77,18 +77,52 @@
 };
 __host__ __device__ inline int pcg_pending(int64_t k) { return (int)(k % kPcgDefer); }
 
-__device__ __forceinline__ double pcg_catch_up(double xj, const PRing *pr, int q, int64_t k,
+#ifndef PSK_PCG_STAGGER
+#define PSK_PCG_STAGGER 1
+#endif
+#define PSK_PCG_STAGGER_ON (PSK_PCG_STAGGER && PSK_PCG_DEFER >= 2)
+constexpr int kPcgStagger = PSK_PCG_STAGGER_ON ? kPcgDefer - 1 : 0;
+static_assert(kPcgStagger >= 0 && kPcgStagger < kPcgDefer, "SpMV k reads p_{k-S} after K3 k-1 wrote p_k: S < ring");
+
+struct PcgPend {
+    int64_t first, last;
+};
+__host__ __device__ inline int64_t pcg_block_tiles(int64_t nv, int S) { return (nv + S - 1) / S; }
+__host__ __device__ inline int pcg_block_of_tile(int64_t tile, int64_t nv, int S) {
+    return (int)(tile / pcg_block_tiles(nv, S));
+}
+__host__ __device__ inline PcgPend pcg_flush_pending(int S, int blk, int64_t k, bool in_spmv) {
+    const int64_t kk = in_spmv ? k - 1 : k;
+    int64_t f = kk - ((kk - blk) % S + S) % S;
+    if (f < 1) f = 0;
+    return PcgPend{f, k - 1};
+}
+__host__ __device__ inline PcgPend pcg_uniform_pending(int64_t k) { return PcgPend{k - pcg_pending(k), k - 1}; }
+
+__device__ __forceinline__ double pcg_catch_up(double xj, const PRing *pr, int64_t first, int64_t k,
                                                const double *__restrict__ alphas, int64_t j) {
-    for (int t = q; t >= 1; --t) xj = xj + alphas[k - t] * pr->b[(k - t) % kPcgDefer][j];
+    for (int64_t t = first; t < k; ++t) xj = xj + alphas[t] * pr->b[t % kPcgDefer][j];
     return xj;
 }
+
+struct SpmvFlush {
+    double *x;
+    const double *alphas;
+    PRing pr;
+    int64_t k;
+    int64_t nv;
+    uint32_t ost, ofl;
+    uint32_t nfl;
+    uint32_t mul;
+};
 
 __device__ inline bool pcg_direction_scalars(int64_t n, double *__restrict__ x, const double *__restrict__ p,
                                              double pTAp, double rr, double ur, double udk, double tauNB,
                                              PcgState *st, double *__restrict__ udr, double *__restrict__ hist, int64_t k,
                                              int64_t maxiter, int fail_on_maxiter, double &alpha, double &beta,
                                              int64_t tile, const PRing *pr = nullptr,
-                                             const double *__restrict__ alphas = nullptr) {
+                                             const double *__restrict__ alphas = nullptr,
+                                             PcgPend pd = PcgPend{0, -1}) {
     alpha = udk / pTAp;
     const double normR = sqrt(rr);
     if (tile == 0 && threadIdx.x == 0) {
@@ -97,10 +131,10 @@
     }
     if (normR <= tauNB || (!fail_on_maxiter && k == maxiter - 1)) {
         const int64_t i = tile * kVecTile + 2 * threadIdx.x;
-        const bool x0 = pr && k < kPcgDefer;
+        const bool x0 = pr && pd.first == 0;
         for (int64_t j = i; j < i + 2 && j < n; ++j) {
             double xj = x0 ? 0.0 : x[j];
-            if (pr) xj = pcg_catch_up(xj, pr, pcg_pending(k), k, alphas, j);
+            if (pr) xj = pcg_catch_up(xj, pr, pd.first, k, alphas, j);
             x[j] = xj + alpha * p[j];
         }
         if (tile == 0 && threadIdx.x == 0) {
@@ -117,6 +151,9 @@
 }
 
 bool pcg_init_diag_eligible(const psk_csr *A);
+bool spmv_flush_eligible(const psk_csr *A);
+bool pcg_staggers(const psk_csr *A, const psk_prec *M);
+int launch_pcg_flush(int64_t n, double *x, const PRing &pr, const double *alphas, int64_t k, bool stag, hipStream_t s);
 int launch_pcg_init_diag(const psk_csr *A, const double *b, double xs, double *p, double *Ap, double *out3,
                          const PcgInitFin &fin, hipStream_t s);
 
diff --git a/pysolvers_amd/csrc/psk_internal.hpp b/pysolvers_amd/csrc/psk_internal.hpp
--- a/pysolvers_amd/csrc/psk_internal.hpp
+++ b/pysolvers_amd/csrc/psk_internal.hpp
@@ -682,12 +682,11 @@
 inline TileMap tile_map_chunked(int64_t ntiles, int64_t c) {
     return c > 0 && ntiles >= 8 * c ? TileMap{0, 0, 0, c} : TileMap{0, 0, 0, 0};
 }
-__device__ __forceinline__ int64_t tile_of_block(TileMap tm) {
-    const int64_t b = blockIdx.x;
+__device__ __forceinline__ int64_t tile_of_index(TileMap tm, int64_t b, int64_t g) {
     if (tm.c > 0) {
         const int64_t k = b & 7, j = b >> 3;
         const int64_t t = ((j / tm.c) * 8 + k) * tm.c + j % tm.c;
-        const int64_t full = (int64_t)(gridDim.x / (8 * tm.c)) * 8 * tm.c;
+        const int64_t full = (int64_t)(g / (8 * tm.c)) * 8 * tm.c;
         return b < full ? t : b;
     }
     if (tm.a == 0) return b;
@@ -695,6 +694,7 @@
     const int64_t start = k * tm.a + (k < tm.r ? k : tm.r);
     return tm.rev ? start + (tm.a + (k < tm.r ? 1 : 0)) - 1 - j : start + j;
 }
+__device__ __forceinline__ int64_t tile_of_block(TileMap tm) { return tile_of_index(tm, blockIdx.x, gridDim.x); }
 
 typedef double dv2 __attribute__((ext_vector_type(2)));
 __device__ __forceinline__ dv2 ld2(const double *p) { return *reinterpret_cast<const dv2 *>(p); }
@@ -767,8 +767,10 @@
 int tile_rows_for(int64_t n, int64_t nnz);
 int csr_choose_layout(psk_csr *A, hipStream_t s);
 void sliced_free(psk_csr *A);
+struct SpmvFlush;
 int launch_spmv(const psk_csr *A, int mode, const double *x, double *y, const double *aux_d,
                 const double *aux_q, double *partial, const int32_t *done_flag, hipStream_t s,
-                hipEvent_t ev0 = nullptr, hipEvent_t ev1 = nullptr, int rev = 0, uint64_t *mail_seq = nullptr);
-
-}
+                hipEvent_t ev0 = nullptr, hipEvent_t ev1 = nullptr, int rev = 0, uint64_t *mail_seq = nullptr,
+                const SpmvFlush *flush = nullptr);
+
+}
diff --git a/pysolvers_amd/csrc/spmv.hip b/pysolvers_amd/csrc/spmv.hip
--- a/pysolvers_amd/csrc/spmv.hip
+++ b/pysolvers_amd/csrc/spmv.hip
@@ -681,12 +681,50 @@
     }
 }
 
-template <int MODE, int NB, int H>
+__host__ __device__ inline uint32_t spmv_flush_octets_before(const SpmvFlush &f, uint32_t o) {
+    if (f.mul == 0) return o > f.ost ? o - f.ost : 0;
+    return (uint32_t)(((uint64_t)o * f.mul) >> 16);
+}
+__device__ __forceinline__ const SpmvFlush &spmv_flush_arg(const SpmvFlush &f) { return f; }
+
+template <int S>
+__device__ __forceinline__ void spmv_flush_tile(const SpmvFlush &fl, uint32_t f, int64_t n) {
+    const int64_t k = fl.k;
+    const int blk = (int)(k % S);
+    const PcgPend pd = pcg_flush_pending(S, blk, k, true);
+    const int q = (int)(k - pd.first);
+    const bool x0 = pd.first == 0;
+    const int64_t i = ((int64_t)blk * pcg_block_tiles(fl.nv, S) + f) * kVecTile + 2 * threadIdx.x;
+    double *__restrict__ x = fl.x;
+    if (i + 1 < n) {
+        dv2 xo{0.0, 0.0};
+        if (!x0) xo = ld2nt(x + i);
+        dv2 pp[S];
+#pragma unroll
+        for (int t = 1; t <= S; ++t)
+            if (t <= q) pp[t - 1] = ld2nt(fl.pr.b[(k - t) % kPcgDefer] + i);
+#pragma unroll
+        for (int t = S; t >= 1; --t)
+            if (t <= q) {
+                const double a = fl.alphas[k - t];
+                xo.x = xo.x + a * pp[t - 1].x;
+                xo.y = xo.y + a * pp[t - 1].y;
+            }
+        st2nt(x + i, xo);
+    } else if (i < n) {
+        x[i] = pcg_catch_up(x0 ? 0.0 : x[i], &fl.pr, pd.first, k, fl.alphas, i);
+    }
+}
+
+template <int MODE, int NB, int H, typename... FLUSH>
 __global__ __launch_bounds__(kBlock, (H == 2 && MODE != kSpmvPlain && MODE != kSpmvDot) ? 4 : 8) void spmv_diagp_kernel(
     int64_t n, const uint8_t *__restrict__ mask, DiagDesc dd, const double *__restrict__ x, double *__restrict__ y,
     const double *__restrict__ aux_d, const double *__restrict__ aux_q, GridSum gs, const int32_t *__restrict__ done,
-    TileMap tm, int64_t ntiles) {
+    TileMap tm, int64_t ntiles, FLUSH... flush) {
     constexpr int KM = 5;
+    constexpr bool FL = sizeof...(FLUSH) == 1;
+    static_assert(sizeof...(FLUSH) <= 1 && (!FL || (MODE == kSpmvDot && H == 2 && kPcgStagger > 0)),
+                  "the flush role rides on the PCG loop's launch only");
     static_assert(NB == 1 || NB == 2, "the 5-diagonal DPP orders");
     static_assert(H == 1 || H == 2, "half-slices per wave");
     constexpr int JD = NB == 1 ? 0 : 2, JM1 = NB == 1 ? 3 : 1, JP1 = NB == 1 ? 4 : 3;
@@ -697,7 +735,21 @@
     const int32_t dnv = (done ? done : &g_spmv_never_done)[spmv_vzero()];
     const int lane = threadIdx.x & 63;
     const int wave = __builtin_amdgcn_readfirstlane(threadIdx.x >> 6);
-    const int64_t grp = tile_of_block(tm);
+    int64_t sidx = blockIdx.x, scnt = gridDim.x;
+    if constexpr (FL) {
+        const SpmvFlush &fl = spmv_flush_arg(flush...);
+        const uint32_t o = blockIdx.x >> 3, fb = spmv_flush_octets_before(fl, o);
+        if (spmv_flush_octets_before(fl, o + 1) != fb) {
+            const uint32_t f = fb * 8 + (blockIdx.x & 7);
+            if (f >= fl.nfl || __builtin_amdgcn_readfirstlane(dnv) != 0) return;
+            spmv_flush_tile<kPcgStagger>(fl, f, n);
+            return;
+        }
+        sidx = (int64_t)(o - fb) * 8 + (blockIdx.x & 7);
+        scnt = (gs.nt + TPB - 1) / TPB;
+        if (sidx >= scnt) return;
+    }
+    const int64_t grp = tile_of_index(tm, sidx, scnt);
     const int64_t t = grp * TPB + (H == 2 ? wave : wave >> 1);
     const bool tv = t < ntiles;
     const int64_t tl = tv ? t : ntiles - 1;
@@ -759,7 +811,15 @@
         if (threadIdx.x < TPB) gsl[threadIdx.x].cnt = 0;
         __syncthreads();
     }
-    if (pub && threadIdx.x == 0 && blockIdx.x == 0 && (gs.nt + TPB - 1) / TPB != gridDim.x) atomicOr(gs.err, 2);
+    if constexpr (FL) {
+        const SpmvFlush &fl = spmv_flush_arg(flush...);
+        const uint32_t ot = gridDim.x >> 3;
+        if (pub && threadIdx.x == 0 && sidx == 0 &&
+            ((gridDim.x & 7) != 0 || (scnt + 7) / 8 != (int64_t)(ot - spmv_flush_octets_before(fl, ot))))
+            atomicOr(gs.err, 2);
+    } else {
+        if (pub && threadIdx.x == 0 && blockIdx.x == 0 && (gs.nt + TPB - 1) / TPB != gridDim.x) atomicOr(gs.err, 2);
+    }
 #pragma unroll
     for (int h = 0; h < H; ++h)
 #pragma unroll
@@ -1523,11 +1583,36 @@
 
 static int64_t spmv_tiles(const psk_csr *A) { return (A->n + A->tile_rows - 1) / A->tile_rows; }
 
+static uint32_t spmv_flush_grid(SpmvFlush &fl, int64_t nwgp) {
+    constexpr int S = kPcgStagger > 0 ? kPcgStagger : 1;
+    const int64_t per = pcg_block_tiles(fl.nv, S), t0 = (fl.k % S) * per;
+    const int64_t nf = std::min(fl.nv, t0 + per) - t0;
+    fl.nfl = nf > 0 ? (uint32_t)nf : 0;
+    if (fl.nfl == 0) return 0;
+    const int64_t ost = (nwgp + 7) / 8, ofl = (nf + 7) / 8;
+    if ((ost + ofl + 2) * 8 > (int64_t)INT32_MAX) return 0;
+    fl.ost = (uint32_t)ost;
+    fl.ofl = (uint32_t)ofl;
+    uint32_t ot = (uint32_t)(ost + ofl);
+    const int64_t mul = (ofl * 65536 + ot - 1) / ot;
+    fl.mul = (uint32_t)std::min<int64_t>(std::max<int64_t>(mul, 1), 65535);
+    while (ot < (uint32_t)(ost + ofl + 2) * 2 &&
+           (spmv_flush_octets_before(fl, ot) < fl.ofl || ot - spmv_flush_octets_before(fl, ot) < fl.ost))
+        ++ot;
+    if (spmv_flush_octets_before(fl, ot) < fl.ofl || ot - spmv_flush_octets_before(fl, ot) != fl.ost) {
+        fl.mul = 0;
+        ot = (uint32_t)(ost + ofl);
+    }
+    return ot * 8;
+}
+
 int launch_spmv(const psk_csr *A, int mode, const double *x, double *y, const double *aux_d,
                 const double *aux_q, double *partial, const int32_t *done_flag, hipStream_t s, hipEvent_t ev0,
-                hipEvent_t ev1, int rev, uint64_t *mail_seq) {
+                hipEvent_t ev1, int rev, uint64_t *mail_seq, const SpmvFlush *flush) {
     Context *c;
     PSK_TRY(ctx(&c));
+    if (flush && (mode != kSpmvDot || !partial || !spmv_flush_eligible(A) || kPcgStagger == 0 || flush->k < 1))
+        return fail(PSK_ERR_ARG, "launch_spmv: the flush role needs the PCG loop's launch in the diagonal pair layout");
     const bool sliced = A->sl_off != nullptr || A->dg_mask != nullptr;
     const int64_t nwg = sliced ? (A->n + kSlice - 1) / kSlice : spmv_tiles(A);
     GridSum gs{nullptr, nullptr, nullptr, nullptr, 0, 0, -1, nullptr, nullptr, 0, 0};
@@ -1564,6 +1649,23 @@
         const int64_t nwgp = pairh ? (nwg + (pairh == 2 ? 4 : 2) - 1) / (pairh == 2 ? 4 : 2) : 1;
         const dim3 gdp((unsigned)nwgp);
         const TileMap tmp = tile_map_for(nwgp, spmv_xcd_bands(), rev != 0);
+#if PSK_PCG_STAGGER_ON
+        if (flush) {
+            SpmvFlush fl = *flush;
+            const uint32_t grid = spmv_flush_grid(fl, nwgp);
+            if (fl.nfl > 0) {
+                if (grid == 0) return fail(PSK_ERR_UNSUPPORTED, "launch_spmv: grid too large for the flush role");
+                if (nbk == 1)
+                    hipExtLaunchKernelGGL((spmv_diagp_kernel<kSpmvDot, 1, 2, SpmvFlush>), dim3(grid), bd, 0, s, ev0,
+                                          ev1, 0, A->n, A->dg_mask, dd, x, y, aux_d, aux_q, gs, done_flag, tmp, nwg, fl);
+                else
+                    hipExtLaunchKernelGGL((spmv_diagp_kernel<kSpmvDot, 2, 2, SpmvFlush>), dim3(grid), bd, 0, s, ev0,
+                                          ev1, 0, A->n, A->dg_mask, dd, x, y, aux_d, aux_q, gs, done_flag, tmp, nwg, fl);
+                PSK_HIP(hipGetLastError());
+                return PSK_OK;
+            }
+        }
+#endif
 #define PSK_DIAGP(M, NB, H)                                                                                        \
     hipExtLaunchKernelGGL((spmv_diagp_kernel<M, NB, H>), gdp, bd, 0, s, ev0, ev1, 0, A->n, A->dg_mask, dd, x, y, aux_d, \
                           aux_q, gs, done_flag, tmp, nwg)
@@ -1701,6 +1803,9 @@
 }
 
 bool pcg_init_diag_eligible(const psk_csr *A) { return !A->comm && A->n > 0 && diag_nb(A) != 0; }
+bool spmv_flush_eligible(const psk_csr *A) {
+    return !A->comm && diag_nb(A) != 0 && A->n >= 2 && A->ncols >= 2 && diag_pair_h() == 2;
+}
 
 int launch_pcg_init_diag(const psk_csr *A, const double *b, double xs, double *p, double *Ap, double *out3,
                          const PcgInitFin &fin, hipStream_t s) {
```

New measurement: 7406 (median of 6 runs). 1.04x the previous value.
